# hku-mars/loam_livox

Measured on AMD Instinct MI355X. Metric: scans_per_s, higher is better.
Workload: dtype f32 points / f64 solve; 1 GPU; C2: 24k-pt Mid-40 scan vs 5M-pt corner+surface map, 10 ICP iters (fixed), k=5, Q-full; scan_points=24000, map_points=4975193, map_corner=995155, map_surf=3980038, icp_iters=10, distinct_scans_in_batch=256

## Files before the change

### __graft_entry__.py

```python
import os
import sys

ROOT = os.path.dirname(os.path.abspath(__file__))
if ROOT not in sys.path:
    sys.path.insert(0, ROOT)


def build() -> None:
    from loam_livox_amd import build as b
    lib = b.build()
    assert os.path.exists(lib)
    from oracle import orc
    orc.build()
    from tests.hostcheck import hc
    hc.build()
    from oracle import ref
    ref.build()
    from tests.test_ll_node import build_node
    build_node()
    from tests import verbatim_build
    verbatim_build.build()
    verbatim_build.build_sequence()
    verbatim_build.build_feature()
    verbatim_build.build_keyframes()
    verbatim_build.build_scene_alignment()
    verbatim_build.build_loop_detector()
    verbatim_build.build_cell_refresh()
    verbatim_build.build_mapping_io()
    import loam_livox_amd
    from loam_livox_amd import capi
    capi.load()


def smoke() -> None:
    import numpy as np

    from loam_livox_amd import synth
    from loam_livox_amd.api import Livox_laser, Map_buffer, Point_cloud_registration
    from oracle import orc

    world, corner, surf = synth.make_maps(60_000)
    sc = synth.make_scan(world, 0, n=6000)
    fe = Livox_laser(max_points=6000)
    fe.extract_laser_features(sc.xyzi, 9.0)
    g = fe.get_features(0.0, 1.0)
    o = orc.fe_extract(sc.xyzi, 10.0)
    ci, si, fi = orc.fe_get_features(o, 0.0, 1.0)
    assert np.array_equal(fe.pts_info()["pt_label"], o.pt_label), "label mismatch vs oracle"
    assert np.array_equal(g["corner_idx"], ci) and np.array_equal(g["surf_idx"], si), "index set mismatch vs oracle"
    m = Map_buffer()
    m.setInputCloud(Map_buffer.CORNER, corner)
    m.setInputCloud(Map_buffer.SURF, surf)
    reg = Point_cloud_registration(max_features=6000)
    p = reg.params
    p.icp_max_iterations, p.ceres_max_iterations, p.force_all_iterations = 4, 20, 1
    p.para_max_angular_rate, p.para_max_speed = 20.0, 0.3
    reg.m_pose_w_last = sc.pose_init.copy()
    reg.m_pose_w_curr = sc.pose_init.copy()
    ret = reg.find_out_incremental_transfrom(m, g["pc_corners"], g["pc_surface"])
    prm = orc.RegParams.defaults(icp_iters=4, ceres_iters=20, force_all=1)
    oret, opc, _, _ = orc.reg_solve(orc.KdTree(corner), orc.KdTree(surf), orc.feature_cloud(o, ci), orc.feature_cloud(o, si),
                                    prm, sc.pose_init, sc.pose_init)
    dt, dr = synth.pose_error(reg.m_pose_w_curr, opc)
    assert ret == oret and dt < 1e-4 and dr < 1e-4, f"pose mismatch vs oracle: {dt} m {dr} rad"
    print(f"smoke ok: labels/index sets identical, pose diff vs oracle {dt:.2e} m {dr:.2e} rad")


if __name__ == "__main__":
    build()
    if "--smoke" in sys.argv:
        smoke()
```

### include/loam_livox_hip.h

```cpp
#ifndef LOAM_LIVOX_HIP_H
#define LOAM_LIVOX_HIP_H

#include <stdint.h>

#ifdef __cplusplus
extern "C" {
#endif

typedef struct ll_fe ll_fe;
typedef struct ll_map ll_map;
typedef struct ll_reg ll_reg;

enum { LL_PT_NORMAL = 0, LL_PT_000 = 1, LL_PT_TOO_NEAR = 2, LL_PT_REFL_LOW = 4, LL_PT_REFL_HIGH = 8,
       LL_PT_CIRCLE_EDGE = 16, LL_PT_NAN = 32, LL_PT_SMALL_VIEW_ANGLE = 64 };
enum { LL_LABEL_INVALID = -1, LL_LABEL_UNLABELED = 0, LL_LABEL_CORNER = 1, LL_LABEL_SURFACE = 2,
       LL_LABEL_NEAR_NAN = 4, LL_LABEL_NEAR_ZERO = 8, LL_LABEL_HIGH_INTENSITY = 16 };


typedef struct {
    float thr_corner_curvature;
    float thr_surface_curvature;
    float minimum_view_angle;
    float livox_min_allow_dis;
    float livox_min_sigma;
    float max_fov;
    float time_internal_pts;
    int32_t device;
    int32_t max_points;
    int32_t max_scans;
    int32_t piecewise_number;
} ll_fe_params;

void ll_fe_default_params(ll_fe_params *p);
int ll_fe_create(const ll_fe_params *p, ll_fe **out);
void ll_fe_destroy(ll_fe *h);

int ll_fe_extract(ll_fe *h, const float *xyzi, int32_t n, double time_stamp, int32_t *n_petal_clouds);

int ll_fe_labels(ll_fe *h, int32_t scan, int32_t *pt_type, int32_t *pt_label, float *depth_sq2,
                 float *polar_dis_sq2, float *curvature, float *view_angle, float *time_stamp, float *polar_angle);

int ll_fe_splits(ll_fe *h, int32_t scan, int32_t *split_idx, int32_t *n_split, int32_t *clutter_size,
                 int32_t *n_petal_clouds, int32_t *first_idx, int32_t *last_idx, float *piece_start, float *piece_end);

int ll_fe_select(ll_fe *h, float minimum_blur, float maximum_blur, int32_t *corner_idx, int32_t *n_corner,
                 int32_t *surf_idx, int32_t *n_surf, int32_t *full_idx, int32_t *n_full, float *corner_xyzi,
                 float *surf_xyzi);

int ll_fe_upload(ll_fe *h, int32_t first_scan, int32_t n_scans, const float *xyzi, int32_t n_points,
                 const double *current_time);
int ll_fe_upload_async(ll_fe *h, int32_t first_scan, int32_t n_scans, const float *xyzi, int32_t n_points,
                       const double *current_time);
int ll_fe_extract_batch(ll_fe *h, int32_t n_scans);
int ll_fe_select_batch(ll_fe *h, int32_t n_scans, int32_t piece, float minimum_blur, float maximum_blur);
int ll_fe_selection(ll_fe *h, int32_t scan, int32_t *corner_idx, int32_t *n_corner, int32_t *surf_idx, int32_t *n_surf,
                    int32_t *full_idx, int32_t *n_full, float *corner_xyzi, float *surf_xyzi);
int ll_fe_counts(ll_fe *h, int32_t n_scans, int32_t *n_corner, int32_t *n_surf, int32_t *n_full,
                 int32_t *n_ambiguous);
int ll_fe_sync(ll_fe *h);
int ll_fe_resolve(ll_fe *h);


enum { LL_MAP_CORNER = 0, LL_MAP_SURF = 1 };

int ll_map_create(int32_t device, ll_map **out);
void ll_map_destroy(ll_map *m);
int ll_map_upload(ll_map *m, int32_t kind, const float *xyz, int32_t stride_floats, int64_t n, float cell_size);
int64_t ll_map_size(const ll_map *m, int32_t kind);

int64_t ll_map_generation(const ll_map *m, int32_t kind);
int64_t ll_map_cells(const ll_map *m, int32_t kind);
int ll_map_upload_gen(ll_map *m, int32_t kind, const float *xyz, int32_t stride_floats, int64_t n, float cell_size, int64_t *generation);
int ll_map_to_f16(ll_map *m, int32_t kind);
int ll_map_dequantized(ll_map *m, int32_t kind, float *xyz, int64_t capacity_points);

int ll_map_knn5(ll_map *m, int32_t kind, const float *queries_xyz, int32_t n_queries, float max_sq_dis,
                int32_t *idx5, float *sq_dis5);
int ll_map_knn5_device(ll_map *m, int32_t kind, const float *dev_queries_xyz, int64_t n_queries, float max_sq_dis, int32_t *dev_idx5,
                       float *dev_sq_dis5, float *kernel_ms);


typedef struct {
    int32_t if_motion_deblur;
    int32_t icp_max_iterations;
    int32_t ceres_max_iterations;
    int32_t ceres_prerun_times;
    int32_t icp_line;
    int32_t icp_plane;
    int32_t current_frame_index;
    int32_t mapping_init_accumulate_frames;
    int32_t maximum_allow_residual_block;
    int32_t force_all_iterations;
    double maximum_dis_line_for_match;
    double maximum_dis_plane_for_match;
    double huber_a;
    double inliner_dis;
    double inlier_ratio;
    double minimum_icp_R_diff;
    double minimum_icp_T_diff;
    float para_max_angular_rate;
    float para_max_speed;
    float max_final_cost;
    float minimum_pt_time_stamp;
    float maximum_pt_time_stamp;
    int32_t if_line_feature_check;
    int32_t if_plane_feature_check;
    int32_t subsample_seed;
} ll_reg_params;

void ll_reg_default_params(ll_reg_params *p);

typedef struct {
    double final_cost, initial_cost;
    double inlier_threshold;
    double angular_diff_deg, t_diff;
    int32_t icp_iterations;
    int32_t n_blocks_last;
    int32_t corner_avail, surf_avail;
    int32_t lm_iterations_total;
    int32_t accepted;
    int32_t gated;
    int32_t aborted;
} ll_reg_report;

int ll_reg_create(int32_t device, int32_t max_scans, int32_t max_features_per_scan, ll_reg **out);
void ll_reg_destroy(ll_reg *r);

int ll_reg_solve(ll_reg *r, const ll_map *map, const float *scan_corner_xyzi, int32_t n_corner,
                 const float *scan_surf_xyzi, int32_t n_surf, const ll_reg_params *prm, const double pose_last[7],
                 double pose_curr[7], double pose_incre[7], ll_reg_report *rep);

int ll_reg_solve_batch_fe(ll_reg *r, const ll_map *map, ll_fe *fe, int32_t n_scans, const ll_reg_params *prm,
                          const double *poses_last, double *poses_curr, double *poses_incre, ll_reg_report *reports,
                          int32_t *results);
int ll_reg_upload_features(ll_reg *r, int32_t n_scans, const float *corner_xyzi, const int32_t *n_corner, int32_t stride_corner,
                           const float *surf_xyzi, const int32_t *n_surf, int32_t stride_surf);
int ll_reg_enqueue_uploaded(ll_reg *r, const ll_map *map, int32_t n_scans, const ll_reg_params *prm, const double *poses_last,
                            const double *poses_curr, const double *poses_incre);

int ll_reg_solve_batch(ll_reg *r, const ll_map *map, int32_t n_scans, const float *corner_xyzi,
                       const int32_t *n_corner, int32_t stride_corner, const float *surf_xyzi, const int32_t *n_surf,
                       int32_t stride_surf, const ll_reg_params *prm, const double *poses_last, double *poses_curr,
                       double *poses_incre, ll_reg_report *reports, int32_t *results);

int ll_reg_enqueue_fe_merged(ll_reg *r, const ll_map *map, ll_fe *fe, int32_t n_scans, int32_t heads, const ll_reg_params *prm,
                             const double *poses_last, const double *poses_curr, const double *poses_incre);
int ll_reg_enqueue_fe(ll_reg *r, const ll_map *map, ll_fe *fe, int32_t n_scans, const ll_reg_params *prm,
                      const double *poses_last, const double *poses_curr, const double *poses_incre);
int ll_reg_collect(ll_reg *r, int32_t n_scans, double *poses_curr, double *poses_incre, ll_reg_report *reports,
                   int32_t *results);

int ll_debug_quintic(int32_t device, const double *args10, int32_t n, double *out_sequential, double *out_wavefront);

int ll_reg_debug_knn(ll_reg *r, int32_t scan, int32_t *corner_idx5, float *corner_d25, int32_t *surf_idx5,
                     float *surf_d25);
int ll_reg_set_debug(ll_reg *r, int32_t enable);
int ll_reg_set_debug_knn_iteration(ll_reg *r, int32_t icp_iteration);

typedef struct ll_voxel ll_voxel;
int ll_voxel_create(int32_t device, int32_t max_clouds, int32_t max_points_per_cloud, ll_voxel **out);
void ll_voxel_destroy(ll_voxel *v);
int ll_voxel_filter(ll_voxel *v, int32_t n_clouds, const float *xyzi, const int32_t *n_points, int32_t stride_points,
                    const float leaf[3], float *out_xyzi, int32_t *n_out, int32_t *status);

int ll_reg_enqueue_fe_downsampled(ll_reg *r, const ll_map *map, ll_fe *fe, ll_voxel *vox_corner, ll_voxel *vox_surf,
                                  float line_res, float plane_res, int32_t n_scans, const ll_reg_params *prm,
                                  const double *poses_last, const double *poses_curr, const double *poses_incre);
int ll_reg_enqueue_fe_maps(ll_reg *r, const ll_map *const *maps, ll_fe *fe, int32_t n_scans, const ll_reg_params *prm,
                           const int32_t *frame_index, const double *poses_last, const double *poses_curr, const double *poses_incre);
int ll_reg_enqueue_fe_downsampled_maps(ll_reg *r, const ll_map *const *maps, ll_fe *fe, ll_voxel *vox_corner, ll_voxel *vox_surf,
                                       float line_res, float plane_res, int32_t n_scans, const ll_reg_params *prm,
                                       const int32_t *frame_index, const double *poses_last, const double *poses_curr,
                                       const double *poses_incre);
int ll_voxel_counts(ll_voxel *v, int32_t n_clouds, int32_t *n_out, int32_t *status);

typedef struct ll_history ll_history;
int ll_history_create(int32_t device, int32_t maximum_history_size, int32_t max_points_per_frame, float line_res, float plane_res,
                      ll_history **out);
void ll_history_destroy(ll_history *h);
int ll_history_add(ll_history *h, const float *corner_xyzi, int32_t n_corner, const float *surf_xyzi, int32_t n_surf,
                   const double pose[7], double history_add_t_step, double history_add_angle_step, int32_t *added);
int ll_history_add_fe(ll_history *h, ll_fe *fe, int32_t scan, const double pose[7], double history_add_t_step,
                      double history_add_angle_step, int32_t *added);
int ll_history_add_voxel(ll_history *h, ll_voxel *vox_corner, ll_voxel *vox_surf, int32_t cloud, const double pose[7],
                         double history_add_t_step, double history_add_angle_step, int32_t *added);
int ll_history_set_gate_pose(ll_history *h, const double pose[7]);
int ll_history_refresh(ll_history *h, ll_map *map, int64_t *n_map_corner, int64_t *n_map_surf);
int32_t ll_history_size(const ll_history *h);
int64_t ll_history_map_cloud(ll_history *h, int32_t kind, float *xyzi, int64_t capacity_points);
int ll_history_map_cloud_device(ll_history *h, int32_t kind, const float **dev_xyzi, int64_t *n_points);

typedef struct ll_history_batch ll_history_batch;
int ll_history_batch_create(int32_t device, int32_t n_sequences, int32_t maximum_history_size, int32_t max_points_per_frame,
                            float line_res, float plane_res, ll_history_batch **out);
void ll_history_batch_destroy(ll_history_batch *h);
int ll_history_batch_add_voxel(ll_history_batch *h, ll_voxel *vox_corner, ll_voxel *vox_surf, const int32_t *active,
                               const double *poses7, const double *gate_poses7, double history_add_t_step,
                               double history_add_angle_step, int32_t *added);
int ll_history_batch_add_fe(ll_history_batch *h, ll_fe *fe, const int32_t *active, const double *poses7, const double *gate_poses7,
                            double history_add_t_step, double history_add_angle_step, int32_t *added);
int ll_history_batch_refresh(ll_history_batch *h, ll_map *const *maps, const int32_t *active, int64_t *n_map_corner,
                             int64_t *n_map_surf);
int32_t ll_history_batch_size(const ll_history_batch *h, int32_t sequence);
int64_t ll_history_batch_map_cloud(ll_history_batch *h, int32_t sequence, int32_t kind, float *xyzi, int64_t capacity_points);
int ll_history_batch_enable_cell_maps(ll_history_batch *h, int64_t initial_points_per_map, float cell_resolution,
                                      int32_t threshold_cell_revisit);
int ll_history_batch_sync_cell_maps(ll_history_batch *h);
int ll_history_batch_cell_map_stats(ll_history_batch *h, int32_t sequence, int32_t kind, int64_t *n_cells, int64_t *n_points,
                                    int32_t *frame_idx);
int ll_history_batch_cell_map_dump(ll_history_batch *h, int32_t sequence, int32_t kind, float *xyzi, int64_t capacity_points,
                                   int32_t *cell_ijk, int32_t *cell_start, int32_t *cell_last_update, int64_t capacity_cells);
int ll_history_batch_cell_map_device_view(ll_history_batch *h, int32_t sequence, int32_t kind, const float **dev_xyz0,
                                          const uint64_t **dev_point_keys, int64_t *n_points, int64_t *n_cells);
int ll_history_batch_cell_map_work(ll_history_batch *h, int64_t out[4]);
int ll_history_batch_refresh_cells(ll_history_batch *h, ll_map *const *maps, const int32_t *active, const double *poses7,
                                   float maximum_search_range_corner, float maximum_search_range_surface,
                                   float maximum_in_fov_angle, int32_t down_sample_replace,
                                   int64_t *n_map_corner, int64_t *n_map_surf);
int ll_history_batch_cell_match_work(ll_history_batch *h, int64_t out[8]);
int ll_history_batch_enable_full_maps(ll_history_batch *h, int64_t initial_points_per_map, float cell_resolution,
                                      int32_t threshold_cell_revisit);
int ll_history_batch_append_full_fe(ll_history_batch *h, ll_fe *fe, const int32_t *active, const double *poses7, int32_t min_points,
                                    int64_t *n_touched);
int ll_history_batch_full_touched(ll_history_batch *h, int32_t sequence, int32_t *cell_ijk, int64_t capacity_cells, int64_t *n);
int ll_history_batch_full_map_work(ll_history_batch *h, int64_t out[4]);
int ll_map_grid_geometry(const float bbox_min_max[6], float cell_size, int32_t dims[3], float *cell, float *slack);

typedef struct ll_cellmap ll_cellmap;
int ll_cellmap_create(int32_t device, int64_t max_points, float resolution, int32_t minimum_revisit_threshold, ll_cellmap **out);
void ll_cellmap_destroy(ll_cellmap *c);
int ll_cellmap_reserve(ll_cellmap *c, int64_t max_points);
int ll_cellmap_append(ll_cellmap *c, const float *xyzi, int32_t n);
int ll_cellmap_append_touched(ll_cellmap *c, const float *xyzi, int32_t n, int32_t min_points, int32_t *cell_ijk, int64_t capacity_cells,
                              int64_t *n_touched);
int ll_cellmap_query_filter(ll_cellmap *c, const double pose[7], float radius, float maximum_in_fov_angle, float leaf,
                            int32_t down_sample_replace, int64_t *n_cells_selected, int64_t *n_out);
int64_t ll_cellmap_result(ll_cellmap *c, float *xyzi, int64_t capacity_points);
int ll_cellmap_stats(const ll_cellmap *c, int64_t *n_cells, int64_t *n_points, int32_t *frame_idx);
int ll_cellmap_dump(ll_cellmap *c, float *xyzi, int64_t capacity_points, int32_t *cell_ijk, int32_t *cell_start,
                    int32_t *cell_last_update, int64_t capacity_cells);
int ll_cellmap_device_view(ll_cellmap *c, const float **dev_xyz0, const uint64_t **dev_point_keys, int64_t *n_points, int64_t *n_cells);
int ll_cellmap_extract_cells(ll_cellmap *src, const int32_t *cell_ijk, int64_t n_list, ll_cellmap *dst, int64_t *n_cells_found,
                             int64_t *n_points);
int ll_history_batch_extract_cells(ll_history_batch *h, int32_t kind, int32_t n_requests, const int32_t *sequences,
                                   const int64_t *list_offsets, const int32_t *cell_ijk, ll_cellmap *const *dst, int64_t *n_cells_found,
                                   int64_t *n_points);
int ll_history_batch_extract_work(ll_history_batch *h, int64_t out[4]);

int ll_cellmap_features(ll_cellmap *c, int32_t *feature_type, float *feature_vector, float *mean, float *cov, float *eigen_val,
                        int64_t capacity_cells);

int ll_cellmap_keyframe_images(ll_cellmap *c, float roi_ratio, float *images, float *ratio_nonzero, float *eigen_R, int32_t *n_vectors,
                               float *centre_and_range);
int ll_keyframe_similarity(int32_t device, const float *img_a, const float *img_b, float *similarity);

int ll_cellmap_feature_clouds(ll_cellmap *c, float *line_xyzi, int64_t capacity_line, int64_t *n_line, float *plane_xyzi, int64_t capacity_plane,
                              int64_t *n_plane, float centre[3]);
typedef struct ll_scene_align ll_scene_align;
typedef struct {
    float line_res, plane_res;
    int32_t maximum_icp_iteration;
    float accepted_threshold;
    int32_t maximum_residual_block;
    int32_t registrar_init;
    int32_t subsample_seed;
} ll_scene_align_params;
void ll_scene_align_default_params(ll_scene_align_params *p);
int ll_scene_align_create(int32_t device, int64_t initial_points, ll_scene_align **out);
void ll_scene_align_destroy(ll_scene_align *h);
int ll_scene_align_run(ll_scene_align *h, ll_cellmap *keyframe_a, ll_cellmap *keyframe_b, const ll_scene_align_params *p, double pose[7],
                       double *inlier_threshold, ll_reg_report reports[3], int32_t *n_reports);
int ll_scene_align_work(ll_scene_align *h, int64_t out[4]);

typedef struct ll_keyframe_bank ll_keyframe_bank;
int ll_keyframe_bank_create(int32_t device, int64_t initial_entries, ll_keyframe_bank **out);
void ll_keyframe_bank_destroy(ll_keyframe_bank *b);
int ll_keyframe_bank_add_cellmap(ll_keyframe_bank *b, ll_cellmap *c, float roi_ratio, float *images, float *ratio_nonzero, float *eigen_R,
                                 int32_t *n_vectors, float *centre_and_range, int64_t *id);
int ll_keyframe_bank_add_images(ll_keyframe_bank *b, const float *img_line, const float *img_plane, int64_t *id);
int ll_keyframe_bank_images(ll_keyframe_bank *b, int64_t id, float *img_line, float *img_plane);
int64_t ll_keyframe_bank_size(const ll_keyframe_bank *b);
int ll_keyframe_bank_match(ll_keyframe_bank *b, int64_t n_pairs, const int64_t *ids_a, const int64_t *ids_b, float *sim_line,
                           float *sim_plane);
int ll_keyframe_bank_debug_surface(ll_keyframe_bank *b, int64_t id_a, int64_t id_b, int32_t kind, double *out);
int ll_keyframe_bank_work(ll_keyframe_bank *b, int64_t out[4]);

typedef struct ll_pose_graph ll_pose_graph;
typedef struct {
    int32_t max_num_iterations;
    int32_t max_num_consecutive_invalid_steps;
    double initial_trust_region_radius;
    double max_trust_region_radius;
    double min_trust_region_radius;
    double min_relative_decrease;
    double min_lm_diagonal, max_lm_diagonal;
    double function_tolerance;
    double gradient_tolerance;
    double parameter_tolerance;
} ll_pose_graph_params;
#define LL_POSE_GRAPH_MAX_ITERATIONS 0
#define LL_POSE_GRAPH_GRADIENT 1
#define LL_POSE_GRAPH_PARAMETER 2
#define LL_POSE_GRAPH_FUNCTION 3
#define LL_POSE_GRAPH_RADIUS 4
#define LL_POSE_GRAPH_INVALID_STEPS 5
// ... 86 lines not shown
```

### loam_livox_amd/build.py

```python
from __future__ import annotations

import os
import shutil
import subprocess
import sys

HERE = os.path.dirname(os.path.abspath(__file__))
CSRC = os.path.join(HERE, "csrc")
LIB = os.environ.get("LL_LIB_OUT") or os.path.join(HERE, "libloamlivox_hip.so")
SOURCES = ["ll_api_common.hip", "ll_api_fe.hip", "ll_api_map.hip", "ll_api_reg.hip", "ll_api_voxel.hip", "ll_api_cellmap.hip", "ll_api_scene_align.hip", "ll_api_keyframe_bank.hip", "ll_api_pose_graph.hip", "ll_api_history.hip", "ll_api_history_batch_buffer.hip", "ll_api_history_batch_stores.hip", "ll_api_history_batch_extract.hip", "ll_api_history_batch_cells.hip", "ll_fe_kernels.hip", "ll_map_kernels.hip", "ll_reg_query_kernels.hip", "ll_reg_solve_kernels.hip", "ll_reg_maps_kernels.hip", "ll_reg_aux_kernels.hip", "ll_reg_small_kernels.hip", "ll_knn_kernels.hip", "ll_voxel_kernels.hip", "ll_cellmap_kernels.hip", "ll_cellmap_extract_kernels.hip", "ll_cellmap_select_kernels.hip", "ll_spin_kernels.hip", "ll_spin_api.hip", "ll_history_batch_kernels.hip", "ll_cellmap_batch_kernels.hip", "ll_cellmap_batch_extract_kernels.hip", "ll_cellmatch_batch_kernels.hip", "ll_fullmap_batch_kernels.hip", "ll_keyframe_bank_kernels.hip", "ll_pose_graph_kernels.hip"]
HEADERS = ["ll_api_internal.h", "ll_api_history_batch_internal.h", "ll_device.h", "ll_fe_core.h", "ll_knn_core.h", "ll_knn_coop.h", "ll_knn_tile.h", "ll_reg_query.h", "ll_reg_solve_fast.h", "ll_reg_big_path.h", "ll_reg_solve_general.h", "ll_reg_solve_common.h", "ll_reg_small_solve.h", "ll_reg_core.h", "ll_voxel.h", "ll_voxel_core.h", "ll_cellmap.h", "ll_cellmap_core.h", "ll_cellmap_select_core.h", "ll_spin.h", "ll_spin_core.h", "ll_history_batch.h", "ll_cellmap_batch.h", "ll_cellmap_batch_core.h", "ll_cellmap_batch_extract_core.h", "ll_cellmatch_batch.h", "ll_cellmatch_batch_core.h", "ll_fullmap_batch.h", "ll_fullmap_batch_core.h", "ll_keyframe_bank.h", "ll_keyframe_bank_core.h", "ll_pose_graph.h", "ll_pose_graph_core.h", "../../include/loam_livox_hip.h"]
FLAGS = ["--offload-arch=gfx950", "-O3", "-std=c++17", "-fPIC", "-ffp-contract=off", "-Wno-unused-result"]
FLAGS += os.environ.get("LL_EXTRA_HIPCC_FLAGS", "").split()


def hipcc() -> str:
    for cand in (shutil.which("hipcc"), "/opt/rocm/bin/hipcc"):
        if cand and os.path.exists(cand):
            return cand
    raise RuntimeError("hipcc not found (ROCm toolchain required to build libloamlivox_hip.so)")



def needs_build(lib: str = LIB) -> bool:
    if not os.path.exists(lib):
        return True
    t = os.path.getmtime(lib)
    deps = [os.path.join(CSRC, f) for f in SOURCES + HEADERS] + [os.path.abspath(__file__)]
    return any(os.path.getmtime(d) > t for d in deps)


def build(force: bool = False, verbose: bool = False, lib: str = LIB, extra_flags=()) -> str:
    if not force and not needs_build(lib):
        return lib
    cc = hipcc()
    default = os.path.join(HERE, "libloamlivox_hip.so")
    objdir = os.path.join(HERE, "build" if lib == default else "build_" + os.path.basename(lib).replace(".so", ""))
    os.makedirs(objdir, exist_ok=True)
    objs = []
    procs = []
    for src in SOURCES:
        obj = os.path.join(objdir, src.replace(".hip", ".o"))
        cmd = [cc] + FLAGS + list(extra_flags) + ["-c", os.path.join(CSRC, src), "-o", obj]
        if verbose:
            print(" ".join(cmd), file=sys.stderr)
        procs.append((src, subprocess.Popen(cmd, stdout=subprocess.PIPE, stderr=subprocess.STDOUT)))
        objs.append(obj)
    for src, p in procs:
        out, _ = p.communicate()
        if p.returncode != 0:
            raise RuntimeError(f"hipcc failed on {src}:\n{out.decode()}")
        if verbose and out:
            print(out.decode(), file=sys.stderr)
    cmd = [cc, "--offload-arch=gfx950", "-shared", "-fPIC", "-o", lib] + objs
    subprocess.check_call(cmd)
    return lib


if __name__ == "__main__":
    print(build(force="--force" in sys.argv, verbose=True))
```

### loam_livox_amd/capi.py

```python
from __future__ import annotations

import ctypes as C
import os

import numpy as np

_HERE = os.path.dirname(os.path.abspath(__file__))
LIB_PATH = os.environ.get("LOAM_LIVOX_LIB", os.path.join(_HERE, "libloamlivox_hip.so"))


class LoamLivoxError(RuntimeError):
    pass


class FeParams(C.Structure):
    _fields_ = [("thr_corner_curvature", C.c_float), ("thr_surface_curvature", C.c_float),
                ("minimum_view_angle", C.c_float), ("livox_min_allow_dis", C.c_float), ("livox_min_sigma", C.c_float),
                ("max_fov", C.c_float), ("time_internal_pts", C.c_float), ("device", C.c_int32),
                ("max_points", C.c_int32), ("max_scans", C.c_int32), ("piecewise_number", C.c_int32)]


class SpinParams(C.Structure):
    _fields_ = [("scan_line", C.c_int32), ("minimum_range", C.c_float), ("plane_resolution", C.c_float), ("device", C.c_int32),
                ("max_points", C.c_int32), ("max_scans", C.c_int32), ("max_line_points", C.c_int32)]
# ... 18 lines not shown
                ("n_blocks_last", C.c_int32), ("corner_avail", C.c_int32), ("surf_avail", C.c_int32),
                ("lm_iterations_total", C.c_int32), ("accepted", C.c_int32), ("gated", C.c_int32), ("aborted", C.c_int32)]


class SceneAlignParams(C.Structure):
    _fields_ = [("line_res", C.c_float), ("plane_res", C.c_float), ("maximum_icp_iteration", C.c_int32), ("accepted_threshold", C.c_float),
                ("maximum_residual_block", C.c_int32), ("registrar_init", C.c_int32), ("subsample_seed", C.c_int32)]


class PoseGraphParams(C.Structure):
    _fields_ = [("max_num_iterations", C.c_int32), ("max_num_consecutive_invalid_steps", C.c_int32),
                ("initial_trust_region_radius", C.c_double), ("max_trust_region_radius", C.c_double),
                ("min_trust_region_radius", C.c_double), ("min_relative_decrease", C.c_double), ("min_lm_diagonal", C.c_double),
                ("max_lm_diagonal", C.c_double), ("function_tolerance", C.c_double), ("gradient_tolerance", C.c_double),
                ("parameter_tolerance", C.c_double)]


class PoseGraphSummary(C.Structure):
    _fields_ = [("iterations", C.c_int32), ("successful_steps", C.c_int32), ("unsuccessful_steps", C.c_int32), ("termination", C.c_int32),
                ("initial_cost", C.c_double), ("final_cost", C.c_double)]


POSE_GRAPH_TERMINATION = ("max_iterations", "gradient", "parameter", "function", "radius", "invalid_steps", "nothing")


_vp, _i32, _i64, _f, _d = C.c_void_p, C.c_int32, C.c_int64, C.c_float, C.c_double
SYMBOLS = {
    "ll_fe_default_params": (None, [C.POINTER(FeParams)]),
    "ll_fe_create": (_i32, [C.POINTER(FeParams), C.POINTER(_vp)]),
    "ll_fe_destroy": (None, [_vp]),
    "ll_fe_extract": (_i32, [_vp, _vp, _i32, _d, C.POINTER(_i32)]),
    "ll_fe_labels": (_i32, [_vp, _i32] + [_vp] * 8),
    "ll_fe_splits": (_i32, [_vp, _i32, _vp, C.POINTER(_i32), C.POINTER(_i32), C.POINTER(_i32), _vp, _vp, _vp, _vp]),
    "ll_fe_select": (_i32, [_vp, _f, _f, _vp, C.POINTER(_i32), _vp, C.POINTER(_i32), _vp, C.POINTER(_i32), _vp, _vp]),
    "ll_fe_selection": (_i32, [_vp, _i32, _vp, C.POINTER(_i32), _vp, C.POINTER(_i32), _vp, C.POINTER(_i32), _vp, _vp]),
    "ll_fe_upload": (_i32, [_vp, _i32, _i32, _vp, _i32, _vp]),
    "ll_fe_upload_async": (_i32, [_vp, _i32, _i32, _vp, _i32, _vp]),
    "ll_fe_extract_batch": (_i32, [_vp, _i32]),
    "ll_fe_select_batch": (_i32, [_vp, _i32, _i32, _f, _f]),
    "ll_fe_counts": (_i32, [_vp, _i32, _vp, _vp, _vp, _vp]),
    "ll_fe_sync": (_i32, [_vp]),
    "ll_fe_resolve": (_i32, [_vp]),
    "ll_map_create": (_i32, [_i32, C.POINTER(_vp)]),
    "ll_map_destroy": (None, [_vp]),
    "ll_map_upload": (_i32, [_vp, _i32, _vp, _i32, _i64, _f]),
    "ll_map_upload_gen": (_i32, [_vp, _i32, _vp, _i32, _i64, _f, _vp]),
    "ll_map_size": (_i64, [_vp, _i32]),
    "ll_map_generation": (_i64, [_vp, _i32]),
    "ll_map_to_f16": (_i32, [_vp, _i32]),
    "ll_map_dequantized": (_i32, [_vp, _i32, _vp, _i64]),
    "ll_map_cells": (_i64, [_vp, _i32]),
    "ll_map_knn5": (_i32, [_vp, _i32, _vp, _i32, _f, _vp, _vp]),
    "ll_map_knn5_device": (_i32, [_vp, _i32, _vp, _i64, _f, _vp, _vp, _vp]),
    "ll_reg_default_params": (None, [C.POINTER(RegParams)]),
    "ll_reg_create": (_i32, [_i32, _i32, _i32, C.POINTER(_vp)]),
    "ll_reg_destroy": (None, [_vp]),
    "ll_reg_solve": (_i32, [_vp, _vp, _vp, _i32, _vp, _i32, C.POINTER(RegParams), _vp, _vp, _vp, C.POINTER(RegReport)]),
    "ll_reg_solve_batch_fe": (_i32, [_vp, _vp, _vp, _i32, C.POINTER(RegParams), _vp, _vp, _vp, _vp, _vp]),
    "ll_reg_solve_batch": (_i32, [_vp, _vp, _i32, _vp, _vp, _i32, _vp, _vp, _i32, C.POINTER(RegParams), _vp, _vp, _vp,
                                  _vp, _vp]),
    "ll_reg_upload_features": (_i32, [_vp, _i32, _vp, _vp, _i32, _vp, _vp, _i32]),
    "ll_reg_enqueue_uploaded": (_i32, [_vp, _vp, _i32, C.POINTER(RegParams), _vp, _vp, _vp]),
    "ll_reg_enqueue_fe": (_i32, [_vp, _vp, _vp, _i32, C.POINTER(RegParams), _vp, _vp, _vp]),
    "ll_reg_enqueue_fe_merged": (_i32, [_vp, _vp, _vp, _i32, _i32, C.POINTER(RegParams), _vp, _vp, _vp]),
    "ll_reg_collect": (_i32, [_vp, _i32, _vp, _vp, _vp, _vp]),
    "ll_reg_debug_knn": (_i32, [_vp, _i32, _vp, _vp, _vp, _vp]),
    "ll_reg_set_debug": (_i32, [_vp, _i32]),
    "ll_reg_set_debug_knn_iteration": (_i32, [_vp, _i32]),
    "ll_cloud_transform": (_i32, [_vp, _vp, _vp, _i32, _vp]),
    "ll_cloud_transform_fe_device": (_i32, [_vp, _vp, _i32, _i32, _vp, _vp, _vp, _i64, _vp]),
    "ll_reg_set_profiling": (_i32, [_vp, _i32]),
    "ll_reg_kernel_times": (_i32, [_vp, _vp, _vp]),
    "ll_reg_debug_cycles": (_i32, [_vp, _i32, _vp]),
    "ll_reg_debug_worklists": (_i32, [_vp, _i32, _vp]),
    "ll_voxel_create": (_i32, [_i32, _i32, _i32, C.POINTER(_vp)]),
    "ll_voxel_destroy": (None, [_vp]),
    "ll_voxel_filter": (_i32, [_vp, _i32, _vp, _vp, _i32, _vp, _vp, _vp, _vp]),
    "ll_voxel_counts": (_i32, [_vp, _i32, _vp, _vp]),
    "ll_reg_enqueue_fe_downsampled": (_i32, [_vp, _vp, _vp, _vp, _vp, _f, _f, _i32, C.POINTER(RegParams), _vp, _vp, _vp]),
    "ll_reg_enqueue_fe_maps": (_i32, [_vp, _vp, _vp, _i32, C.POINTER(RegParams), _vp, _vp, _vp, _vp]),
    "ll_reg_enqueue_fe_downsampled_maps": (_i32, [_vp, _vp, _vp, _vp, _vp, _f, _f, _i32, C.POINTER(RegParams), _vp, _vp, _vp, _vp]),
    "ll_history_create": (_i32, [_i32, _i32, _i32, _f, _f, C.POINTER(_vp)]),
    "ll_history_destroy": (None, [_vp]),
    "ll_history_add": (_i32, [_vp, _vp, _i32, _vp, _i32, _vp, C.c_double, C.c_double, _vp]),
    "ll_history_add_fe": (_i32, [_vp, _vp, _i32, _vp, C.c_double, C.c_double, _vp]),
    "ll_history_add_voxel": (_i32, [_vp, _vp, _vp, _i32, _vp, C.c_double, C.c_double, _vp]),
    "ll_history_refresh": (_i32, [_vp, _vp, _vp, _vp]),
    "ll_history_size": (_i32, [_vp]),
    "ll_history_map_cloud": (_i64, [_vp, _i32, _vp, _i64]),
    "ll_history_set_gate_pose": (_i32, [_vp, _vp]),
    "ll_history_map_cloud_device": (_i32, [_vp, _i32, _vp, _vp]),
    "ll_history_batch_create": (_i32, [_i32, _i32, _i32, _i32, _f, _f, C.POINTER(_vp)]),
    "ll_history_batch_destroy": (None, [_vp]),
    "ll_history_batch_add_voxel": (_i32, [_vp, _vp, _vp, _vp, _vp, _vp, C.c_double, C.c_double, _vp]),
    "ll_history_batch_add_fe": (_i32, [_vp, _vp, _vp, _vp, _vp, C.c_double, C.c_double, _vp]),
    "ll_history_batch_refresh": (_i32, [_vp, _vp, _vp, _vp, _vp]),
    "ll_history_batch_size": (_i32, [_vp, _i32]),
    "ll_history_batch_map_cloud": (_i64, [_vp, _i32, _i32, _vp, _i64]),
    "ll_history_batch_enable_cell_maps": (_i32, [_vp, _i64, C.c_float, _i32]),
    "ll_history_batch_sync_cell_maps": (_i32, [_vp]),
    "ll_history_batch_cell_map_stats": (_i32, [_vp, _i32, _i32, _vp, _vp, _vp]),
    "ll_history_batch_cell_map_dump": (_i32, [_vp, _i32, _i32, _vp, _i64, _vp, _vp, _vp, _i64]),
    "ll_history_batch_cell_map_device_view": (_i32, [_vp, _i32, _i32, _vp, _vp, _vp, _vp]),
    "ll_history_batch_cell_map_work": (_i32, [_vp, _vp]),
    "ll_history_batch_refresh_cells": (_i32, [_vp, _vp, _vp, _vp, C.c_float, C.c_float, C.c_float, _i32, _vp, _vp]),
    "ll_history_batch_cell_match_work": (_i32, [_vp, _vp]),
    "ll_history_batch_enable_full_maps": (_i32, [_vp, _i64, C.c_float, _i32]),
    "ll_history_batch_append_full_fe": (_i32, [_vp, _vp, _vp, _vp, _i32, _vp]),
    "ll_history_batch_full_touched": (_i32, [_vp, _i32, _vp, _i64, _vp]),
    "ll_history_batch_full_map_work": (_i32, [_vp, _vp]),
    "ll_history_batch_extract_cells": (_i32, [_vp, _i32, _i32, _vp, _vp, _vp, _vp, _vp, _vp]),
    "ll_history_batch_extract_work": (_i32, [_vp, _vp]),
    "ll_map_grid_geometry": (_i32, [_vp, _f, _vp, _vp, _vp]),
    "ll_cellmap_create": (_i32, [_i32, _i64, C.c_float, _i32, _vp]),
    "ll_cellmap_destroy": (None, [_vp]),
    "ll_cellmap_reserve": (_i32, [_vp, _i64]),
    "ll_cellmap_device_view": (_i32, [_vp, _vp, _vp, _vp, _vp]),
    "ll_cellmap_extract_cells": (_i32, [_vp, _vp, _i64, _vp, _vp, _vp]),
    "ll_cellmap_append": (_i32, [_vp, _vp, _i32]),
    "ll_cellmap_append_touched": (_i32, [_vp, _vp, _i32, _i32, _vp, _i64, C.POINTER(_i64)]),
    "ll_cellmap_query_filter": (_i32, [_vp, _vp, C.c_float, C.c_float, C.c_float, _i32, _vp, _vp]),
    "ll_cellmap_result": (_i64, [_vp, _vp, _i64]),
    "ll_cellmap_stats": (_i32, [_vp, _vp, _vp, _vp]),
    "ll_cellmap_dump": (_i32, [_vp, _vp, _i64, _vp, _vp, _vp, _i64]),
    "ll_cellmap_features": (_i32, [_vp, _vp, _vp, _vp, _vp, _vp, _i64]),
    "ll_cellmap_keyframe_images": (_i32, [_vp, C.c_float, _vp, _vp, _vp, _vp, _vp]),
    "ll_keyframe_similarity": (_i32, [_i32, _vp, _vp, _vp]),
    "ll_cellmap_feature_clouds": (_i32, [_vp, _vp, _i64, C.POINTER(_i64), _vp, _i64, C.POINTER(_i64), _vp]),
    "ll_scene_align_default_params": (None, [C.POINTER(SceneAlignParams)]),
    "ll_scene_align_create": (_i32, [_i32, _i64, C.POINTER(_vp)]),
    "ll_scene_align_destroy": (None, [_vp]),
    "ll_scene_align_run": (_i32, [_vp, _vp, _vp, C.POINTER(SceneAlignParams), _vp, C.POINTER(_d), _vp, C.POINTER(_i32)]),
    "ll_scene_align_work": (_i32, [_vp, _vp]),
    "ll_keyframe_bank_create": (_i32, [_i32, _i64, C.POINTER(_vp)]),
    "ll_keyframe_bank_destroy": (None, [_vp]),
    "ll_keyframe_bank_add_cellmap": (_i32, [_vp, _vp, C.c_float, _vp, _vp, _vp, _vp, _vp, C.POINTER(_i64)]),
    "ll_keyframe_bank_add_images": (_i32, [_vp, _vp, _vp, C.POINTER(_i64)]),
    "ll_keyframe_bank_images": (_i32, [_vp, _i64, _vp, _vp]),
    "ll_keyframe_bank_size": (_i64, [_vp]),
    "ll_keyframe_bank_match": (_i32, [_vp, _i64, _vp, _vp, _vp, _vp]),
    "ll_keyframe_bank_debug_surface": (_i32, [_vp, _i64, _i64, _i32, _vp]),
    "ll_keyframe_bank_work": (_i32, [_vp, _vp]),
    "ll_pose_graph_default_params": (None, [C.POINTER(PoseGraphParams)]),
    "ll_pose_graph_create": (_i32, [_i32, _i64, _i64, _i64, _i64, C.POINTER(_vp)]),
    "ll_pose_graph_destroy": (None, [_vp]),
    "ll_pose_graph_solve": (_i32, [_vp, C.POINTER(PoseGraphParams), _i64, _vp, _vp, _vp, _vp, _vp, _vp, _vp]),
    "ll_pose_graph_work": (_i32, [_vp, _vp]),
    "ll_history_enable_cell_map": (_i32, [_vp, _i64, C.c_float, _i32]),
    "ll_history_set_cell_map_async": (_i32, [_vp, _i32]),
    "ll_history_sync_cell_maps": (_i32, [_vp]),
    "ll_history_cell_map": (_vp, [_vp, _i32]),
    "ll_history_refresh_cells": (_i32, [_vp, _vp, _vp, C.c_float, C.c_float, C.c_float, _i32, _vp, _vp]),
    "ll_debug_quintic": (_i32, [_i32, _vp, _i32, _vp, _vp]),
    "ll_spin_default_params": (None, [C.POINTER(SpinParams)]),
    "ll_spin_create": (_i32, [C.POINTER(SpinParams), C.POINTER(_vp)]),
    "ll_spin_destroy": (None, [_vp]),
    "ll_spin_upload": (_i32, [_vp, _i32, _i32, _vp, _vp, _i32]),
    "ll_spin_extract_batch": (_i32, [_vp, _i32]),
    "ll_spin_resolve": (_i32, [_vp]),
    "ll_spin_sync": (_i32, [_vp]),
    "ll_spin_counts": (_i32, [_vp, _i32, _vp, _vp]),
    "ll_spin_cloud": (_i32, [_vp, _i32, _i32, _vp, _vp, C.POINTER(_i32)]),
    "ll_spin_lines": (_i32, [_vp, _i32, _vp, _vp]),
    "ll_spin_extract": (_i32, [_vp, _vp, _i32]),
    "ll_spin_kernel_times": (_i32, [_vp, _vp]),
    "ll_reg_enqueue_spin": (_i32, [_vp, _vp, _vp, _i32, C.POINTER(RegParams), _vp, _vp, _vp]),
    "ll_reg_enqueue_spin_downsampled": (_i32, [_vp, _vp, _vp, _vp, _vp, _f, _f, _i32, C.POINTER(RegParams), _vp, _vp, _vp]),
    "ll_history_add_spin": (_i32, [_vp, _vp, _i32, _vp, C.c_double, C.c_double, _vp]),
    "ll_cloud_transform_spin_device": (_i32, [_vp, _vp, _i32, _i32, _vp, _vp, _vp, _i64, _vp]),
    "ll_spin_handoff_time": (_i32, [_vp, _vp]),
    "ll_reg_stream": (_vp, [_vp]),
    "ll_fe_stream": (_vp, [_vp]),
    "ll_runtime_hint_hw_queues": (_i32, [_i32]),
    "ll_last_error": (C.c_char_p, []),
    "ll_version": (C.c_char_p, []),
}

_lib = None




def hint_hw_queues(n: int = 16) -> bool:
    return check(load().ll_runtime_hint_hw_queues(int(n)), "ll_runtime_hint_hw_queues") == 1


def load():
    global _lib
    if _lib is not None:
        return _lib
    if not os.path.exists(LIB_PATH):
        raise LoamLivoxError(
            f"{LIB_PATH} not found: build it with `python -m loam_livox_amd.build` (hipcc, gfx950). "
            "There is no CPU fallback.")
    try:
        L = C.CDLL(LIB_PATH)
    except OSError as e:
        raise LoamLivoxError(f"cannot load {LIB_PATH}: {e} (ROCm runtime required; there is no CPU fallback)") from e
    for name, (res, args) in SYMBOLS.items():
        fn = getattr(L, name)
        fn.restype = res
        fn.argtypes = args
    _lib = L
    return L


class use_library:

    def __init__(self, path: str):
        self.path = path

    def __enter__(self):
        global _lib, LIB_PATH
        self.saved = (_lib, LIB_PATH)
        _lib, LIB_PATH = None, self.path
        try:
            return load()
        except Exception:
            _lib, LIB_PATH = self.saved
            raise

    def __exit__(self, *exc):
        global _lib, LIB_PATH
        _lib, LIB_PATH = self.saved
        return False


def check(rc: int, what: str = "") -> int:
    if rc < 0:
        msg = load().ll_last_error()
        raise LoamLivoxError(f"{what}: {msg.decode() if msg else 'error'}")
    return rc


def ptr(a):
    return None if a is None else a.ctypes.data_as(C.c_void_p)


def fe_default_params() -> FeParams:
    p = FeParams()
    load().ll_fe_default_params(C.byref(p))
    return p


def spin_default_params() -> SpinParams:
    p = SpinParams()
    load().ll_spin_default_params(C.byref(p))
    return p


def reg_default_params() -> RegParams:
    p = RegParams()
    load().ll_reg_default_params(C.byref(p))
    return p


def scene_align_default_params() -> SceneAlignParams:
    p = SceneAlignParams()
    load().ll_scene_align_default_params(C.byref(p))
    return p


def pose_graph_default_params() -> PoseGraphParams:
    p = PoseGraphParams()
    load().ll_pose_graph_default_params(C.byref(p))
    return p


def as_f32(a, cols=None):
    a = np.ascontiguousarray(a, dtype=np.float32)
    if cols is not None:
        a = a.reshape(-1, cols)
    return a
```

### loam_livox_amd/csrc/ll_api_reg.hip

```cpp
#include "ll_api_internal.h"

extern "C" void ll_reg_default_params(ll_reg_params *p)
{
    memset(p, 0, sizeof(*p));
    p->if_motion_deblur = 0;
    p->icp_max_iterations = 20;
    p->ceres_max_iterations = 100;
    p->ceres_prerun_times = 2;
    p->icp_line = 1;
    p->icp_plane = 1;
    p->if_line_feature_check = 0;
    p->if_plane_feature_check = 0;
    p->subsample_seed = 0;
    p->current_frame_index = 101;
    p->mapping_init_accumulate_frames = 100;
    p->maximum_allow_residual_block = 100000;
    p->force_all_iterations = 0;
    p->maximum_dis_line_for_match = 2.0;
    p->maximum_dis_plane_for_match = 50.0;
    p->huber_a = 0.1;
    p->inliner_dis = 0.02;
    p->inlier_ratio = 0.80;
    p->minimum_icp_R_diff = 0.01;
    p->minimum_icp_T_diff = 0.01;
// ... 286 lines not shown
    return 0;
}

static int reg_size_check(const char *where, const ll_reg *r, const ll_reg_params *prm, int max_nc, int max_ns, const char *cite)
{
    if (max_nc > r->dev.cap_c || max_ns > r->dev.cap_s) return set_err(where, "feature count exceeds the registrar capacity");
    if (!prm->subsample_seed && (max_nc > prm->maximum_allow_residual_block || max_ns > prm->maximum_allow_residual_block))
        return set_err(where, (std::string("feature count exceeds maximum_allow_residual_block and subsample_seed is 0 (strict mode): raise the "
                                           "limit, or set a seed to get the reference's sub-sampling ") + cite + "with a reproducible random stream").c_str());
    return 0;
}

static int reg_finish(ll_reg *r, int n_scans, PinGuard &pin_guard)
{
    prof_begin(r, 2);
    launch_reg_finalize(r->dev, r->rc, n_scans, r->stream);
    prof_end(r);
    HC(hipGetLastError());
    pin_guard.keep = true;
    return 0;
}

static int reg_enqueue(const char *where, ll_reg *r, const ll_map *map, int n_scans, const ll_reg_params *prm, const double *poses_last,
                       const double *poses_curr, const double *poses_incre, const int *known_counts = nullptr)
{
    if (!map) return set_err(where, "null argument");
    if (reg_params_check(where, r, n_scans, prm, poses_last, poses_curr)) return -1;
    if (map->device != r->device) return set_err(where, "map lives on another device");
    int debug = 0;
    if (reg_begin(r, prm, &debug)) return -1;
    PinGuard pin_guard{r};
    r->pinned[0] = map_pin(map, 0);
    r->pinned[1] = map_pin(map, 1);
    const MapKind empty_kind{};
    const MapKind &mk0 = r->pinned[0] ? r->pinned[0]->mk : empty_kind, &mk1 = r->pinned[1] ? r->pinned[1]->mk : empty_kind;
    const bool run = mk0.n > 0 && mk1.n > 50 && prm->current_frame_index > prm->mapping_init_accumulate_frames;
    r->last_gated = run ? 0 : 1;
    r->last_n_scans = n_scans;
    for (int b = 0; b < n_scans; b++) reg_init_state(r->h_state[b], b, poses_last, poses_curr, poses_incre, run);
    if (reg_exchange_counts(r, n_scans, false, n_scans == 1 ? known_counts : nullptr)) return -1;
    int max_nc = 0, max_ns = 0;
    for (int b = 0; b < n_scans; b++) {
        max_nc = r->h_nc[b] > max_nc ? r->h_nc[b] : max_nc;
        max_ns = r->h_ns[b] > max_ns ? r->h_ns[b] : max_ns;
    }
    if (reg_size_check(where, r, prm, max_nc, max_ns, "(point_cloud_registration.hpp:232-238,339-345,438-458) ")) return -1;
    if (prm->subsample_seed && (max_nc > 2 * prm->maximum_allow_residual_block || max_ns > 2 * prm->maximum_allow_residual_block))
        r->rc.knn_reuse = 0;
    if (max_ns < LL_KNN_TILE_MIN_SURF || max_ns > LL_KNN_TILE_MAX_SURF || (n_scans <= LL_KNN_COOP_MAX_SCANS && !(debug & 2048))) r->rc.knn_tile = 0;
    if (r->rc.knn_tile == 2 && max_ns > LL_KNN_TILE_SEG) r->rc.knn_tile = 1;
    if (r->rc.knn_tile == 2) r->rc.knn_reuse = 0;
    r->rc.solve_group = (r->rc.solve_group == 1 || n_scans > LL_GRP_MAX_SCANS || r->rc.if_motion_deblur || r->rc.force_general ||
                         max_nc + max_ns < LL_GRP_MIN_BLOCKS) ? 1 : LL_GRP;
    if (run) {
        if (!mk0.pts || !mk1.pts) return set_err(where, "map not uploaded (or converted to fp16 points: the registrar needs the fp32 records)");
        Grid g0 = mk0.grid, g1 = mk1.grid;
        g0.guard = g1.guard = r->rc.knn_reuse ? 0.05f : 0.0f;
        if (r->rc.solve_group > 1)
            HC(hipMemsetAsync(r->dev.grp_xch, 0, (size_t)n_scans * 2 * LL_GRP * 56 * sizeof(unsigned long long), r->stream));
        for (int it = 0; it < prm->icp_max_iterations; it++) {
            r->rc.xch_epoch = it + 1;
            prof_begin(r, 0);
            launch_reg_knn_build(r->dev, r->rc, g0, g1, n_scans, it, max_nc, max_ns, r->stream);
            prof_end(r);
            prof_begin(r, 1);
            if (r->rc.solve_group > 1) HC(hipMemsetAsync(r->dev.grp_ctl, 0, (size_t)(2 * n_scans + 1) * sizeof(int), r->stream));
            launch_reg_solve(r->dev, r->rc, mk1.grid, n_scans, max_nc, max_ns, it, r->stream);
            prof_end(r);
        }
    }
    return reg_finish(r, n_scans, pin_guard);
}

extern "C" int ll_reg_collect(ll_reg *r, int32_t n_scans, double *poses_curr, double *poses_incre, ll_reg_report *reports,
                              int32_t *results)
{
    if (!r) return set_err("ll_reg_collect", "null handle");
    if (n_scans < 1 || n_scans > r->max_scans) return set_err("ll_reg_collect", "n_scans out of range");
    HC(hipSetDevice(r->device));
    HC(hipMemcpyAsync(r->h_state.data(), r->dev.state, (size_t)n_scans * sizeof(RegState), hipMemcpyDeviceToHost, r->stream));
    HC(hipStreamSynchronize(r->stream));
    r->pinned[0].reset();
    r->pinned[1].reset();
    r->pinned_maps.clear();
    int n_aborted = 0;
    for (int b = 0; b < n_scans; b++) {
        const RegState &s = r->h_state[b];
        n_aborted += s.aborted ? 1 : 0;
        for (int i = 0; i < 7; i++) {
            if (poses_curr) poses_curr[7 * b + i] = s.pose_curr[i];
            if (poses_incre) poses_incre[7 * b + i] = s.inc[i];
        }
        if (results) results[b] = s.result;
        if (reports) {
            ll_reg_report &rp = reports[b];
            rp.final_cost = s.final_cost;
            rp.initial_cost = s.initial_cost;
            rp.inlier_threshold = s.inlier_thr;
            rp.angular_diff_deg = s.angular_diff;
            rp.t_diff = s.t_diff;
            rp.icp_iterations = s.icp_iters;
            rp.n_blocks_last = s.n_blocks_last;
            rp.corner_avail = s.corner_avail;
            rp.surf_avail = s.surf_avail;
            rp.lm_iterations_total = s.lm_total;
            rp.accepted = s.accepted;
            rp.gated = s.gated;
            rp.aborted = s.aborted ? 1 : 0;
        }
    }
    if (r->profiling) {
        for (int k = 0; k < 3; k++) {
            r->prof_ms[k] = 0.f;
            r->prof_launches[k] = 0;
        }
        for (size_t i = 0; i < r->ev_class.size(); i++) {
            float ms = 0.f;
            if (hipEventElapsedTime(&ms, r->ev[2 * i], r->ev[2 * i + 1]) == hipSuccess) {
                r->prof_ms[r->ev_class[i]] += ms;
                r->prof_launches[r->ev_class[i]]++;
            }
        }
    }
    if (n_aborted) {
        (void)set_err("ll_reg_collect", "a group barrier of the small-batch solver timed out (device oversubscribed?): the affected scans were rejected");
        return n_aborted;
    }
    return 0;
}

extern "C" int ll_debug_quintic(int32_t device, const double *args10, int32_t n, double *out_sequential, double *out_wavefront)
{
    if (!args10 || !out_sequential || !out_wavefront || n < 0) return set_err("ll_debug_quintic", "bad argument");
    if (check_device(device)) return -1;
    double *d_a = nullptr, *d_s = nullptr, *d_w = nullptr;
    const size_t m = (size_t)(n > 0 ? n : 1);
    HC(hipMalloc((void **)&d_a, m * 10 * sizeof(double)));
    HC(hipMalloc((void **)&d_s, m * sizeof(double)));
    HC(hipMalloc((void **)&d_w, m * sizeof(double)));
    int rc = 0;
    if (hipMemcpy(d_a, args10, (size_t)n * 10 * sizeof(double), hipMemcpyHostToDevice) != hipSuccess) rc = -1;
    if (!rc) {
        launch_debug_quintic(d_a, n, d_s, d_w, nullptr);
        if (hipDeviceSynchronize() != hipSuccess || hipMemcpy(out_sequential, d_s, (size_t)n * sizeof(double), hipMemcpyDeviceToHost) != hipSuccess ||
            hipMemcpy(out_wavefront, d_w, (size_t)n * sizeof(double), hipMemcpyDeviceToHost) != hipSuccess)
            rc = -1;
    }
    (void)hipFree(d_a);
    (void)hipFree(d_s);
    (void)hipFree(d_w);
    return rc ? set_err("ll_debug_quintic", "device error") : 0;
}

extern "C" int ll_reg_debug_cycles(ll_reg *r, int32_t scan, long long out[16])
{
    if (!r || scan < 0 || scan >= r->max_scans) return set_err("ll_reg_debug_cycles", "bad argument");
    for (int i = 0; i < 16; i++) out[i] = r->h_state[scan].dbg_cycles[i];
    return 0;
}

extern "C" int ll_reg_debug_worklists(ll_reg *r, int32_t n_scans, int64_t out[4])
{
    if (!r || !out || n_scans < 1 || n_scans > r->max_scans) return set_err("ll_reg_debug_worklists", "bad argument");
    HC(hipSetDevice(r->device));
    const size_t n = (size_t)n_scans * 4;
    std::vector<int> h(n);
    HC(hipStreamSynchronize(r->stream));
    HC(hipMemcpy(h.data(), r->dev.work_cnt, n * sizeof(int), hipMemcpyDeviceToHost));
    out[0] = out[1] = out[2] = out[3] = 0;
    for (size_t i = 0; i < n; i++) out[i & 3] += h[i];
    return 0;
}

extern "C" int ll_reg_kernel_times(ll_reg *r, float ms[3], int32_t launches[3])
{
    if (!r) return set_err("ll_reg_kernel_times", "null handle");
    for (int k = 0; k < 3; k++) {
        if (ms) ms[k] = r->prof_ms[k];
        if (launches) launches[k] = r->prof_launches[k];
    }
    return 0;
}

static int reg_fe_fits(const char *where, const ll_reg *r, const ll_fe *fe, int n_scans)
{
    if (n_scans > fe->prm.max_scans) return set_err(where, "n_scans exceeds the extractor capacity");
    if (fe->prm.max_points > r->max_feat) return set_err(where, "registrar feature capacity < extractor max_points");
    return 0;
}

extern "C" int ll_reg_enqueue_fe(ll_reg *r, const ll_map *map, ll_fe *fe, int32_t n_scans, const ll_reg_params *prm,
                                 const double *poses_last, const double *poses_curr, const double *poses_incre)
{
    static const char *where = "ll_reg_enqueue_fe";
    if (!r || !fe) return set_err(where, "null handle");
    if (fe->prm.device != r->device) return set_err(where, "extractor lives on another device");
    if (reg_fe_fits(where, r, fe, n_scans)) return -1;
    HC(hipSetDevice(r->device));
    if (reg_bind(r, feat_view(fe))) return -1;
    return reg_enqueue(where, r, map, n_scans, prm, poses_last, poses_curr, poses_incre);
}

static int reg_maps_check(const char *where, ll_reg *r, const ll_map *const *maps, int n_scans, const ll_reg_params *prm, const double *poses_last,
                          const double *poses_curr)
{
    if (!r || !maps) return set_err(where, "null argument");
    if (reg_params_check(where, r, n_scans, prm, poses_last, poses_curr)) return -1;
    if (prm->if_motion_deblur)
        return set_err(where, "motion deblur is not supported with a map per slot (if_motion_deblur must be 0): register such scans through the single-map entry points");
    for (int b = 0; b < n_scans; b++)
        if (maps[b] && maps[b]->device != r->device) return set_err(where, "map lives on another device");
    return 0;
}

static int reg_enqueue_maps(const char *where, ll_reg *r, const ll_map *const *maps, int n_scans, const ll_reg_params *prm, const int32_t *frame_index,
                            const double *poses_last, const double *poses_curr, const double *poses_incre)
{
    if (reg_begin(r, prm)) return -1;
    PinGuard pin_guard{r};
    r->rc.knn_tile = 0;
    r->rc.knn_reuse = 0;
    std::vector<const ll_map *> seen;
    std::vector<int> pin_of(n_scans, -1);
    for (int b = 0; b < n_scans; b++) {
        if (!maps[b]) continue;
        size_t k = 0;
        while (k < seen.size() && seen[k] != maps[b]) k++;
        if (k == seen.size()) {
            seen.push_back(maps[b]);
            r->pinned_maps.push_back(map_pin(maps[b], 0));
            r->pinned_maps.push_back(map_pin(maps[b], 1));
        }
        pin_of[b] = (int)k;
    }
    const MapKind empty_kind{};
    int n_run = 0;
    for (int b = 0; b < n_scans; b++) {
        const MapSnap *s0 = pin_of[b] >= 0 ? r->pinned_maps[2 * pin_of[b]].get() : nullptr, *s1 = pin_of[b] >= 0 ? r->pinned_maps[2 * pin_of[b] + 1].get() : nullptr;
        const MapKind &mk0 = s0 ? s0->mk : empty_kind, &mk1 = s1 ? s1->mk : empty_kind;
        const int fi = frame_index ? frame_index[b] : prm->current_frame_index;
        const bool run = mk0.n > 0 && mk1.n > 50 && fi > prm->mapping_init_accumulate_frames;
        if (run && (!mk0.pts || !mk1.pts)) return set_err(where, "map not uploaded (or converted to fp16 points: the registrar needs the fp32 records)");
        Grid g0{}, g1{};
        if (run) g0 = mk0.grid, g1 = mk1.grid;
        g0.guard = g1.guard = 0.0f;
        r->h_map_tab[2 * b] = g0;
        r->h_map_tab[2 * b + 1] = g1;
        n_run += run ? 1 : 0;
        reg_init_state(r->h_state[b], b, poses_last, poses_curr, poses_incre, run);
    }
    r->last_gated = n_run ? 0 : 1;
    r->last_n_scans = n_scans;
    if (reg_exchange_counts(r, n_scans, true)) return -1;
    int max_nc = 0, max_ns = 0;
    RegMapsClasses cls{};
    int max_tot[4] = {0, 0, 0, 0};
    cls.grp_min = r->rc.solve_group == 1 ? 0x7fffffff : LL_GRP_MIN_BLOCKS;
    for (int b = 0; b < n_scans; b++) {
        if (r->h_state[b].done) continue;
        const int nc = r->h_nc[b], ns = r->h_ns[b], c = reg_maps_class(r->rc, nc, ns, cls.grp_min);
        max_nc = nc > max_nc ? nc : max_nc;
        max_ns = ns > max_ns ? ns : max_ns;
        cls.n[c]++;
        cls.max_nc[c] = nc > cls.max_nc[c] ? nc : cls.max_nc[c];
        cls.max_ns[c] = ns > cls.max_ns[c] ? ns : cls.max_ns[c];
        max_tot[c] = nc + ns > max_tot[c] ? nc + ns : max_tot[c];
    }
    for (int c = 0; c < 2; c++) cls.max_ns[c] = max_tot[c] - cls.max_nc[c];
    if (reg_size_check(where, r, prm, max_nc, max_ns, "")) return -1;
    r->rc.solve_group = cls.n[3] ? LL_GRP : 1;
    if (n_run) {
        if ((cls.n[2] && !reg_solve_fast_eligible(r->rc, cls.max_nc[2], cls.max_ns[2])) || (cls.n[3] && !reg_solve_fast_eligible(r->rc, cls.max_nc[3], cls.max_ns[3])))
            return set_err(where, "a scan of this batch is beyond the compact solver's size (or the general solver was forced): not supported with a map "
                                  "per slot, register such scans through the single-map entry points");
        if (r->rc.solve_group > 1)
            HC(hipMemsetAsync(r->dev.grp_xch, 0, (size_t)n_scans * 2 * LL_GRP * 56 * sizeof(unsigned long long), r->stream));
        for (int it = 0; it < prm->icp_max_iterations; it++) {
            r->rc.xch_epoch = it + 1;
            prof_begin(r, 0);
            launch_reg_knn_build_maps(r->dev, r->rc, r->d_map_tab, n_scans, it, max_nc, max_ns, r->stream);
            prof_end(r);
            prof_begin(r, 1);
            if (r->rc.solve_group > 1) HC(hipMemsetAsync(r->dev.grp_ctl, 0, (size_t)(2 * n_scans + 1) * sizeof(int), r->stream));
            launch_reg_solve_maps(r->dev, r->rc, r->d_map_tab, n_scans, cls, it, r->stream);
            prof_end(r);
        }
    }
    return reg_finish(r, n_scans, pin_guard);
}

extern "C" int ll_reg_enqueue_fe_maps(ll_reg *r, const ll_map *const *maps, ll_fe *fe, int32_t n_scans, const ll_reg_params *prm,
                                      const int32_t *frame_index, const double *poses_last, const double *poses_curr, const double *poses_incre)
{
    static const char *where = "ll_reg_enqueue_fe_maps";
    if (!r || !fe) return set_err(where, "null handle");
    if (reg_maps_check(where, r, maps, n_scans, prm, poses_last, poses_curr)) return -1;
    if (fe->prm.device != r->device) return set_err(where, "extractor lives on another device");
    if (reg_fe_fits(where, r, fe, n_scans)) return -1;
    HC(hipSetDevice(r->device));
    if (reg_bind(r, feat_view(fe))) return -1;
    return reg_enqueue_maps(where, r, maps, n_scans, prm, frame_index, poses_last, poses_curr, poses_incre);
}

static int reg_voxel_check(const char *where, const ll_reg *r, const ll_voxel *vc, const ll_voxel *vs)
{
    if (vc->device != r->device || vs->device != r->device) return set_err(where, "handles live on different devices");
// ... 300 lines not shown
```

### loam_livox_amd/csrc/ll_device.h

```cpp
#pragma once
#include <hip/hip_runtime.h>
#include <stdint.h>

#include "ll_fe_core.h"
#include "ll_knn_core.h"

namespace ll {

#define LL_MAX_PIECES 8
#define LL_GRP 8
#define LL_GRP_MIN_BLOCKS 6000
#define LL_GRP_MAX_SCANS 16
#define LL_KNN_COOP_MAX_QUERIES 8192
#define LL_KNN_COOP_MAX_SCANS 16
#define LL_KNN_COOP_MAX_SURF 2048
#define LL_KNN_TILE_MIN_SURF 1024
#define LL_KNN_TILE_SEG 24576
#define LL_KNN_TILE_MAX_SURF (4 * LL_KNN_TILE_SEG)

#define LL_SMALL_MAX_BLOCKS 2048
#define LL_SMALL_W1_MIN_SCANS 512
#define LL_SMALL_ORDER_MIN_SCANS 512
#define LL_SMALL_ORDER_MAX_SCANS 8192

struct FeScanInfo {
    int n_split;
    int clutter_size;
    int n_petal_clouds;
    int pad;
    float piece_start[LL_MAX_PIECES], piece_end[LL_MAX_PIECES];
};

struct FeDev {
    const float4 *xyzi;
    const int *npts;
    const double *time0;
    int stride;
    int *type, *label;
    float *depth2, *polar2, *curv, *view, *tstamp, *polar_angle;
    float2 *img;
    signed char *flags;
    int *cand;
    int split_cap;
    int *split_idx, *petal_first, *petal_last;
    float *run_angle;
    FeScanInfo *info;
    int *corner_idx, *surf_idx, *full_idx;
    float4 *corner_feat, *surf_feat;
    int *n_corner, *n_surf, *n_full;
    int *n_ambig;
    int2 *ambig_list;
    int ambig_cap;
};

void launch_fe_point(const FeDev &fb, const FeConst &fc, int n_scans, int max_n, hipStream_t s);
void launch_fe_split(const FeDev &fb, int pieces, int n_scans, hipStream_t s);
void launch_fe_select(const FeDev &fb, int n_scans, int piece, float min_blur, float max_blur, hipStream_t s);


struct MapKind {
    f4 *pts = nullptr;
    int *cell_start = nullptr;
    unsigned long long *pts16 = nullptr;
    int *perm = nullptr;
    int64_t n = 0;
    int64_t n_valid = 0;
    Grid grid{};
    size_t ncell = 0;
    size_t cap_pts = 0, cap_cells = 0;
    size_t cap_n = 0, cap_tmp = 0;
    unsigned int *b_keys = nullptr, *b_keys2 = nullptr;
    int *b_vals = nullptr, *b_vals2 = nullptr, *b_counts = nullptr;
    void *b_tmp = nullptr;
    float *b_mm = nullptr;
};

int map_build(MapKind &mk, const float *d_raw, int stride, int64_t n, float cell, hipStream_t s, const char **err);
int map_bbox_enqueue(const float *d_raw, int stride, const int *d_n, int64_t n_max, float *d_mm, hipStream_t s, const char **err);
int map_build_boxed(MapKind &mk, const float *d_raw, int stride, int64_t n, float cell, const float mm[6], bool wait, hipStream_t s, const char **err);
void map_free(MapKind &mk);
void map_grid_geometry(const float mm[6], float cell, Grid &g);
int map_to_f16(MapKind &mk, hipStream_t s, const char **err);
int map_f16_dequant(const MapKind &mk, float *d_out_xyz, hipStream_t s, const char **err);
void launch_knn5(const Grid &g, const float *d_q, int nq, float max_d2, int *d_idx, float *d_d2, hipStream_t s);


struct RegState {
    double pose_last[7], pose_curr[7], inc[7];
    double prev_q[4], prev_t[3];
    double interp_theta, hat[9], hat_sq[9];
    double inlier_thr, final_cost, initial_cost, angular_diff, t_diff;
    int icp_iters, n_blocks_last, corner_avail, surf_avail, lm_total;
    int done, accepted, gated, result;
    int last_work;
    int aborted;
    long long dbg_cycles[16];
};

struct RegConst {
    int if_motion_deblur, icp_max_iterations, ceres_max_iterations, ceres_prerun_times;
    int icp_line, icp_plane, force_all_iterations, debug_knn;
    int debug_knn_iter;
    int force_general;
    int knn_reuse;
    int knn_reuse_from;
    int check_line_pca, check_plane_pca;
    int solve_group;
    int xch_epoch;
    int test_group_abort;
    int knn_coop;
    int knn_tile_last_sort;
    int no_solve_order;
    int no_small_solver;
    int small_waves;
    int no_line_cache;
    int knn_tile;
    unsigned int subsample_seed;
    int max_blocks;
    float max_d2_line, max_d2_plane;
    double max_d2_line_d, max_d2_plane_d;
    double huber_a, inliner_dis, inlier_ratio, minimum_icp_R_diff, minimum_icp_T_diff;
    double bound;
    float para_max_angular_rate, max_final_cost, min_ts, max_ts;
};

struct RegDev {
    RegState *state;
    const float4 *corner_feat;
    const float4 *surf_feat;
    const int *n_corner, *n_surf;
    int feat_stride_c, feat_stride_s;
    int cap_c, cap_s, cap;
    float4 *blk_f;
    double *blk_av;
    unsigned short *blk_id;
    int4 *pl_tab;
    int tab_cap;
    float4 *qw;
    float4 *ref_q;
    int4 *ref_p;
    float2 *ref_s;
    int *solve_order;
    int *grp_ctl;
    double *grp_part;
    unsigned long long *grp_xch;
    unsigned char *blk_flag0;
    int *work_search;
    int *work_build;
    int *work_off;
    int *work_cnt;
    int n_chunks;
    int4 *nn;
    unsigned short *qperm;
    unsigned short *qperm_c;
    float4 *qsorted;
    unsigned char *blk_flag;
    double *blk_l1;
    unsigned long long *hash;
    int hash_cap;
    int *dbg_idx;
    float *dbg_d2;
};

void launch_reg_knn_build(const RegDev &rd, const RegConst &rc, const Grid &gc, const Grid &gs, int n_scans, int iter,
                          int max_nc, int max_ns, hipStream_t s);
#define LL_QSORT_CORNER_MAX 2048
void launch_reg_qsort(const RegDev &rd, const RegConst &rc, const Grid &gc, const Grid &gs, int n_scans, int max_nc, int max_ns, bool fused, hipStream_t s);
void launch_debug_quintic(const double *args, int n, double *out_seq, double *out_wave, hipStream_t s);
void launch_reg_knn_tile(const RegDev &rd, const RegConst &rc, const Grid &gc, const Grid &gs, int n_scans, int iter, int max_nc, int max_ns,
                         bool fused, hipStream_t s);
void launch_reg_solve(const RegDev &rd, const RegConst &rc, const Grid &gs, int n_scans, int max_nc, int max_ns, int iter, hipStream_t s);
bool reg_solve_small_eligible(const RegConst &rc, int max_nc, int max_ns);
bool reg_solve_fast_eligible(const RegConst &rc, int max_nc, int max_ns);
void launch_reg_solve_small(const RegDev &rd, const RegConst &rc, const Grid &gs, int n_scans, int max_nc, int max_ns, int iter, hipStream_t s);
int reg_solve_small_waves(const RegConst &rc, int n_scans, int max_nc, int max_ns);
void launch_reg_knn_build_maps(const RegDev &rd, const RegConst &rc, const Grid *map_tab, int n_scans, int iter, int max_nc, int max_ns, hipStream_t s);
__host__ __device__ inline int reg_maps_class(const RegConst &rc, int nc, int ns, int grp_min)
{
    const bool small = !rc.force_general && !rc.no_small_solver && nc + ns > 0 && nc + ns <= LL_SMALL_MAX_BLOCKS && nc <= 1024;
    return small ? (nc + ns <= 1024 ? 0 : 1) : (nc + ns < grp_min ? 2 : 3);
}
struct RegMapsClasses {
    int n[4], max_nc[4], max_ns[4];
    int grp_min;
};
void launch_reg_solve_maps(const RegDev &rd, const RegConst &rc, const Grid *map_tab, int n_scans, const RegMapsClasses &cls, int iter, hipStream_t s);
void launch_reg_solve_small_maps(const RegDev &rd, const RegConst &rc, const Grid *map_tab, int n_scans, int cls, int max_nc, int max_ns, int iter, hipStream_t s);
void launch_reg_finalize(const RegDev &rd, const RegConst &rc, int n_scans, hipStream_t s);
void launch_cloud_transform(const float4 *in, float4 *out, int n, const double *d_pose, hipStream_t s);
#define LL_HIST_CONCAT_MAX 1023
void launch_history_concat(const float4 *frames, const int2 *d_table, int n_seg, int total, float4 *out, hipStream_t s);
void launch_reg_merge_heads(const float4 *fe_corner, const float4 *fe_surf, const int *fe_nc, const int *fe_ns, int fe_stride, int heads,
                            float4 *dst_corner, float4 *dst_surf, int *dst_nc, int *dst_ns, int dst_stride, int n_scans, hipStream_t s);

}
```

### loam_livox_amd/csrc/ll_reg_aux_kernels.hip

```cpp
#include <hip/hip_runtime.h>

#include "ll_device.h"
#include "ll_reg_solve_common.h"

namespace ll {

__global__ void reg_finalize_kernel(RegDev rd, RegConst rc, int n_scans)
{
    const int b = blockIdx.x * blockDim.x + threadIdx.x;
    if (b >= n_scans) return;
    RegState *st = rd.state + b;
    st->result = 1;
    st->accepted = 1;
    if (st->gated || st->icp_iters == 0) return;
    st->inlier_thr = st->inlier_thr * st->final_cost / st->initial_cost;
    const float minimize_cost = (float)st->final_cost;
    const bool broken = st->aborted || !((st->angular_diff - st->angular_diff) == 0.0) || !((st->final_cost - st->final_cost) == 0.0);
    if (broken || st->angular_diff > (double)rc.para_max_angular_rate || minimize_cost > rc.max_final_cost) {
        for (int i = 0; i < 7; i++) st->pose_curr[i] = st->pose_last[i];
        st->result = 0;
        st->accepted = 0;
    }
}
void launch_reg_finalize(const RegDev &rd, const RegConst &rc, int n_scans, hipStream_t s)
{
    hipLaunchKernelGGL(reg_finalize_kernel, dim3((n_scans + 63) / 64), dim3(64), 0, s, rd, rc, n_scans);
}

__global__ void cloud_transform_kernel(const float4 *in, float4 *out, int n, const double *pose)
{
    const int i = blockIdx.x * blockDim.x + threadIdx.x;
    if (i >= n) return;
    double p[7];
#pragma unroll
    for (int k = 0; k < 7; k++) p[k] = pose[k];
    const float4 v = in[i];
    float o[3];
    point_to_map(p, v.x, v.y, v.z, o);
    out[i] = make_float4(o[0], o[1], o[2], v.w);
}
void launch_cloud_transform(const float4 *in, float4 *out, int n, const double *d_pose, hipStream_t s)
{
    if (n <= 0) return;
    hipLaunchKernelGGL(cloud_transform_kernel, dim3((n + 255) / 256), dim3(256), 0, s, in, out, n, d_pose);
}

__global__ void reg_merge_heads_kernel(const float4 *fe_corner, const float4 *fe_surf, const int *fe_nc, const int *fe_ns, int fe_stride,
                                       int heads, float4 *dst_corner, float4 *dst_surf, int *dst_nc, int *dst_ns, int dst_stride)
{
    const int slot = blockIdx.y, kind = blockIdx.z;
    const int b = slot / heads, h = slot - b * heads;
    const int *cnt = kind ? fe_ns : fe_nc;
    int off = 0;
    for (int k = 0; k < h; k++) off += cnt[b * heads + k];
    const int n = cnt[slot];
    const int i = blockIdx.x * blockDim.x + threadIdx.x;
    if (i < n && off + i < dst_stride) {
        const float4 *src = (kind ? fe_surf : fe_corner) + (size_t)slot * fe_stride;
        float4 *dst = (kind ? dst_surf : dst_corner) + (size_t)b * dst_stride;
        dst[off + i] = src[i];
    }
    if (i == 0 && h == heads - 1) (kind ? dst_ns : dst_nc)[b] = off + n;
}
void launch_reg_merge_heads(const float4 *fe_corner, const float4 *fe_surf, const int *fe_nc, const int *fe_ns, int fe_stride, int heads,
                            float4 *dst_corner, float4 *dst_surf, int *dst_nc, int *dst_ns, int dst_stride, int n_scans, hipStream_t s)
{
    hipLaunchKernelGGL(reg_merge_heads_kernel, dim3((fe_stride + 255) / 256, n_scans * heads, 2), dim3(256), 0, s, fe_corner, fe_surf, fe_nc,
                       fe_ns, fe_stride, heads, dst_corner, dst_surf, dst_nc, dst_ns, dst_stride);
}

__global__ __launch_bounds__(256) void history_concat_kernel(const float4 *frames, const int2 *table, int n_seg, float4 *out)
{
    __shared__ int2 s_tab[LL_HIST_CONCAT_MAX + 1];
    for (int e = threadIdx.x; e <= n_seg; e += 256) s_tab[e] = table[e];
    __syncthreads();
    const int total = s_tab[n_seg].y;
    for (int i = blockIdx.x * 256 + threadIdx.x; i < total; i += gridDim.x * 256) {
        int lo = 0, hi = n_seg - 1;
        while (lo < hi) {
            const int mid = (lo + hi + 1) >> 1;
            if (s_tab[mid].y <= i)
                lo = mid;
            else
                hi = mid - 1;
        }
        out[i] = frames[(size_t)s_tab[lo].x + (size_t)(i - s_tab[lo].y)];
    }
}
void launch_history_concat(const float4 *frames, const int2 *d_table, int n_seg, int total, float4 *out, hipStream_t s)
{
    if (n_seg <= 0 || total <= 0) return;
    const int blocks = (total + 255) / 256 < 1024 ? (total + 255) / 256 : 1024;
    hipLaunchKernelGGL(history_concat_kernel, dim3(blocks), dim3(256), 0, s, frames, d_table, n_seg, out);
}

__global__ __launch_bounds__(64) void debug_quintic_kernel(const double *args, int n, double *out_seq, double *out_wave)
{
    const int i = blockIdx.x, lane = threadIdx.x;
    if (i >= n) return;
    const double *a = args + 10 * (size_t)i;
    const double w = lm_quintic_min_step_wave(a[0], a[1], a[2], a[3], a[4], a[5], a[6], a[7], a[8], a[9], lane);
    if (lane == 0) {
        out_wave[i] = w;
        out_seq[i] = lm_quintic_min_step(a[0], a[1], a[2], a[3], a[4], a[5], a[6], a[7], a[8], a[9]);
    }
}
void launch_debug_quintic(const double *args, int n, double *out_seq, double *out_wave, hipStream_t s)
{
    if (n > 0) hipLaunchKernelGGL(debug_quintic_kernel, dim3(n), dim3(64), 0, s, args, n, out_seq, out_wave);
}

}
```

### loam_livox_amd/csrc/ll_reg_big_path.h

```cpp
#pragma once
#include "ll_reg_solve_fast.h"
#include "ll_reg_solve_general.h"

namespace ll {

#define PT_BIG_MAX_PROBE 32

struct Act2 {
    unsigned long long lo, hi;
};
__device__ __forceinline__ bool act_test(const Act2 &a, int k) { return (((k & 64) ? a.hi : a.lo) >> (k & 63)) & 1ull; }
__device__ __forceinline__ void act_set(Act2 &a, int k)
{
    const unsigned long long bit = 1ull << (k & 63);
    a.lo |= (k & 64) ? 0ull : bit;
    a.hi |= (k & 64) ? bit : 0ull;
}
__device__ __forceinline__ void act_clear(Act2 &a, int k)
{
    const unsigned long long bit = 1ull << (k & 63);
    a.lo &= (k & 64) ? ~0ull : ~bit;
    a.hi &= (k & 64) ? ~bit : ~0ull;
}
__device__ __forceinline__ int act_count(const Act2 &a) { return __popcll(a.lo) + __popcll(a.hi); }
// ... 286 lines not shown
        Q.b = lds_load_i4(tabL + 2 * idl_);                                                        \
        Q.c = lds_load_i4(tabL + 2 * idl_ + 1);                                                    \
        if (!TAB_LDS) {                                                                            \
            G_.b = gload_i4(tabG + 2 * idg_);                                                      \
            G_.c = gload_i4(tabG + 2 * idg_ + 1);                                                  \
        }                                                                                          \
    }
#define LB_USE(R, Q, G_, K)                                                                                \
    if ((K) < kp) {                                                                                        \
        const int pp_ = tid + (K) * RS_THREADS;                                                            \
        if (pp_ < nS && act_test(act, (K))) {                                                              \
            const bool near_ = TAB_LDS || R.id < (unsigned int)Tl;                                         \
            const int4 pb_ = near_ ? Q.b : G_.b, pc_ = near_ ? Q.c : G_.c;                                 \
            const double f[3] = {(double)__int_as_float(R.fx), (double)__int_as_float(R.fy), (double)__int_as_float(R.fz)}; \
            const double v[3] = {__hiloint2double(pb_.y, pb_.x), __hiloint2double(pb_.w, pb_.z), __hiloint2double(pc_.y, pc_.x)}; \
            const double a[3] = {__hiloint2double(pc_.w, pc_.z), 0.0, 0.0};                                \
            if (DEBLUR) {                                                                                  \
                const double s_ = (double)refine_blur(1, __int_as_float(R.fw), min_ts, max_ts);  \
                block_accumulate_mb(BLK_PLANE, mb_, t_, s_, f, a, v, huber_a, acc);                        \
                if (L1OUT) gstore_f64(l1_planes + pp_, block_l1_mb(BLK_PLANE, mb_, t_, s_, f, a, v, huber_a, q_last)); \
            } else {                                                                                       \
                block_accumulate(BLK_PLANE, R_, t_, f, a, v, huber_a, acc);                                \
                if (L1OUT) gstore_f64(l1_planes + pp_, block_l1(BLK_PLANE, R_, t_, f, a, v, huber_a, q_last)); \
            }                                                                                              \
        }                                                                                                  \
    }
#define LB_PIPE()                                                      \
    {                                                                  \
        if (kp > 0) {                                                  \
            RecB r0, r1, r2, r3, r4;                                   \
            Pl3 q0, q1, g0, g1;                                        \
            LB_LOAD(r0, 0)                                             \
            LB_LOAD(r1, 1)                                             \
            LB_LOAD(r2, 2)                                             \
            LB_LOAD(r3, 3)                                             \
            LB_PLANE(q0, g0, r0)                                       \
            for (int k = 0; k < kp; k += 10) {                         \
                LB_LOAD(r4, k + 4)                                     \
                LB_PLANE(q1, g1, r1)                                   \
                LB_USE(r0, q0, g0, k)                                  \
                LB_LOAD(r0, k + 5)                                     \
                LB_PLANE(q0, g0, r2)                                   \
                LB_USE(r1, q1, g1, k + 1)                              \
                LB_LOAD(r1, k + 6)                                     \
                LB_PLANE(q1, g1, r3)                                   \
                LB_USE(r2, q0, g0, k + 2)                              \
                LB_LOAD(r2, k + 7)                                     \
                LB_PLANE(q0, g0, r4)                                   \
                LB_USE(r3, q1, g1, k + 3)                              \
                LB_LOAD(r3, k + 8)                                     \
                LB_PLANE(q1, g1, r0)                                   \
                LB_USE(r4, q0, g0, k + 4)                              \
                LB_LOAD(r4, k + 9)                                     \
                LB_PLANE(q0, g0, r1)                                   \
                LB_USE(r0, q1, g1, k + 5)                              \
                LB_LOAD(r0, k + 10)                                    \
                LB_PLANE(q1, g1, r2)                                   \
                LB_USE(r1, q0, g0, k + 6)                              \
                LB_LOAD(r1, k + 11)                                    \
                LB_PLANE(q0, g0, r3)                                   \
                LB_USE(r2, q1, g1, k + 7)                              \
                LB_LOAD(r2, k + 12)                                    \
                LB_PLANE(q1, g1, r4)                                   \
                LB_USE(r3, q0, g0, k + 8)                              \
                LB_LOAD(r3, k + 13)                                    \
                LB_PLANE(q0, g0, r0)                                   \
                LB_USE(r4, q1, g1, k + 9)                              \
            }                                                          \
        }                                                              \
    }

template <bool L1OUT, int DEBLUR>
__device__ __noinline__ void big_eval(const RegDev &rd, const RegConst &rc, int b, int nC, int nS, const double *x, Act2 act, uint4 *s_raw,
                                      const double *q_last_g, SolveShared &sh)
{
    const int tid = threadIdx.x, lane = tid & 63, wave = tid >> 6;
    const double huber_a = rc.huber_a;
    const float min_ts = rc.min_ts, max_ts = rc.max_ts;
    double q_last[4] = {0.0, 0.0, 0.0, 1.0};
    if (L1OUT) {
        q_last[0] = q_last_g[0];
        q_last[1] = q_last_g[1];
        q_last[2] = q_last_g[2];
        q_last[3] = q_last_g[3];
    }
    double *l1_planes = rd.blk_l1 + (size_t)b * rd.cap + rd.cap_c;
    double *l1_lines = rd.blk_l1 + (size_t)b * rd.cap;
    LL_CTX_DECL(x)
    double acc[LL_NACC];
#pragma unroll
    for (int i = 0; i < LL_NACC; i++) acc[i] = 0.0;
    const int Tl = sh.pt_Tl;
    const int kp = (nS + RS_THREADS - 1) / RS_THREADS;
    const int4 *tabL = (const int4 *)s_raw;
    const int4 *tabG = pt_table_global(rd, b, 0, false);
    const unsigned short *ids = rd.blk_id + (size_t)b * rd.cap_s;
    const float4 *feat = rd.surf_feat + (size_t)b * rd.feat_stride_s;
    if (sh.pt_T <= PT_TCAP) {
        constexpr bool TAB_LDS = true;
        LB_PIPE()
    } else {
        constexpr bool TAB_LDS = false;
        LB_PIPE()
    }
    {
        const size_t sb = (size_t)b * rd.cap;
        const double *av = rd.blk_av + (size_t)b * 6 * rd.cap;
        int k = kp;
        for (int l = tid; l < nC; l += RS_THREADS, k++) {
            if (!act_test(act, k)) continue;
            BlkRegs br;
            load_blk(rd, sb, av, l, br);
            const double a[3] = {br.a0, br.a1, br.a2};
            const double v[3] = {br.v0, br.v1, br.v2};
            LL_CTX_ACCUM(BLK_LINE, br.f, a, v, huber_a, acc);
            if (L1OUT) {
                double l1;
                LL_CTX_L1(l1, BLK_LINE, br.f, a, v, huber_a, q_last);
                l1_lines[l] = l1;
            }
        }
    }
    wave_sum_acc(acc, sh.red[wave], lane);
    __syncthreads();
    if (tid < LL_NACC) {
        double s = 0.0;
        for (int w = 0; w < RS_WAVES; w++) s += sh.red[w][tid];
        sh.sum[tid] = s;
    }
    __syncthreads();
}
#undef LB_LOAD
#undef LB_PLANE
#undef LB_USE
#undef LB_PIPE

template <bool WANT_L1, int DEBLUR>
__device__ __forceinline__ void big_lm(const RegDev &rd, const RegConst &rc, int b, int nC, int nS, const double *x0, int max_iter, int n_active, Act2 act,
                                       uint4 *s_raw, const double *q_last, SolveShared &sh)
{
    const int tid = threadIdx.x;
    if (tid == 0) {
        lm_begin(sh.ctl, x0, max_iter, rc.bound);
        sh.l1_valid = 0;
    }
    __syncthreads();
    {
        LL_T0(t0);
        big_eval<false, DEBLUR>(rd, rc, b, nC, nS, sh.ctl.x, act, s_raw, q_last, sh);
        LL_TACC(0, t0);
    }
    {
        LL_T0(t1);
        if (tid == 0) sh.need = lm_init(sh.ctl, sh.sum, n_active);
        __syncthreads();
        LL_TACC(1, t1);
    }
    while (sh.need) {
        const bool spec = WANT_L1 && sh.ctl.iteration >= max_iter;
        LL_T0(t0);
        if (spec)
            big_eval<true, DEBLUR>(rd, rc, b, nC, nS, sh.ctl.cand, act, s_raw, q_last, sh);
        else
            big_eval<false, DEBLUR>(rd, rc, b, nC, nS, sh.ctl.cand, act, s_raw, q_last, sh);
        LL_TACC(0, t0);
        LL_T0(t1);
        if (tid < 64) {
            const int need = lm_update_wave(sh.ctl, sh.sum, sh.fit, tid);
            if (tid == 0) {
                sh.need = need;
                sh.l1_valid = (spec && !need && sh.ctl.last_accept == 1) ? 1 : 0;
            }
        }
        __syncthreads();
        LL_TACC(1, t1);
    }
}

template <int DEBLUR>
__device__ __noinline__ Act2 big_inlier(const RegDev &rd, const RegConst &rc, int b, RegState *st, SolveShared &sh, uint4 *s_raw, Act2 act, int nC, int nS)
{
    const int tid = threadIdx.x, lane = tid & 63, wave = tid >> 6;
    const int kp = (nS + RS_THREADS - 1) / RS_THREADS;
    const int nSp = kp * RS_THREADS;
    const int totp = nSp + nC;
    const int kt = (totp + RS_THREADS - 1) / RS_THREADS;
    const size_t sb = (size_t)b * rd.cap;
    double *l1g = rd.blk_l1 + sb;
    LL_T0(t_l1);
    if (!sh.l1_valid) {
        LL_CTX_DECL(sh.ctl.x)
        const int4 *tabG = pt_table_global(rd, b, 0, false);
        const unsigned short *ids = rd.blk_id + (size_t)b * rd.cap_s;
        const float4 *feat = rd.surf_feat + (size_t)b * rd.feat_stride_s;
        const double *av = rd.blk_av + (size_t)b * 6 * rd.cap;
        int k = 0;
        for (int p = tid; p < nS; p += RS_THREADS, k++) {
            if (!act_test(act, k)) continue;
            const float4 ff = gload_f4(feat + p);
            const unsigned int id = gload_u16(ids + p);
            const int4 qb = gload_i4(tabG + 2 * id), qc = gload_i4(tabG + 2 * id + 1);
            const double f[3] = {(double)ff.x, (double)ff.y, (double)ff.z};
            const double v[3] = {__hiloint2double(qb.y, qb.x), __hiloint2double(qb.w, qb.z), __hiloint2double(qc.y, qc.x)};
            const double a[3] = {__hiloint2double(qc.w, qc.z), 0.0, 0.0};
            if (DEBLUR)
                l1g[rd.cap_c + p] = block_l1_mb(BLK_PLANE, mb_, t_, (double)refine_blur(1, ff.w, rc.min_ts, rc.max_ts), f, a, v, rc.huber_a, st->pose_last);
            else
                l1g[rd.cap_c + p] = block_l1(BLK_PLANE, R_, t_, f, a, v, rc.huber_a, st->pose_last);
        }
        k = kp;
        for (int l = tid; l < nC; l += RS_THREADS, k++) {
            if (!act_test(act, k)) continue;
            BlkRegs br;
            load_blk(rd, sb, av, l, br);
            const double a[3] = {br.a0, br.a1, br.a2};
            const double v[3] = {br.v0, br.v1, br.v2};
            double l1;
            LL_CTX_L1(l1, BLK_LINE, br.f, a, v, rc.huber_a, st->pose_last);
            l1g[l] = l1;
        }
    } else if (tid == 0) {
        sh.tcyc[9] += 1;
    }
    __syncthreads();
    LL_TACC(2, t_l1);
    LL_T0(t_dd);

#define LB_KEYS8(V8, K0)                                                                                   \
    {                                                                                                      \
        _Pragma("unroll") for (int u = 0; u < 8; u++)                                                      \
        {                                                                                                  \
            const int j = tid + ((K0) + u) * RS_THREADS;                                                   \
            const int jc = j < totp ? j : 0;                                                               \
            const size_t src = jc < nS ? (size_t)rd.cap_c + jc : (jc >= nSp ? (size_t)(jc - nSp) : (size_t)rd.cap_c); \
            V8[u] = gload_f64(l1g + src);                                                                  \
        }                                                                                                  \
        _Pragma("unroll") for (int u = 0; u < 8; u++) V8[u] = ((K0) + u < kt && act_test(act, (K0) + u)) ? V8[u] : -1.0; \
    }
    auto slot_a = [](unsigned long long key) -> unsigned int {
        unsigned int h = (unsigned int)key * 0x9E3779B1u;
        h ^= h >> 15;
        h += (unsigned int)(key >> 32) * 0x85EBCA77u;
        h ^= h >> 13;
        return h & (DD2_SLOTS - 1);
    };
    auto slot_b = [](unsigned long long key) -> unsigned int {
        unsigned int h2 = ((unsigned int)(key >> 32) * 0xC2B2AE3Du) ^ ((unsigned int)key * 0x27D4EB2Fu);
        return (h2 ^ (h2 >> 16)) & (DD2B_SLOTS - 1);
    };
    unsigned int *bmA = (unsigned int *)s_raw;
    unsigned int *bmB = bmA + DD2_WORDS;
    unsigned long long *dlk = (unsigned long long *)(bmB + DD2B_WORDS);
    int *dlj = (int *)(dlk + DD2_LIST);
    int *bins = dlj + DD2_LIST;
    static_assert((DD2_WORDS + DD2B_WORDS) * 4 + DD2_LIST * 12 + SEL_BINS * 4 <= PT_LDS_BYTES, "tables of the inlier phase fit s_raw");
    {
        uint4 *z = (uint4 *)s_raw;
        for (int e = tid; e < (DD2_WORDS + DD2B_WORDS) / 4; e += RS_THREADS) z[e] = make_uint4(0u, 0u, 0u, 0u);
        for (int e = tid; e < SEL_BINS; e += RS_THREADS) bins[e] = 0;
        if (tid == 0) sh.n_cand = 0;
    }
    __syncthreads();
    LL_T0(t_a);
    Act2 valid = {0ull, 0ull};
    double kmin = INFINITY, kmax = -INFINITY;
    for (int k0 = 0; k0 < kt; k0 += 8) {
        double v8[8];
        LB_KEYS8(v8, k0)
#pragma unroll
        for (int u = 0; u < 8; u++) {
            const double l1 = v8[u];
            const bool ok = l1 >= 0.0;
            const unsigned int slot = slot_a((unsigned long long)__double_as_longlong(l1));
            const unsigned int bit0 = ok ? (1u << ((slot & 15u) * 2u)) : 0u;
            const unsigned int old = atomicOr(&bmA[slot >> 4], bit0);
            atomicOr(&bmA[slot >> 4], (old & bit0) << 1);
            if (ok) {
                act_set(valid, k0 + u);
                kmin = fmin(kmin, l1);
                kmax = fmax(kmax, l1);
            }
        }
    }
    for (int off = 32; off > 0; off >>= 1) {
        kmin = fmin(kmin, __shfl_down(kmin, off));
        kmax = fmax(kmax, __shfl_down(kmax, off));
    }
    if (lane == 0) {
        sh.red[wave][0] = kmin;
        sh.red[wave][1] = kmax;
    }
    __syncthreads();
    double lo = sh.red[0][0], hi = sh.red[0][1];
    for (int w = 1; w < RS_WAVES; w++) {
        lo = fmin(lo, sh.red[w][0]);
        hi = fmax(hi, sh.red[w][1]);
    }
    const double scale = (hi > lo) ? (double)(SEL_BINS - 1) / (hi - lo) : 0.0;
    LL_TACC(10, t_a);
    LL_T0(t_b);
    Act2 cont = {0ull, 0ull};
    for (int k0 = 0; k0 < kt; k0 += 8) {
        double v8[8];
        LB_KEYS8(v8, k0)
#pragma unroll
        for (int u = 0; u < 8; u++) {
            const unsigned long long key = (unsigned long long)__double_as_longlong(v8[u]);
            const unsigned int slot = slot_a(key);
            const bool contested = act_test(valid, k0 + u) && ((bmA[slot >> 4] >> ((slot & 15u) * 2u)) & 2u);
            const unsigned int h2 = slot_b(key);
            const unsigned int bit0 = contested ? (1u << ((h2 & 15u) * 2u)) : 0u;
            const unsigned int old = atomicOr(&bmB[h2 >> 4], bit0);
            atomicOr(&bmB[h2 >> 4], (old & bit0) << 1);
            if (contested) act_set(cont, k0 + u);
        }
    }
    __syncthreads();
    LL_TACC(11, t_b);
    LL_T0(t_c);
    Act2 first = {0ull, 0ull};
    for (int k0 = 0; k0 < kt; k0 += 8) {
// ... 101 lines not shown
            int part = 0;
            for (int e = 0; e < per; e++) part += bins[tid * per + e];
            int incl = part;
#pragma unroll
            for (int off = 1; off < 64; off <<= 1) {
                const int y = __shfl_up(incl, off);
                if (lane >= off) incl += y;
            }
            if (lane == 63) sh.isum[wave] = incl;
            if (tid == 0) sh.n_cand = 0;
            __syncthreads();
            int below = incl - part;
            for (int w = 0; w < wave; w++) below += sh.isum[w];
            const int rank = sh.sel_rank;
            __syncthreads();
            const bool last_thread = tid == RS_THREADS - 1;
            if ((rank >= below && rank < below + part) || (last_thread && rank >= below + part)) {
                int cum = below, bi = tid * per;
                for (; bi < tid * per + per - 1; bi++) {
                    if (cum + bins[bi] > rank) break;
                    cum += bins[bi];
                }
                sh.sel_bin = bi;
                sh.sel_rank = rank - cum;
                sh.sel_cnt = bins[bi];
            }
            __syncthreads();
        }
        const int sel_bin = sh.sel_bin;
        if (sh.sel_cnt <= SEL_CAND) {
            for (int k0 = 0; k0 < kt; k0 += 8) {
                double v8[8];
                LB_KEYS8(v8, k0)
#pragma unroll
                for (int u = 0; u < 8; u++) {
                    if (!act_test(first, k0 + u)) continue;
                    int bi = (int)((v8[u] - lo) * scale);
                    bi = bi < 0 ? 0 : (bi > SEL_BINS - 1 ? SEL_BINS - 1 : bi);
                    if (bi == sel_bin) cand[atomicAdd(&sh.n_cand, 1)] = (unsigned long long)__double_as_longlong(v8[u]);
                }
            }
#pragma unroll
            for (int q = 0; q < 4; q++) {
                if (!((list_first >> q) & 1u)) continue;
                const unsigned long long key = dlk[tid + q * RS_THREADS];
                int bi = (int)((__longlong_as_double((long long)key) - lo) * scale);
                bi = bi < 0 ? 0 : (bi > SEL_BINS - 1 ? SEL_BINS - 1 : bi);
                if (bi == sel_bin) cand[atomicAdd(&sh.n_cand, 1)] = key;
            }
            __syncthreads();
            const int m = sh.n_cand;
            for (int i = tid; i < m; i += RS_THREADS) {
                const unsigned long long ki = cand[i];
                int rk = 0;
                for (int j = 0; j < m; j++) rk += (cand[j] < ki) ? 1 : 0;
                if (rk == sh.sel_rank) sh.sel_prefix = ki;
            }
            __syncthreads();
        } else {
            if (tid == 0) sh.sel_prefix = 0ull;
            __syncthreads();
            for (int pass = 0; pass < 8; pass++) {
                const int shift = 56 - 8 * pass;
                for (int e = tid; e < 256; e += RS_THREADS) sh.hist[e] = 0;
                __syncthreads();
                const unsigned long long prefix = sh.sel_prefix;
                for (int k0 = 0; k0 < kt; k0 += 8) {
                    double v8[8];
                    LB_KEYS8(v8, k0)
#pragma unroll
                    for (int u = 0; u < 8; u++) {
                        if (!act_test(first, k0 + u)) continue;
                        int bi = (int)((v8[u] - lo) * scale);
                        bi = bi < 0 ? 0 : (bi > SEL_BINS - 1 ? SEL_BINS - 1 : bi);
                        if (bi != sel_bin) continue;
                        const unsigned long long key = (unsigned long long)__double_as_longlong(v8[u]);
                        if (pass == 0 || (key >> (shift + 8)) == prefix) atomicAdd(&sh.hist[(int)((key >> shift) & 255ull)], 1);
                    }
                }
#pragma unroll
                for (int q = 0; q < 4; q++) {
                    if (!((list_first >> q) & 1u)) continue;
                    const unsigned long long key = dlk[tid + q * RS_THREADS];
                    int bi = (int)((__longlong_as_double((long long)key) - lo) * scale);
                    bi = bi < 0 ? 0 : (bi > SEL_BINS - 1 ? SEL_BINS - 1 : bi);
                    if (bi == sel_bin && (pass == 0 || (key >> (shift + 8)) == prefix)) atomicAdd(&sh.hist[(int)((key >> shift) & 255ull)], 1);
                }
                __syncthreads();
                if (tid == 0) {
                    int rank = sh.sel_rank, d = 0, cum = 0;
                    for (d = 0; d < 256; d++) {
                        if (cum + sh.hist[d] > rank) break;
                        cum += sh.hist[d];
                    }
                    if (d > 255) d = 255;
                    sh.sel_rank = rank - cum;
                    sh.sel_prefix = (prefix << 8) | (unsigned long long)d;
                }
                __syncthreads();
            }
        }
        if (tid == 0) sh.thr = fmax(rc.inliner_dis, __longlong_as_double((long long)sh.sel_prefix));
    } else {
        if (tid == 0) sh.thr = rc.inliner_dis;
    }
    __syncthreads();
    LL_TACC(4, t_sel);
    LL_T0(t_prune);
    {
        const double thr = sh.thr;
        int na = 0;
        for (int k0 = 0; k0 < kt; k0 += 8) {
            double v8[8];
            LB_KEYS8(v8, k0)
#pragma unroll
            for (int u = 0; u < 8; u++) {
                const int k = k0 + u;
                if (k >= kt || !act_test(act, k)) continue;
                if (v8[u] > thr)
                    act_clear(act, k);
                else
                    na++;
            }
        }
        na = block_sum_int(na, sh);
        if (tid == 0) sh.n_active = na;
        __syncthreads();
    }
    LL_TACC(7, t_prune);
#undef LB_KEYS8
    return act;
}

template <int DEBLUR>
__device__ void solve_big(const RegDev &rd, const RegConst &rc, const f4 *map_pts, int b, RegState *st, SolveShared &sh, uint4 *s_raw)
{
    const int tid = threadIdx.x;
    const int nC = rd.n_corner[b], nS = rd.n_surf[b];
    if (tid < 16) sh.tcyc[tid] = 0;
    __syncthreads();
    LL_T0(t_total);
    Act2 act = big_census_and_plane_table(rd, rc, map_pts, b, st, nC, nS, s_raw, sh);
    big_lm<true, DEBLUR>(rd, rc, b, nC, nS, st->inc, rc.ceres_prerun_times, sh.n_active, act, s_raw, st->pose_last, sh);
    int lm_iters = sh.ctl.iteration;
    act = big_inlier<DEBLUR>(rd, rc, b, st, sh, s_raw, act, nC, nS);
    {
        __shared__ double x_start_b[7];
        if (tid < 7) x_start_b[tid] = sh.ctl.x[tid];
        plane_table_reload(rd, b, false, s_raw, sh);
        big_lm<false, DEBLUR>(rd, rc, b, nC, nS, x_start_b, rc.ceres_max_iterations, sh.n_active, act, s_raw, st->pose_last, sh);
    }
    lm_iters += sh.ctl.iteration;
    solve_epilogue(rc, st, sh, lm_iters);
#ifdef LL_SOLVE_TIMING
    LL_TACC(5, t_total);
    if (tid == 0)
        for (int i = 0; i < 16; i++) st->dbg_cycles[i] += sh.tcyc[i];
#endif
}

template <int DEBLUR>
__global__ __launch_bounds__(RS_THREADS) void reg_solve_big_kernel(RegDev rd, RegConst rc, const f4 *map_surf)
{
    __shared__ SolveShared sh;
    __shared__ uint4 s_raw[PT_LDS_BYTES / 16];
    static_assert(PT_LDS_BYTES >= HT_SIZE * 8, "s_raw holds the general path's tables");
    const int b = blockIdx.x;
    RegState *st = rd.state + b;
    if (st->done) return;
    if (threadIdx.x == 0) {
        sh.grp_g = 0;
        sh.grp_G = 1;
        sh.grp_seq = 0;
        sh.xch_seq = 0;
        sh.xch_epoch = rc.xch_epoch;
        sh.grp_abort = 0;
    }
    __syncthreads();
    if (scan_is_compact(rd, rc, b))
        solve_big<DEBLUR>(rd, rc, map_surf, b, st, sh, s_raw);
    else
        solve_general<DEBLUR>(rd, rc, b, st, sh, (unsigned long long *)s_raw);
}

}
```

### loam_livox_amd/csrc/ll_reg_small_kernels.hip

```cpp
#include <hip/hip_runtime.h>

#include "ll_reg_query.h"
#include "ll_reg_solve_common.h"

namespace ll {

#define LL_CTX_DECL_SMALL(x)                                   \
    double R_[9], t_[3];                                        \
    {                                                           \
        const double q_[4] = {(x)[0], (x)[1], (x)[2], (x)[3]};  \
        quat_to_mat(q_, R_);                                    \
        t_[0] = (x)[4];                                         \
        t_[1] = (x)[5];                                         \
        t_[2] = (x)[6];                                         \
    }

#ifdef LL_SOLVE_TIMING
#define SM_T0(var) long long var = clock64()
#define SM_TACC(slot, var)                                      \
    do {                                                        \
        if (threadIdx.x == 0) sh.tcyc[slot] += clock64() - var; \
    } while (0)
#else
#define SM_T0(var)
// ... 10 lines not shown
    double x_start[7];
    int need, n_active, n_corner_avail, n_surf_avail;
    int nL, nA;
    int n_eval;
    int cnt[16][8];
    int isum[8];
    unsigned long long lsum[8];
    int hist[256];
    int sel_digit, sel_rank;
};

struct SmallArgs {
    RegState *state;
    const int *n_corner, *n_surf;
    const int *order;
    const unsigned char *blk_flag0;
    const float4 *blk_f;
    const double *blk_av;
    const int4 *nn;
    const float4 *surf_feat;
    const f4 *map_surf;
    int cap_all, cap_c, feat_stride_s;
    int cap, capl;
};

struct SmallBlocks {
    LL_AS_LDS double *v0, *v1, *v2, *a0, *a1, *a2;
    LL_AS_LDS float *fx, *fy, *fz;
};

template <int W>
__device__ __forceinline__ unsigned long long small_sum_u64(unsigned long long v, SmallShared &sh)
{
    const int tid = threadIdx.x, lane = tid & 63, wave = tid >> 6;
#pragma unroll
    for (int off = 32; off > 0; off >>= 1) v += (unsigned long long)__shfl_xor((long long)v, off);
    if (W == 1) return v;
    if (lane == 0) sh.lsum[wave] = v;
    __syncthreads();
    unsigned long long s = 0;
#pragma unroll
    for (int w = 0; w < W; w++) s += sh.lsum[w];
    __syncthreads();
    return s;
}

__device__ __forceinline__ void cx_local(unsigned long long &a, unsigned long long &b, bool up)
{
    const bool sw = (b < a) == up;
    const unsigned long long lo = sw ? b : a, hi = sw ? a : b;
    a = lo;
    b = hi;
}

template <int K>
__device__ __forceinline__ void wave_bitonic_sort(unsigned long long (&key)[K], int lane)
{
    static_assert(K == 1 || K == 2 || K == 4 || K == 8 || K == 16, "keys per lane: a power of two");
    constexpr int N = 64 * K;
#pragma unroll
    for (int k = 2; k <= N; k <<= 1) {
#pragma unroll
        for (int j = k >> 1; j >= 1; j >>= 1) {
            if (j >= K) {
                const int lj = j / K;
                const bool lower = (lane & lj) == 0;
#pragma unroll
                for (int r = 0; r < K; r++) {
                    const int g = lane * K + r;
                    const bool up = (g & k) == 0;
                    const unsigned long long mine = key[r];
                    const unsigned long long other = (unsigned long long)__shfl_xor((long long)mine, lj);
                    const bool keep_min = lower == up;
                    const bool take = (other < mine) == keep_min;
                    key[r] = take ? other : mine;
                }
            } else {
#pragma unroll
                for (int r = 0; r < K; r++) {
                    if ((r & j) == 0) {
                        const int g = lane * K + r;
                        const bool up = (g & k) == 0;
                        cx_local(key[r], key[r | j], up);
                    }
                }
            }
        }
    }
}

template <int W>
__device__ __forceinline__ void small_eval(const SmallBlocks &B, const double *x, double huber_a, unsigned int act, int nL, int nA, SmallShared &sh)
{
    constexpr int DEBLUR = 0;
    constexpr int NT = 64 * W;
    const int tid = threadIdx.x, lane = tid & 63, wave = tid >> 6;
    LL_CTX_DECL_SMALL(x)
    double acc[LL_NACC];
#pragma unroll
    for (int i = 0; i < LL_NACC; i++) acc[i] = 0.0;
    if (nA > 0) {
        int idx = tid < nA ? tid : nA - 1;
        float nfx = B.fx[idx], nfy = B.fy[idx], nfz = B.fz[idx];
        double nv0 = B.v0[idx], nv1 = B.v1[idx], nv2 = B.v2[idx], na0 = B.a0[idx];
        int il = idx < nL ? idx : 0;
        double na1 = B.a1[il], na2 = B.a2[il];
        for (int r = 0; r * NT < nA; r++) {
            const int cur = r * NT + tid;
            const double f[3] = {(double)nfx, (double)nfy, (double)nfz};
            const double v[3] = {nv0, nv1, nv2};
            const double a[3] = {na0, na1, na2};
            {
                const int nx = cur + NT;
                idx = nx < nA ? nx : nA - 1;
                nfx = B.fx[idx], nfy = B.fy[idx], nfz = B.fz[idx];
                nv0 = B.v0[idx], nv1 = B.v1[idx], nv2 = B.v2[idx], na0 = B.a0[idx];
                il = idx < nL ? idx : 0;
                na1 = B.a1[il], na2 = B.a2[il];
            }
            if (cur < nA && ((act >> r) & 1u)) {
                if (cur < nL) {
                    block_accumulate(BLK_LINE, R_, t_, f, a, v, huber_a, acc);
                } else {
                    const double ap[3] = {a[0], 0.0, 0.0};
                    block_accumulate(BLK_PLANE, R_, t_, f, ap, v, huber_a, acc);
                }
            }
        }
    }
    wave_sum_acc(acc, sh.red[wave], lane);
    __syncthreads();
    if (tid < LL_NACC) {
        double s = sh.red[0][tid];
#pragma unroll
        for (int w = 1; w < W; w++) s += sh.red[w][tid];
        sh.sum[tid] = s;
    }
    __syncthreads();
}

template <int W>
__device__ __forceinline__ void small_lm(const SmallBlocks &B, const RegConst &rc, const double *x0, int max_iter, unsigned int act, SmallShared &sh)
{
    const int tid = threadIdx.x;
    if (tid == 0) lm_begin(sh.ctl, x0, max_iter, rc.bound);
    __syncthreads();
    {
        SM_T0(t0);
        small_eval<W>(B, sh.ctl.x, rc.huber_a, act, sh.nL, sh.nA, sh);
        SM_TACC(0, t0);
    }
    {
        SM_T0(t1);
        if (tid == 0) sh.need = lm_init(sh.ctl, sh.sum, sh.n_active);
        __syncthreads();
        SM_TACC(1, t1);
    }
    while (sh.need) {
        SM_T0(t0);
        small_eval<W>(B, sh.ctl.cand, rc.huber_a, act, sh.nL, sh.nA, sh);
        SM_TACC(0, t0);
        SM_T0(t1);
        if (tid < 64) {
            const int need = lm_update_wave(sh.ctl, sh.sum, sh.fit, tid);
            if (tid == 0) {
                sh.need = need;
                sh.n_eval++;
            }
        }
        __syncthreads();
        SM_TACC(1, t1);
#ifdef LL_SOLVE_TIMING
        if (tid == 0) sh.tcyc[9] += 1;
#endif
    }
}

#define LL_SMALL_KERNEL reg_solve_small_kernel
#define LL_SMALL_MORE_ARGS
#define LL_SMALL_BIND_MAP
#include "ll_reg_small_solve.h"
#undef LL_SMALL_KERNEL
#undef LL_SMALL_MORE_ARGS
#undef LL_SMALL_BIND_MAP

#define LL_SMALL_KERNEL reg_solve_small_maps_kernel
#define LL_SMALL_MORE_ARGS , const Grid *map_tab, int cls
#define LL_SMALL_BIND_MAP                                                         \
    if (reg_maps_class(rc, rd.n_corner[b], rd.n_surf[b], 0x7fffffff) != cls) return;  \
    map_surf = map_tab[2 * b + 1].pts;
#include "ll_reg_small_solve.h"
#undef LL_SMALL_KERNEL
#undef LL_SMALL_MORE_ARGS
#undef LL_SMALL_BIND_MAP

#define SO_THREADS 1024
#define SO_BINS 256
__global__ __launch_bounds__(SO_THREADS) void reg_solve_order_kernel(const RegState *state, int n_scans, int *order)
{
    __shared__ int hist[SO_BINS], start[SO_BINS];
    const int tid = threadIdx.x;
    for (int e = tid; e < SO_BINS; e += SO_THREADS) hist[e] = 0;
    __syncthreads();
    for (int b = tid; b < n_scans; b += SO_THREADS) {
        int w = state[b].last_work;
        w = w < 0 ? 0 : (w > SO_BINS - 1 ? SO_BINS - 1 : w);
        atomicAdd(&hist[SO_BINS - 1 - w], 1);
    }
    __syncthreads();
    if (tid == 0) {
        int run = 0;
        for (int e = 0; e < SO_BINS; e++) {
            start[e] = run;
            run += hist[e];
        }
    }
    __syncthreads();
    for (int b = tid; b < n_scans; b += SO_THREADS) {
        int w = state[b].last_work;
        w = w < 0 ? 0 : (w > SO_BINS - 1 ? SO_BINS - 1 : w);
        order[atomicAdd(&start[SO_BINS - 1 - w], 1)] = b;
    }
}

static size_t small_lds_bytes(int W, int M, int cap, int capl)
{
    const int keys = M * 64 * W;
    const int ns = W <= 2 ? 0 : (keys <= 256 ? 256 : (keys <= 512 ? 512 : (keys <= 1024 ? 1024 : 2048)));
    return (size_t)cap * (4 * 8 + 3 * 4) + (size_t)capl * 16 + (size_t)ns * 16;
}

template <int W, int M, bool MAPS>
static void launch_small(const SmallArgs &a, const RegConst &rc, const Grid *map_tab, int maps_cls, int n_scans, hipStream_t s)
{
    const size_t lds = small_lds_bytes(W, M, a.cap, a.capl);
    const void *fn = MAPS ? (const void *)reg_solve_small_maps_kernel<W, M> : (const void *)reg_solve_small_kernel<W, M>;
    static bool attr_set = false;
    if (!attr_set) {
        hipFuncAttributes fa;
        int room = 160 * 1024 - 8 * 1024;
        if (hipFuncGetAttributes(&fa, fn) == hipSuccess) room = 160 * 1024 - (int)fa.sharedSizeBytes;
        if (hipFuncSetAttribute(fn, hipFuncAttributeMaxDynamicSharedMemorySize, room) != hipSuccess)
            (void)hipGetLastError();
        attr_set = true;
    }
    if (MAPS)
        hipLaunchKernelGGL((reg_solve_small_maps_kernel<W, M>), dim3(n_scans), dim3(64 * W), lds, s, a, rc, map_tab, maps_cls);
    else
        hipLaunchKernelGGL((reg_solve_small_kernel<W, M>), dim3(n_scans), dim3(64 * W), lds, s, a, rc);
}

bool reg_solve_small_eligible(const RegConst &rc, int max_nc, int max_ns)
{
    return !rc.if_motion_deblur && !rc.force_general && !rc.no_small_solver && max_nc + max_ns > 0 &&
           max_nc + max_ns <= LL_SMALL_MAX_BLOCKS && max_nc <= 1024;
}

int reg_solve_small_waves(const RegConst &rc, int n_scans, int max_nc, int max_ns)
{
    const int total = max_nc + max_ns;
    if (total > 1024) return 8;
    if (rc.small_waves) return rc.small_waves;
    if (n_scans < LL_SMALL_W1_MIN_SCANS) return 4;
    const int cap = (total + 63) / 64 * 64, capl = (max_nc + 63) / 64 * 64 + 64;
    const size_t per_scan = small_lds_bytes(1, 1, cap, capl) + sizeof(SmallShared) + 512;
    const int per_cu = (int)((size_t)(160 * 1024) / per_scan);
    return per_cu >= 8 ? 1 : (per_cu >= 4 ? 2 : 4);
}

template <bool MAPS>
static void launch_reg_solve_small_any(const RegDev &rd, const RegConst &rc, const f4 *map_surf, const Grid *map_tab, int maps_cls, int n_scans, int max_nc, int max_ns, int iter, hipStream_t s)
{
    const int total = max_nc + max_ns;
    SmallArgs a;
    a.state = rd.state, a.n_corner = rd.n_corner, a.n_surf = rd.n_surf, a.blk_flag0 = rd.blk_flag0, a.blk_f = rd.blk_f, a.blk_av = rd.blk_av;
    a.nn = rd.nn, a.surf_feat = rd.surf_feat, a.map_surf = map_surf, a.cap_all = rd.cap, a.cap_c = rd.cap_c, a.feat_stride_s = rd.feat_stride_s;
    a.cap = (total + 63) / 64 * 64, a.capl = (max_nc + 63) / 64 * 64 + 64;
    const int W = reg_solve_small_waves(rc, MAPS ? 1 : n_scans, max_nc, max_ns);
    a.order = nullptr;
    if (rd.solve_order && !rc.no_solve_order && n_scans >= LL_SMALL_ORDER_MIN_SCANS && n_scans <= LL_SMALL_ORDER_MAX_SCANS && iter > 0) {
        hipLaunchKernelGGL(reg_solve_order_kernel, dim3(1), dim3(SO_THREADS), 0, s, rd.state, n_scans, rd.solve_order);
        a.order = rd.solve_order;
    }
    const int cls = total <= 256 ? 0 : (total <= 512 ? 1 : 2);
    if (W == 1) {
        if (cls == 0) launch_small<1, 4, MAPS>(a, rc, map_tab, maps_cls, n_scans, s);
        else if (cls == 1) launch_small<1, 8, MAPS>(a, rc, map_tab, maps_cls, n_scans, s);
        else launch_small<1, 16, MAPS>(a, rc, map_tab, maps_cls, n_scans, s);
    } else if (W == 2) {
        if (cls == 0) launch_small<2, 2, MAPS>(a, rc, map_tab, maps_cls, n_scans, s);
        else if (cls == 1) launch_small<2, 4, MAPS>(a, rc, map_tab, maps_cls, n_scans, s);
        else launch_small<2, 8, MAPS>(a, rc, map_tab, maps_cls, n_scans, s);
    } else if (W == 4) {
        if (cls == 0) launch_small<4, 1, MAPS>(a, rc, map_tab, maps_cls, n_scans, s);
        else if (cls == 1) launch_small<4, 2, MAPS>(a, rc, map_tab, maps_cls, n_scans, s);
        else launch_small<4, 4, MAPS>(a, rc, map_tab, maps_cls, n_scans, s);
    } else {
        launch_small<8, 4, MAPS>(a, rc, map_tab, maps_cls, n_scans, s);
    }
}
void launch_reg_solve_small(const RegDev &rd, const RegConst &rc, const Grid &gs, int n_scans, int max_nc, int max_ns, int iter, hipStream_t s)
{
    launch_reg_solve_small_any<false>(rd, rc, gs.pts, nullptr, 0, n_scans, max_nc, max_ns, iter, s);
}
void launch_reg_solve_small_maps(const RegDev &rd, const RegConst &rc, const Grid *map_tab, int n_scans, int cls, int max_nc, int max_ns, int iter, hipStream_t s)
{
    launch_reg_solve_small_any<true>(rd, rc, nullptr, map_tab, cls, n_scans, max_nc, max_ns, iter, s);
}

}
```

### loam_livox_amd/csrc/ll_reg_small_solve.h

```cpp
template <int W, int M>
__global__ __launch_bounds__(64 * W) __attribute__((amdgpu_waves_per_eu(W == 4 ? 1 : 2, 8)))
void LL_SMALL_KERNEL(SmallArgs rd, RegConst rc LL_SMALL_MORE_ARGS)
{
    const int cap = rd.cap, capl = rd.capl;
    const f4 *map_surf = rd.map_surf;
    constexpr int NT = 64 * W;
    constexpr int K = W <= 2 ? M * W : 1;
    constexpr int NS = W <= 2 ? 1 : (M * NT <= 256 ? 256 : (M * NT <= 512 ? 512 : (M * NT <= 1024 ? 1024 : 2048)));
    static_assert(M <= 16 && K <= 16 && M * NT <= 2048, "census rounds / sort keys per lane / LDS sort size");
    __shared__ SmallShared sh;
    extern __shared__ double s_dyn[];
    const int tid = threadIdx.x, lane = tid & 63, wave = tid >> 6;
    const int b = rd.order ? rd.order[blockIdx.x] : (int)blockIdx.x;
    RegState *st = rd.state + b;
    if (st->done) return;
    LL_SMALL_BIND_MAP
    SmallBlocks B;
    {
        LL_AS_LDS double *p = (LL_AS_LDS double *)s_dyn;
        B.v0 = p, B.v1 = p + cap, B.v2 = p + 2 * cap, B.a0 = p + 3 * cap;
        B.a1 = p + 4 * cap, B.a2 = p + 4 * cap + capl;
        LL_AS_LDS float *q = (LL_AS_LDS float *)(p + 4 * cap + 2 * capl + (W >= 4 ? 2 * NS : 0));
        B.fx = q, B.fy = q + cap, B.fz = q + 2 * cap;
    }
    const int nC = rd.n_corner[b], nS = rd.n_surf[b];
    const int ncand = nC + nS;
    if (ncand > NT * M) {
        if (tid == 0) {
            st->aborted = 1;
            st->done = 1;
            st->icp_iters += 1;
        }
        return;
    }
    const size_t sb = (size_t)b * rd.cap_all;
    const unsigned char *flag0 = rd.blk_flag0 + sb;
#ifdef LL_SOLVE_TIMING
    if (tid < 16) sh.tcyc[tid] = 0;
    __syncthreads();
#endif
    SM_T0(t_total);
    SM_T0(t_census);

    unsigned int act = 0;
    int na = 0, nca = 0, nsa = 0;
#pragma unroll
    for (int r = 0; r < M; r++) {
        const int c = r * NT + tid;
        const int cc = c < ncand ? c : 0;
        const size_t slot = cc < nC ? (size_t)cc : (size_t)rd.cap_c + (cc - nC);
        const unsigned char fl = (c < ncand) ? gload_u8(flag0 + slot) : (unsigned char)0;
        if (fl & BLK_ACTIVE) {
            act |= 1u << r;
            na++;
        }
        if (fl & 8) {
            if (c < nC) nca++; else nsa++;
        }
    }
    {
        const unsigned long long tot = small_sum_u64<W>((unsigned long long)na | ((unsigned long long)nca << 20) | ((unsigned long long)nsa << 40), sh);
        na = (int)(tot & 0xfffffull);
        nca = (int)((tot >> 20) & 0xfffffull);
        nsa = (int)((tot >> 40) & 0xfffffull);
    }
    if (rc.subsample_seed && na > rc.max_blocks) {
#pragma unroll
        for (int r = 0; r < M; r++) {
            if (!((act >> r) & 1u)) continue;
            if (subsample_drop_block(rc.subsample_seed, st->icp_iters, r * NT + tid, na, rc.max_blocks)) act &= ~(1u << r);
        }
    }
    int pos[M];
    {
        int mine[M];
#pragma unroll
        for (int r = 0; r < M; r++) {
            const unsigned long long bal = __ballot((act >> r) & 1u);
            mine[r] = __popcll(bal & ((1ull << lane) - 1ull));
            if (lane == 0) sh.cnt[r][wave] = __popcll(bal);
        }
        __syncthreads();
        int base = 0, kept_lines = 0;
#pragma unroll
        for (int r = 0; r < M; r++) {
            int before = 0, round_total = 0;
#pragma unroll
            for (int w = 0; w < W; w++) {
                const int c = sh.cnt[r][w];
                if (w < wave) before += c;
                round_total += c;
            }
            pos[r] = base + before + mine[r];
            base += round_total;
        }
        {
            int kl = 0;
#pragma unroll
            for (int r = 0; r < M; r++)
                if (((act >> r) & 1u) && r * NT + tid < nC) kl++;
            kept_lines = (int)small_sum_u64<W>((unsigned long long)kl, sh);
        }
        if (tid == 0) {
            sh.n_eval = 0;
            sh.n_active = base;
            sh.nA = base;
            sh.nL = kept_lines;
            sh.n_corner_avail = nca;
            sh.n_surf_avail = nsa;
        }
    }
    SM_TACC(6, t_census);
    SM_T0(t_build);
    {
        double pose_last[7];
#pragma unroll
        for (int i = 0; i < 7; i++) pose_last[i] = gload_f64(st->pose_last + i);
        const double *av = rd.blk_av + (size_t)b * 6 * rd.cap_all;
        const float4 *sfeat = rd.surf_feat + (size_t)b * rd.feat_stride_s;
#pragma unroll
        for (int r = 0; r < M; r++) {
            const int c = r * NT + tid;
            if (!((act >> r) & 1u)) continue;
            const int p = pos[r];
            if (c < nC) {
                const float4 f = gload_f4(rd.blk_f + sb + c);
                double a0, a1, a2, v0, v1, v2;
                av_load(av, rd.cap_all, c, true, a0, a1, a2, v0, v1, v2);
                B.fx[p] = f.x, B.fy[p] = f.y, B.fz[p] = f.z;
                B.v0[p] = v0, B.v1[p] = v1, B.v2[p] = v2;
                B.a0[p] = a0, B.a1[p] = a1, B.a2[p] = a2;
            } else {
                const int q = c - nC;
                const int4 t = gload_i4(rd.nn + sb + rd.cap_c + q);
                const f4 m0 = gload_pt(map_surf + (unsigned int)t.x), m1 = gload_pt(map_surf + (unsigned int)t.y), m2 = gload_pt(map_surf + (unsigned int)t.z);
                float fx, fy, fz;
                gload_f3(sfeat + q, fx, fy, fz);
                const double pa[3] = {(double)m0.x, (double)m0.y, (double)m0.z};
                const double pb[3] = {(double)m1.x, (double)m1.y, (double)m1.z};
                const double pc[3] = {(double)m2.x, (double)m2.y, (double)m2.z};
                double a_out[3] = {0.0, 0.0, 0.0}, v_out[3] = {0.0, 0.0, 0.0};
                (void)block_plane(pose_last, pa, pb, pc, a_out, v_out);
                B.fx[p] = fx, B.fy[p] = fy, B.fz[p] = fz;
                B.v0[p] = v_out[0], B.v1[p] = v_out[1], B.v2[p] = v_out[2];
                B.a0[p] = a_out[0];
            }
        }
    }
    __syncthreads();
    SM_TACC(8, t_build);
    const int nA = sh.nA, nL = sh.nL;
    unsigned int live = 0;
#pragma unroll
    for (int r = 0; r < M; r++)
        if (r * NT + tid < nA) live |= 1u << r;

    small_lm<W>(B, rc, st->inc, rc.ceres_prerun_times, live, sh);
    int lm_iters = sh.ctl.iteration;

    double l1[M];
    SM_T0(t_l1);
    {
        constexpr int DEBLUR = 0;
        LL_CTX_DECL_SMALL(sh.ctl.x)
        double q_last[4];
#pragma unroll
        for (int i = 0; i < 4; i++) q_last[i] = gload_f64(st->pose_last + i);
#pragma unroll
        for (int r = 0; r < M; r++) {
            const int idx = r * NT + tid;
            double v1 = -1.0;
            if ((live >> r) & 1u) {
                const double f[3] = {(double)B.fx[idx], (double)B.fy[idx], (double)B.fz[idx]};
                const double v[3] = {B.v0[idx], B.v1[idx], B.v2[idx]};
                if (idx < nL) {
                    const double a[3] = {B.a0[idx], B.a1[idx], B.a2[idx]};
                    v1 = block_l1(BLK_LINE, R_, t_, f, a, v, rc.huber_a, q_last);
                } else {
                    const double a[3] = {B.a0[idx], 0.0, 0.0};
                    v1 = block_l1(BLK_PLANE, R_, t_, f, a, v, rc.huber_a, q_last);
                }
            }
            l1[r] = v1;
        }
    }
    SM_TACC(2, t_l1);
    SM_T0(t_sort);
    if (W <= 2) {
        unsigned long long key[K];
#pragma unroll
// ... 4 lines not shown
        if (W > 1) {
            unsigned long long *xch = (unsigned long long *)&sh.red[0][0];
            static_assert(sizeof(sh.red) >= 64 * sizeof(unsigned long long), "exchange buffer");
#pragma unroll
            for (int w = 1; w < (W <= 2 ? W : 1); w++) {
#pragma unroll
                for (int r = 0; r < M; r++) {
                    if (wave == w) xch[lane] = key[r];
                    __syncthreads();
                    if (wave == 0) key[(w * M + r) < K ? (w * M + r) : 0] = xch[lane];
                    __syncthreads();
                }
            }
        }
        if (wave == 0) {
            wave_bitonic_sort<K>(key, lane);
            const unsigned long long prev_last = (unsigned long long)__shfl_up((long long)key[K - 1], 1);
            unsigned int first = 0;
#pragma unroll
            for (int k = 0; k < K; k++) {
                const unsigned long long pv = k == 0 ? prev_last : key[k - 1];
                const bool valid = key[k] != 0xffffffffffffffffull;
                if (valid && ((k == 0 && lane == 0) || key[k] != pv)) first |= 1u << k;
            }
            const int cnt = __popc(first);
            int incl = cnt;
#pragma unroll
            for (int off = 1; off < 64; off <<= 1) {
                const int y = __shfl_up(incl, off);
                if (lane >= off) incl += y;
            }
            const int nu = __shfl(incl, 63);
            int target = (int)(rc.inlier_ratio * (double)nu);
            if (target > nu - 1) target = nu - 1;
            if (nu == 0) {
                if (lane == 0) sh.thr = rc.inliner_dis;
            } else if (target >= incl - cnt && target < incl) {
                int rk = incl - cnt;
                unsigned long long sel = 0;
#pragma unroll
                for (int k = 0; k < K; k++) {
                    if ((first >> k) & 1u) {
                        if (rk == target) sel = key[k];
                        rk++;
                    }
                }
                sh.thr = fmax(rc.inliner_dis, __longlong_as_double((long long)sel));
            }
        }
    } else {
        LL_AS_LDS unsigned long long *tab = (LL_AS_LDS unsigned long long *)(B.a2 + capl);
        constexpr unsigned int TS = 2u * NS;
        for (int e = tid; e < (int)TS; e += NT) tab[e] = 0xffffffffffffffffull;
        __syncthreads();
        unsigned int uniq = 0;
#pragma unroll
        for (int r = 0; r < M; r++) {
            const double v = l1[r];
            if (!(v >= 0.0)) continue;
            const unsigned long long key = (unsigned long long)__double_as_longlong(v);
            unsigned int hsh = (unsigned int)key * 0x9E3779B1u;
            hsh ^= hsh >> 15;
            hsh += (unsigned int)(key >> 32) * 0x85EBCA77u;
            hsh ^= hsh >> 13;
            unsigned int slot = hsh & (TS - 1u);
            for (;;) {
                const unsigned long long old = atomicCAS((unsigned long long *)&tab[slot], 0xffffffffffffffffull, key);
                if (old == 0xffffffffffffffffull) {
                    uniq |= 1u << r;
                    break;
                }
                if (old == key) break;
                slot = (slot + 1u) & (TS - 1u);
            }
        }
        const int nu = (int)small_sum_u64<W>((unsigned long long)__popc(uniq), sh);
        int target = (int)(rc.inlier_ratio * (double)nu);
        if (target > nu - 1) target = nu - 1;
        if (nu == 0) {
            if (tid == 0) sh.thr = rc.inliner_dis;
        } else {
            unsigned long long prefix = 0ull;
            int rank = target;
            for (int pass = 0; pass < 8; pass++) {
                const int shift = 56 - 8 * pass;
                if (tid < 256) sh.hist[tid] = 0;
                __syncthreads();
#pragma unroll
                for (int r = 0; r < M; r++) {
                    if (!((uniq >> r) & 1u)) continue;
                    const unsigned long long key = (unsigned long long)__double_as_longlong(l1[r]);
                    if (pass == 0 || (key >> (shift + 8)) == prefix) atomicAdd(&sh.hist[(int)((key >> shift) & 255ull)], 1);
                }
                __syncthreads();
                if (wave == 0) {
                    const int b0 = sh.hist[4 * lane], b1 = sh.hist[4 * lane + 1], b2 = sh.hist[4 * lane + 2], b3 = sh.hist[4 * lane + 3];
                    const int part = b0 + b1 + b2 + b3;
                    int incl = part;
#pragma unroll
                    for (int off = 1; off < 64; off <<= 1) {
                        const int y = __shfl_up(incl, off);
                        if (lane >= off) incl += y;
                    }
                    const int below = incl - part;
                    if (rank >= below && rank < incl) {
                        int d = 4 * lane, cum = below;
                        if (cum + b0 <= rank) {
                            cum += b0;
                            d++;
                            if (cum + b1 <= rank) {
                                cum += b1;
                                d++;
                                if (cum + b2 <= rank) {
                                    cum += b2;
                                    d++;
                                }
                            }
                        }
                        sh.sel_digit = d;
                        sh.sel_rank = rank - cum;
                    }
                }
                __syncthreads();
                prefix = (prefix << 8) | (unsigned long long)sh.sel_digit;
                rank = sh.sel_rank;
            }
            if (tid == 0) sh.thr = fmax(rc.inliner_dis, __longlong_as_double((long long)prefix));
        }
    }
    __syncthreads();
    SM_TACC(3, t_sort);
    SM_T0(t_prune);
    {
        const double thr = sh.thr;
        int keep = 0;
#pragma unroll
        for (int r = 0; r < M; r++) {
            if (!((live >> r) & 1u)) continue;
            if (l1[r] > thr)
                live &= ~(1u << r);
            else
                keep++;
        }
        keep = (int)small_sum_u64<W>((unsigned long long)keep, sh);
        if (tid == 0) sh.n_active = keep;
        if (tid < 7) sh.x_start[tid] = sh.ctl.x[tid];
        __syncthreads();
    }
    SM_TACC(7, t_prune);
    small_lm<W>(B, rc, sh.x_start, rc.ceres_max_iterations, live, sh);
    lm_iters += sh.ctl.iteration;
    solve_epilogue(rc, st, sh, lm_iters);
    if (tid == 0) st->last_work = sh.n_eval;
#ifdef LL_SOLVE_TIMING
    SM_TACC(5, t_total);
    if (tid == 0)
        for (int i = 0; i < 16; i++) st->dbg_cycles[i] += sh.tcyc[i];
#endif
}
```

### loam_livox_amd/csrc/ll_reg_solve_common.h

```cpp
#pragma once
#include <hip/hip_runtime.h>

#include "ll_reg_query.h"

namespace ll {

__device__ __forceinline__ void wave_sum_acc(const double (&acc)[LL_NACC], double *red, int lane)
{
    static_assert(LL_NACC <= 32 && LL_NACC > 16, "butterfly over 32 value slots");
    const bool b5 = (lane & 32) != 0, b4 = (lane & 16) != 0, b3 = (lane & 8) != 0, b2 = (lane & 4) != 0, b1 = (lane & 2) != 0;
    double w16[16], w8[8], w4[4], w2[2];
#pragma unroll
    for (int i = 0; i < 16; i++) {
        const double hi = (16 + i < LL_NACC) ? acc[16 + i] : 0.0;
        const double keep = b5 ? hi : acc[i], send = b5 ? acc[i] : hi;
        w16[i] = keep + __shfl_xor(send, 32);
    }
#pragma unroll
    for (int i = 0; i < 8; i++) {
        const double keep = b4 ? w16[8 + i] : w16[i], send = b4 ? w16[i] : w16[8 + i];
        w8[i] = keep + __shfl_xor(send, 16);
    }
#pragma unroll
    for (int i = 0; i < 4; i++) {
        const double keep = b3 ? w8[4 + i] : w8[i], send = b3 ? w8[i] : w8[4 + i];
        w4[i] = keep + __shfl_xor(send, 8);
    }
#pragma unroll
    for (int i = 0; i < 2; i++) {
        const double keep = b2 ? w4[2 + i] : w4[i], send = b2 ? w4[i] : w4[2 + i];
        w2[i] = keep + __shfl_xor(send, 4);
    }
    const double keep1 = b1 ? w2[1] : w2[0], send1 = b1 ? w2[0] : w2[1];
    const double w1 = keep1 + __shfl_xor(send1, 2);
    const double tot = w1 + __shfl_xor(w1, 1);
    const int idx = (lane >> 1) & 31;
    if (!(lane & 1) && idx < LL_NACC) red[idx] = tot;
}

__device__ inline void compute_interp(const double q[4], RegState *st)
{
    double n = sqrt(q[0] * q[0] + q[1] * q[1] + q[2] * q[2]);
    double axis[3];
    if (q[3] < 0) n = -n;
    if (n != 0.0) {
        st->interp_theta = 2.0 * atan2(n, fabs(q[3]));
        axis[0] = q[0] / n;
        axis[1] = q[1] / n;
        axis[2] = q[2] / n;
    } else {
        st->interp_theta = 0.0;
        axis[0] = 1.0;
        axis[1] = 0.0;
        axis[2] = 0.0;
    }
    const double an = sqrt(dot3(axis, axis));
    axis[0] /= an;
    axis[1] /= an;
    axis[2] /= an;
    for (int i = 0; i < 9; i++) st->hat[i] = 0.0;
    st->hat[1] = -axis[2];
    st->hat[3] = axis[2];
    st->hat[2] = axis[1];
    st->hat[6] = -axis[1];
    st->hat[5] = -axis[0];
    st->hat[7] = axis[0];
    for (int i = 0; i < 3; i++)
        for (int j = 0; j < 3; j++) {
            double s = 0;
            for (int k = 0; k < 3; k++) s += st->hat[i * 3 + k] * st->hat[k * 3 + j];
            st->hat_sq[i * 3 + j] = s;
        }
}

template <class SH>
__device__ void solve_epilogue(const RegConst &rc, RegState *st, SH &sh, int lm_iters)
{
    const int tid = threadIdx.x;
    if (tid == 0) {
        for (int i = 0; i < 7; i++) st->inc[i] = sh.ctl.x[i];
        if (rc.if_motion_deblur) compute_interp(st->inc, st);
        double tw[3];
        quat_rot(st->pose_last, &st->inc[4], tw);
        st->pose_curr[4] = tw[0] + st->pose_last[4];
        st->pose_curr[5] = tw[1] + st->pose_last[5];
        st->pose_curr[6] = tw[2] + st->pose_last[6];
        double qc[4];
        quat_mul(st->pose_last, st->inc, qc);
        for (int i = 0; i < 4; i++) st->pose_curr[i] = qc[i];
        st->angular_diff = (double)((float)quat_angular_distance(qc, st->pose_last)) * 57.3;
        const double dt[3] = {st->pose_curr[4] - st->pose_last[4], st->pose_curr[5] - st->pose_last[5],
                              st->pose_curr[6] - st->pose_last[6]};
        st->t_diff = sqrt(dot3(dt, dt));
        st->final_cost = sh.ctl.final_cost;
        st->initial_cost = sh.ctl.initial_cost;
        st->inlier_thr = sh.thr;
        st->n_blocks_last = sh.n_active;
        st->corner_avail = sh.n_corner_avail;
        st->surf_avail = sh.n_surf_avail;
        st->lm_total += lm_iters;
        st->icp_iters += 1;
        const double dto[3] = {st->prev_t[0] - st->inc[4], st->prev_t[1] - st->inc[5], st->prev_t[2] - st->inc[6]};
        const bool conv = quat_angular_distance(st->prev_q, st->inc) < 57.3 * rc.minimum_icp_R_diff &&
                          sqrt(dot3(dto, dto)) < rc.minimum_icp_T_diff;
        if (conv && !rc.force_all_iterations) {
            st->done = 1;
        } else {
            for (int i = 0; i < 4; i++) st->prev_q[i] = st->inc[i];
            for (int i = 0; i < 3; i++) st->prev_t[i] = st->inc[4 + i];
        }
        if (st->icp_iters >= rc.icp_max_iterations) st->done = 1;
    }
}

__device__ __forceinline__ double lm_quintic_min_step_wave(double f0, double g0, double x1, double f1, double g1, double x2, double f2, double g2,
                                                           double lo, double hi, int lane)
{
    Quintic q;
    if (!quintic_fit(f0, g0, x1, f1, g1, x2, f2, g2, q)) return fmin(fmax(0.5 * x1, lo), hi);
    QuinticChain c;
    quintic_chain(q, c);
    double r3[2] = {hi, hi};
    const int n3 = quintic_quadratic_roots(c.A, c.B, c.C, lo, hi, r3);
    const double P1 = n3 >= 1 ? r3[0] : hi, P2 = n3 >= 2 ? r3[1] : hi;
    double R0, R1, R2;
    int n2;
    {
        const double a = lane == 0 ? lo : (lane == 1 ? P1 : P2), b = lane == 0 ? P1 : (lane == 1 ? P2 : hi);
        double root = 0.0;
        const bool has = lane <= n3 && lane < 3 && quintic_interval_root(c.d2, a, b, quintic_poly4(c.d2, a), quintic_poly4(c.d2, b), &root);
        const int h0 = __shfl((int)has, 0), h1 = __shfl((int)has, 1), h2 = __shfl((int)has, 2);
        const double y0 = __shfl(root, 0), y1 = __shfl(root, 1), y2 = __shfl(root, 2);
        n2 = h0 + h1 + h2;
        R0 = h0 ? y0 : (h1 ? y1 : y2);
        R1 = (h0 && h1) ? y1 : y2;
        R2 = y2;
        const double last = n2 == 3 ? R2 : (n2 == 2 ? R1 : R0);
        if (n2 > 0 && !(last < hi)) n2--;
    }
    const double Q1 = n2 >= 1 ? R0 : hi, Q2 = n2 >= 2 ? R1 : hi, Q3 = n2 >= 3 ? R2 : hi;
    const double a = lane == 0 ? lo : (lane == 1 ? Q1 : (lane == 2 ? Q2 : Q3)), b = lane == 0 ? Q1 : (lane == 1 ? Q2 : (lane == 2 ? Q3 : hi));
    double root = 0.0;
    const bool has = lane <= n2 && lane < 4 && quintic_interval_root(c.dq, a, b, quintic_poly4(c.dq, a), quintic_poly4(c.dq, b), &root);
    const double xe = lane == 4 ? lo : (lane == 5 ? hi : root);
    double ve, de;
    quintic_eval(q, xe, ve, de);
    (void)de;
    double best_x = lo, best_v = __shfl(ve, 4);
    const double vh = __shfl(ve, 5);
    if (!(best_v < vh)) {
        best_v = vh;
        best_x = hi;
    }
#pragma unroll
    for (int i = 0; i < 4; i++) {
        const int hi_ = __shfl((int)has, i);
        const double xi = __shfl(root, i), v = __shfl(ve, i);
        if (hi_ && v < best_v) {
            best_v = v;
            best_x = xi;
        }
    }
    return best_x;
}

__device__ __forceinline__ double lm_quintic_min_step_wave_call(const double *a, int lane)
{
    return lm_quintic_min_step_wave(a[0], a[1], a[2], a[3], a[4], a[5], a[6], a[7], a[8], a[9], lane);
}

__device__ __forceinline__ int lm_update_wave(LmCtl &c, const double *sum, double *fit, int lane)
{
    int code = 0;
    double e[LL_NACC];
    if (lane == 0) {
#pragma unroll
        for (int i = 0; i < LL_NACC; i++) e[i] = sum[i];
        double cur_cost = 0.0, cg = 0.0;
        code = lm_update_pre(c, e, &cur_cost, &cg);
        if (code == LM_FIT) {
            fit[0] = c.cost, fit[1] = c.gd, fit[2] = c.ls_step, fit[3] = cur_cost, fit[4] = cg, fit[5] = c.ls_prev_x, fit[6] = c.ls_prev_f, fit[7] = c.ls_prev_g;
            fit[8] = 1e-3 * c.ls_step, fit[9] = 0.6 * c.ls_step;
        }
    }
    if (__shfl(code, 0) == LM_FIT) {
        __builtin_amdgcn_fence(__ATOMIC_RELEASE, "wavefront");
        __builtin_amdgcn_wave_barrier();
        __builtin_amdgcn_fence(__ATOMIC_ACQUIRE, "wavefront");
        const double step = lm_quintic_min_step_wave_call(fit, lane);
        if (lane == 0) code = lm_update_post(c, fit[3], fit[4], step);
    }
    int r = 0;
    if (lane == 0) r = lm_update_close(c, e, code);
    return r;
}

}
```

### loam_livox_amd/csrc/ll_reg_solve_fast.h

```cpp
#pragma once
#include <hip/hip_runtime.h>

#include "ll_reg_query.h"
#include "ll_reg_solve_common.h"

namespace ll {

#define RS_WAVES (RS_THREADS / 64)

#define LL_CTX_DECL(x)                                   \
    double R_[9], t_[3];                                  \
    MbRot mb_;                                            \
    {                                                     \
        const double q_[4] = {(x)[0], (x)[1], (x)[2], (x)[3]}; \
        quat_to_mat(q_, R_);                              \
        t_[0] = (x)[4];                                   \
        t_[1] = (x)[5];                                   \
        t_[2] = (x)[6];                                   \
        if (DEBLUR) mb_prepare(q_, mb_);                  \
    }
#define LL_CTX_ACCUM(kind, ff, a, v, huber_a, acc)                                                        \
    do {                                                                                                  \
        const double f_[3] = {(double)(ff).x, (double)(ff).y, (double)(ff).z};                            \
        if (DEBLUR)                                                                                       \
// ... 908 lines not shown
            if (L1OUT) gstore_f64(l1_planes + pp_, plane_l1_scaled(R_, t_, f, v, beta_, huber_a, q_last)); \
        }                                                                                                  \
    }
#define LL3_PIPE(FROM_CACHE, KB, KE)                                   \
    {                                                                  \
        constexpr bool FROM_CACHE_ = FROM_CACHE;                       \
        const int KB_ = (KB), KE_ = (KE);                              \
        if (KB_ < KE_) {                                               \
            Rec3 r0, r1, r2, r3, r4;                                   \
            Pl3 q0, q1, q2, q3, q4;                                    \
            LL3_LOAD(r0, KB_)                                          \
            LL3_LOAD(r1, KB_ + 1)                                      \
            LL3_LOAD(r2, KB_ + 2)                                      \
            LL3_LOAD(r3, KB_ + 3)                                      \
            LL3_PLANE(q0, r0)                                          \
            for (int k = KB_; k < KE_; k += 5) {                       \
                LL3_LOAD(r4, k + 4)                                    \
                LL3_PLANE(q1, r1)                                      \
                LL3_USE(r0, q0, k)                                     \
                LL3_LOAD(r0, k + 5)                                    \
                LL3_PLANE(q2, r2)                                      \
                LL3_USE(r1, q1, k + 1)                                 \
                LL3_LOAD(r1, k + 6)                                    \
                LL3_PLANE(q3, r3)                                      \
                LL3_USE(r2, q2, k + 2)                                 \
                LL3_LOAD(r2, k + 7)                                    \
                LL3_PLANE(q4, r4)                                      \
                LL3_USE(r3, q3, k + 3)                                 \
                LL3_LOAD(r3, k + 8)                                    \
                LL3_PLANE(q0, r0)                                      \
                LL3_USE(r4, q4, k + 4)                                 \
            }                                                          \
        }                                                              \
    }

template <bool FILL, bool L1OUT, bool GROUPED>
__device__ __noinline__ void solver_eval3(const RegDev &rd, int b, int nC, int nS, const double *x, double huber_a, unsigned long long act,
                                          uint4 *s_raw, const double *q_last_g, SolveShared &sh)
{
    constexpr int DEBLUR = 0;
    const int tid = threadIdx.x, lane = tid & 63, wave = tid >> 6;
    double q_last[4] = {0.0, 0.0, 0.0, 1.0};
    if (L1OUT) {
        q_last[0] = q_last_g[0];
        q_last[1] = q_last_g[1];
        q_last[2] = q_last_g[2];
        q_last[3] = q_last_g[3];
    }
    double *l1_planes = rd.blk_l1 + (size_t)b * rd.cap + rd.cap_c;
    double *l1_lines = rd.blk_l1 + (size_t)b * rd.cap;
    LL_CTX_DECL(x)
    double acc[LL_NACC];
#pragma unroll
    for (int i = 0; i < LL_NACC; i++) acc[i] = 0.0;
    constexpr int G = GROUPED ? LL_GRP : 1, GS = G * RS_THREADS;
    const int g = GROUPED ? sh.grp_g : 0;
    const int p0 = g * RS_THREADS + tid;
    const int Tl = sh.pt_Tl, kc = sh.pt_kc;
    const int kp = (nS + GS - 1) / GS;
    const int4 *tabL = (const int4 *)s_raw;
    int4 *cache = (int4 *)s_raw + 2 * Tl;
    const int4 *tabG = pt_table_global(rd, b, g, GROUPED);
    const unsigned short *ids = rd.blk_id + (size_t)b * rd.cap_s;
    const float4 *feat = rd.surf_feat + (size_t)b * rd.feat_stride_s;
    if (sh.pt_T <= PT_TCAP) {
        constexpr bool TAB_LDS = true;
        if (!FILL) LL3_PIPE(true, 0, kc)
        LL3_PIPE(false, FILL ? 0 : kc, kp)
    } else {
        constexpr bool TAB_LDS = false;
        if (!FILL) LL3_PIPE(true, 0, kc)
        LL3_PIPE(false, FILL ? 0 : kc, kp)
    }
    plane_unfold2(acc);
    {
        const size_t sb = (size_t)b * rd.cap;
        const double *av = rd.blk_av + (size_t)b * 6 * rd.cap;
        const int kpl = (nS + RS_THREADS - 1) / RS_THREADS;
        const int nl = sh.pt_nl;
        int4 *lc = (int4 *)s_raw + (PT_LDS_BYTES / 16 - 4 * nl);
        int k = 0;
        for (int l = p0; l < nC; l += GS, k++) {
            if (!((act >> (kpl + g + G * k)) & 1ull)) continue;
            BlkRegs br;
            const int j = GROUPED ? (k == 0 ? tid : nl) : l;
            if (!FILL && j < nl) {
                const int4 c0 = lds_load_i4(lc + j), c1 = lds_load_i4(lc + nl + j), c2 = lds_load_i4(lc + 2 * nl + j), c3 = lds_load_i4(lc + 3 * nl + j);
                br.f = make_float4(__int_as_float(c0.x), __int_as_float(c0.y), __int_as_float(c0.z), __int_as_float(c0.w));
                br.a0 = __hiloint2double(c1.y, c1.x);
                br.v0 = __hiloint2double(c1.w, c1.z);
                br.v1 = __hiloint2double(c2.y, c2.x);
                br.v2 = __hiloint2double(c2.w, c2.z);
                br.a1 = __hiloint2double(c3.y, c3.x);
                br.a2 = __hiloint2double(c3.w, c3.z);
            } else {
                load_blk(rd, sb, av, l, br);
                if (FILL && j < nl) {
                    lds_store_i4(lc + j, make_int4(__float_as_int(br.f.x), __float_as_int(br.f.y), __float_as_int(br.f.z), __float_as_int(br.f.w)));
                    lds_store_i4(lc + nl + j, make_int4(__double2loint(br.a0), __double2hiint(br.a0), __double2loint(br.v0), __double2hiint(br.v0)));
                    lds_store_i4(lc + 2 * nl + j, make_int4(__double2loint(br.v1), __double2hiint(br.v1), __double2loint(br.v2), __double2hiint(br.v2)));
                    lds_store_i4(lc + 3 * nl + j, make_int4(__double2loint(br.a1), __double2hiint(br.a1), __double2loint(br.a2), __double2hiint(br.a2)));
                }
            }
            const double a[3] = {br.a0, br.a1, br.a2};
            const double v[3] = {br.v0, br.v1, br.v2};
            LL_CTX_ACCUM(BLK_LINE, br.f, a, v, huber_a, acc);
            if (L1OUT) {
                double l1;
                LL_CTX_L1(l1, BLK_LINE, br.f, a, v, huber_a, q_last);
                l1_lines[l] = l1;
            }
        }
    }
    if (__ballot(act != 0ull) != 0ull) {
        wave_sum_acc(acc, sh.red[wave], lane);
    } else if (lane < LL_NACC) {
        sh.red[wave][lane] = 0.0;
    }
    __syncthreads();
    if (tid < LL_NACC) {
        double s = 0.0;
        for (int w = 0; w < RS_WAVES; w++) s += sh.red[w][tid];
        sh.sum[tid] = s;
    }
    __syncthreads();
    if (GROUPED) {
        LL_T0(t_grp);
        group_reduce<L1OUT>(rd, b, sh);
        LL_TACC(9, t_grp);
    }
}
#undef LL3_LOAD
#undef LL3_PLANE
#undef LL3_USE
#undef LL3_PIPE

template <bool WANT_L1, bool GROUPED>
__device__ __forceinline__ void solver_lm3(const RegDev &rd, const RegConst &rc, int b, int nC, int nS, const double *x0, int max_iter,
                                           int n_active, unsigned long long act, uint4 *s_raw, const double *q_last, SolveShared &sh)
{
    const int tid = threadIdx.x;
    if (tid == 0) {
        lm_begin(sh.ctl, x0, max_iter, rc.bound);
        sh.l1_valid = 0;
    }
    __syncthreads();
    {
        LL_T0(t0);
        solver_eval3<true, false, GROUPED>(rd, b, nC, nS, sh.ctl.x, rc.huber_a, act, s_raw, q_last, sh);
        LL_TACC(0, t0);
    }
    {
        LL_T0(t1);
        if (tid == 0) sh.need = lm_init(sh.ctl, sh.sum, n_active);
        __syncthreads();
        LL_TACC(1, t1);
    }
    while (sh.need) {
        const bool spec = WANT_L1 && sh.ctl.iteration >= max_iter;
        LL_T0(t0);
        if (spec)
            solver_eval3<false, true, GROUPED>(rd, b, nC, nS, sh.ctl.cand, rc.huber_a, act, s_raw, q_last, sh);
        else
            solver_eval3<false, false, GROUPED>(rd, b, nC, nS, sh.ctl.cand, rc.huber_a, act, s_raw, q_last, sh);
        LL_TACC(0, t0);
        LL_T0(t1);
        if (tid < 64) {
            const int need = lm_update_wave(sh.ctl, sh.sum, sh.fit, tid);
            if (tid == 0) {
                sh.need = need;
                sh.l1_valid = (spec && !need && sh.ctl.last_accept == 1) ? 1 : 0;
            }
        }
        __syncthreads();
        LL_TACC(1, t1);
    }
}

template <int NK, bool GROUPED>
__device__ __noinline__ unsigned long long inlier_phase3(const RegDev &rd, const RegConst &rc, int b, RegState *st, SolveShared &sh, uint4 *s_raw,
                                                         unsigned long long act, int nC, int nS)
{
    constexpr int DEBLUR = 0;
    const int tid = threadIdx.x;
    const int nSp = (nS + RS_THREADS - 1) / RS_THREADS * RS_THREADS;
    const int totp = nSp + nC;
    const size_t sb = (size_t)b * rd.cap;
    LL_T0(t_l1);
    double *l1g = rd.blk_l1 + sb;
    if (!sh.l1_valid) {
        LL_CTX_DECL(sh.ctl.x)
        constexpr int G = GROUPED ? LL_GRP : 1, GS = G * RS_THREADS;
        const int g = GROUPED ? sh.grp_g : 0;
        const int p0 = g * RS_THREADS + tid;
        const int4 *tabG = pt_table_global(rd, b, g, GROUPED);
        const unsigned short *ids = rd.blk_id + (size_t)b * rd.cap_s;
        const float4 *feat = rd.surf_feat + (size_t)b * rd.feat_stride_s;
        const double *av = rd.blk_av + (size_t)b * 6 * rd.cap;
        int k = 0;
        for (int p = p0; p < nS; p += GS, k++) {
            if (!((act >> (g + G * k)) & 1ull)) continue;
            const float4 ff = gload_f4(feat + p);
            const unsigned int id = gload_u16(ids + p);
            const int4 qb = gload_i4(tabG + 2 * id), qc = gload_i4(tabG + 2 * id + 1);
            const double f[3] = {(double)ff.x, (double)ff.y, (double)ff.z};
            const double v[3] = {__hiloint2double(qb.y, qb.x), __hiloint2double(qb.w, qb.z), __hiloint2double(qc.y, qc.x)};
            l1g[rd.cap_c + p] = plane_l1_scaled(R_, t_, f, v, __hiloint2double(qc.w, qc.z), rc.huber_a, st->pose_last);
        }
        const int kpl = nSp / RS_THREADS;
        k = 0;
        for (int l = p0; l < nC; l += GS, k++) {
            if (!((act >> (kpl + g + G * k)) & 1ull)) continue;
            BlkRegs br;
            load_blk(rd, sb, av, l, br);
            const double a[3] = {br.a0, br.a1, br.a2};
            const double v[3] = {br.v0, br.v1, br.v2};
            double l1;
            LL_CTX_L1(l1, BLK_LINE, br.f, a, v, rc.huber_a, st->pose_last);
            l1g[l] = l1;
        }
        if (GROUPED)
            group_barrier<true>(rd, b, sh);
        else
            __syncthreads();
    } else if (tid == 0) {
        sh.tcyc[9] += 1;
    }
    double l1r[NK];
    {
        const int kt = (totp + RS_THREADS - 1) / RS_THREADS;
#pragma unroll
        for (int k = 0; k < NK; k++) {
            const int j = tid + k * RS_THREADS;
            double v = -1.0;
            if (k < kt) {
                const int jc = j < totp ? j : 0;
                const size_t src = jc < nS ? (size_t)rd.cap_c + jc : (jc >= nSp ? (size_t)(jc - nSp) : (size_t)rd.cap_c);
                v = gload_f64(l1g + src);
            }
            l1r[k] = v;
        }
#pragma unroll
        for (int k = 0; k < NK; k++) l1r[k] = ((act >> k) & 1ull) ? l1r[k] : -1.0;
    }
    __syncthreads();
    LL_TACC(2, t_l1);

    inlier_threshold_regs<NK>(l1r, totp, (unsigned long long *)s_raw, sh, rc);

    LL_T0(t_prune);
    {
        const double thr = sh.thr;
        int na = 0;
#pragma unroll
        for (int k = 0; k < NK; k++) {
            if (!((act >> k) & 1ull)) continue;
            if (l1r[k] > thr)
                act &= ~(1ull << k);
            else
                na++;
        }
        na = block_sum_int(na, sh);
        if (tid == 0) sh.n_active = na;
        __syncthreads();
    }
    LL_TACC(7, t_prune);
    return act;
}

template <bool GROUPED>
__device__ void solve_fast3(const RegDev &rd, const RegConst &rc, const f4 *map_pts, int b, RegState *st, SolveShared &sh, uint4 *s_raw)
{
    constexpr int DEBLUR = 0;
    const int tid = threadIdx.x;
    const int nC = rd.n_corner[b], nS = rd.n_surf[b];
    const int nSp = (nS + RS_THREADS - 1) / RS_THREADS * RS_THREADS;
    const int totp = nSp + nC;
    const size_t sb = (size_t)b * rd.cap;
    if (tid < 16) sh.tcyc[tid] = 0;
    __syncthreads();
    LL_T0(t_total);

    unsigned long long act = census_and_plane_table<GROUPED>(rd, rc, map_pts, b, st, nC, nS, s_raw, sh);

    solver_lm3<true, GROUPED>(rd, rc, b, nC, nS, st->inc, rc.ceres_prerun_times, sh.n_active, act, s_raw, st->pose_last, sh);
    int lm_iters = sh.ctl.iteration;

    if (totp <= 36 * RS_THREADS)
        act = inlier_phase3<36, GROUPED>(rd, rc, b, st, sh, s_raw, act, nC, nS);
    else
        act = inlier_phase3<FAST_MAXK, GROUPED>(rd, rc, b, st, sh, s_raw, act, nC, nS);

    {
        __shared__ double x_start_3[7];
        if (tid < 7) x_start_3[tid] = sh.ctl.x[tid];
        plane_table_reload(rd, b, GROUPED, s_raw, sh);
        solver_lm3<false, GROUPED>(rd, rc, b, nC, nS, x_start_3, rc.ceres_max_iterations, sh.n_active, act, s_raw, st->pose_last, sh);
    }
    lm_iters += sh.ctl.iteration;
    if (GROUPED) {
        group_barrier<false>(rd, b, sh);
        if (sh.grp_g != 0) return;
        if (sh.grp_abort) {
            if (tid == 0) {
                st->aborted = 1;
                st->done = 1;
                st->icp_iters += 1;
            }
            return;
        }
    }
    solve_epilogue(rc, st, sh, lm_iters);
#ifdef LL_SOLVE_TIMING
    LL_TACC(5, t_total);
    if (tid == 0)
        for (int i = 0; i < 16; i++) st->dbg_cycles[i] += sh.tcyc[i];
#endif
}

struct SolveTicket {
    int b, g, G;
};
__device__ __forceinline__ SolveTicket solve_fast_ticket(const RegDev &rd, const RegConst &rc, SolveShared &sh)
{
    SolveTicket t = {(int)blockIdx.x, 0, 1};
    if (rc.solve_group > 1) {
        if (threadIdx.x == 0) sh.grp_seq = atomicAdd(rd.grp_ctl, 1);
        __syncthreads();
        t.G = rc.solve_group;
        t.b = sh.grp_seq / t.G;
        t.g = sh.grp_seq - t.b * t.G;
        __syncthreads();
    }
    return t;
}
__device__ __forceinline__ bool solve_fast_check(const RegDev &rd, const RegConst &rc, int b, int g, int nC, int nS, RegState *st)
{
    if (padded_block_count(nC, nS) > FAST_MAX_BLOCKS || !scan_is_compact(rd, rc, b)) {
        if (g == 0 && threadIdx.x == 0) {
            st->aborted = 1;
            st->done = 1;
            st->icp_iters += 1;
        }
        return false;
    }
    return true;
}
__device__ __forceinline__ void solve_fast_group_fields(const RegConst &rc, int g, int G, SolveShared &sh)
{
    if (threadIdx.x == 0) {
        sh.grp_g = g;
        sh.grp_G = G;
        sh.grp_seq = 0;
        sh.xch_seq = 0;
        sh.xch_epoch = rc.xch_epoch;
        sh.grp_abort = (rc.test_group_abort && G > 1) ? 1 : 0;
    }
    __syncthreads();
}

}
```

Before: 52700 scans/s.

## Run LM init/update trust-region step across a full wavefront instead of lane 0

Adds a wavefront-parallel Levenberg-Marquardt controller (lmw_init/lmw_update), where the 6x6 Cholesky solve, the step and the state-plus candidates are spread across 64 lanes using readlane broadcasts. The solver paths now use it by default in place of the serial lane-0 lm_init/lm_update, which is meant to shorten the serial critical section between evaluation passes. It also adds a lane-0 comparison build, a debug entry point that checks the two controllers match, and forceinlines solve_fast3. The cost is more register pressure and more code size, and the numerics must match the serial path exactly.

```diff
diff --git a/__graft_entry__.py b/__graft_entry__.py
--- a/__graft_entry__.py
+++ b/__graft_entry__.py
@@ -10,6 +10,7 @@
     from loam_livox_amd import build as b
     lib = b.build()
     assert os.path.exists(lib)
+    assert os.path.exists(b.build_lm_lane0())
     from oracle import orc
     orc.build()
     from tests.hostcheck import hc
diff --git a/include/loam_livox_hip.h b/include/loam_livox_hip.h
--- a/include/loam_livox_hip.h
+++ b/include/loam_livox_hip.h
@@ -151,6 +151,9 @@
                    int32_t *results);
 
 int ll_debug_quintic(int32_t device, const double *args10, int32_t n, double *out_sequential, double *out_wavefront);
+
+int ll_debug_lm_sequence(int32_t device, const double *hdr12, const double *evals28, int32_t n, int32_t max_calls, void *out_lane0,
+                         void *out_wavefront, int32_t *ret_lane0, int32_t *ret_wavefront, int32_t *ctl_bytes);
 
 int ll_reg_debug_knn(ll_reg *r, int32_t scan, int32_t *corner_idx5, float *corner_d25, int32_t *surf_idx5,
                      float *surf_d25);
diff --git a/loam_livox_amd/build.py b/loam_livox_amd/build.py
--- a/loam_livox_amd/build.py
+++ b/loam_livox_amd/build.py
@@ -9,7 +9,7 @@
 CSRC = os.path.join(HERE, "csrc")
 LIB = os.environ.get("LL_LIB_OUT") or os.path.join(HERE, "libloamlivox_hip.so")
 SOURCES = ["ll_api_common.hip", "ll_api_fe.hip", "ll_api_map.hip", "ll_api_reg.hip", "ll_api_voxel.hip", "ll_api_cellmap.hip", "ll_api_scene_align.hip", "ll_api_keyframe_bank.hip", "ll_api_pose_graph.hip", "ll_api_history.hip", "ll_api_history_batch_buffer.hip", "ll_api_history_batch_stores.hip", "ll_api_history_batch_extract.hip", "ll_api_history_batch_cells.hip", "ll_fe_kernels.hip", "ll_map_kernels.hip", "ll_reg_query_kernels.hip", "ll_reg_solve_kernels.hip", "ll_reg_maps_kernels.hip", "ll_reg_aux_kernels.hip", "ll_reg_small_kernels.hip", "ll_knn_kernels.hip", "ll_voxel_kernels.hip", "ll_cellmap_kernels.hip", "ll_cellmap_extract_kernels.hip", "ll_cellmap_select_kernels.hip", "ll_spin_kernels.hip", "ll_spin_api.hip", "ll_history_batch_kernels.hip", "ll_cellmap_batch_kernels.hip", "ll_cellmap_batch_extract_kernels.hip", "ll_cellmatch_batch_kernels.hip", "ll_fullmap_batch_kernels.hip", "ll_keyframe_bank_kernels.hip", "ll_pose_graph_kernels.hip"]
-HEADERS = ["ll_api_internal.h", "ll_api_history_batch_internal.h", "ll_device.h", "ll_fe_core.h", "ll_knn_core.h", "ll_knn_coop.h", "ll_knn_tile.h", "ll_reg_query.h", "ll_reg_solve_fast.h", "ll_reg_big_path.h", "ll_reg_solve_general.h", "ll_reg_solve_common.h", "ll_reg_small_solve.h", "ll_reg_core.h", "ll_voxel.h", "ll_voxel_core.h", "ll_cellmap.h", "ll_cellmap_core.h", "ll_cellmap_select_core.h", "ll_spin.h", "ll_spin_core.h", "ll_history_batch.h", "ll_cellmap_batch.h", "ll_cellmap_batch_core.h", "ll_cellmap_batch_extract_core.h", "ll_cellmatch_batch.h", "ll_cellmatch_batch_core.h", "ll_fullmap_batch.h", "ll_fullmap_batch_core.h", "ll_keyframe_bank.h", "ll_keyframe_bank_core.h", "ll_pose_graph.h", "ll_pose_graph_core.h", "../../include/loam_livox_hip.h"]
+HEADERS = ["ll_api_internal.h", "ll_api_history_batch_internal.h", "ll_device.h", "ll_fe_core.h", "ll_knn_core.h", "ll_knn_coop.h", "ll_knn_tile.h", "ll_reg_query.h", "ll_reg_solve_fast.h", "ll_reg_big_path.h", "ll_reg_solve_general.h", "ll_reg_solve_common.h", "ll_lm_wave.h", "ll_reg_small_solve.h", "ll_reg_core.h", "ll_voxel.h", "ll_voxel_core.h", "ll_cellmap.h", "ll_cellmap_core.h", "ll_cellmap_select_core.h", "ll_spin.h", "ll_spin_core.h", "ll_history_batch.h", "ll_cellmap_batch.h", "ll_cellmap_batch_core.h", "ll_cellmap_batch_extract_core.h", "ll_cellmatch_batch.h", "ll_cellmatch_batch_core.h", "ll_fullmap_batch.h", "ll_fullmap_batch_core.h", "ll_keyframe_bank.h", "ll_keyframe_bank_core.h", "ll_pose_graph.h", "ll_pose_graph_core.h", "../../include/loam_livox_hip.h"]
 FLAGS = ["--offload-arch=gfx950", "-O3", "-std=c++17", "-fPIC", "-ffp-contract=off", "-Wno-unused-result"]
 FLAGS += os.environ.get("LL_EXTRA_HIPCC_FLAGS", "").split()
 
@@ -57,5 +57,33 @@
     return lib
 
 
+LM_LANE0_LIB = os.path.join(HERE, "libloamlivox_hip_lm_lane0.so")
+LM_LANE0_SOURCES = ["ll_reg_solve_kernels.hip", "ll_reg_maps_kernels.hip", "ll_reg_small_kernels.hip"]
+
+
+def build_lm_lane0(force: bool = False) -> str:
+    build()
+    if not force and not needs_build(LM_LANE0_LIB) and os.path.getmtime(LM_LANE0_LIB) >= os.path.getmtime(LIB):
+        return LM_LANE0_LIB
+    flags = ["-DLL_LM_LANE0", "-DLL_LM_COUNTS"]
+    shared = [os.path.join(HERE, "build", s.replace(".hip", ".o")) for s in SOURCES if s not in LM_LANE0_SOURCES]
+    if not all(os.path.exists(o) for o in shared):
+        return build(force=True, lib=LM_LANE0_LIB, extra_flags=flags)
+    cc = hipcc()
+    objdir = os.path.join(HERE, "build_lm_lane0")
+    os.makedirs(objdir, exist_ok=True)
+    procs = []
+    for src in LM_LANE0_SOURCES:
+        obj = os.path.join(objdir, src.replace(".hip", ".o"))
+        procs.append((src, obj, subprocess.Popen([cc] + FLAGS + flags + ["-c", os.path.join(CSRC, src), "-o", obj], stdout=subprocess.PIPE,
+                                                 stderr=subprocess.STDOUT)))
+    for src, _, p in procs:
+        out, _ = p.communicate()
+        if p.returncode != 0:
+            raise RuntimeError(f"hipcc failed on {src}:\n{out.decode()}")
+    subprocess.check_call([cc, "--offload-arch=gfx950", "-shared", "-fPIC", "-o", LM_LANE0_LIB] + shared + [o for _, o, _ in procs])
+    return LM_LANE0_LIB
+
+
 if __name__ == "__main__":
     print(build(force="--force" in sys.argv, verbose=True))
diff --git a/loam_livox_amd/capi.py b/loam_livox_amd/capi.py
--- a/loam_livox_amd/capi.py
+++ b/loam_livox_amd/capi.py
@@ -194,6 +194,7 @@
     "ll_history_cell_map": (_vp, [_vp, _i32]),
     "ll_history_refresh_cells": (_i32, [_vp, _vp, _vp, C.c_float, C.c_float, C.c_float, _i32, _vp, _vp]),
     "ll_debug_quintic": (_i32, [_i32, _vp, _i32, _vp, _vp]),
+    "ll_debug_lm_sequence": (_i32, [_i32, _vp, _vp, _i32, _i32, _vp, _vp, _vp, _vp, _vp]),
     "ll_spin_default_params": (None, [C.POINTER(SpinParams)]),
     "ll_spin_create": (_i32, [C.POINTER(SpinParams), C.POINTER(_vp)]),
     "ll_spin_destroy": (None, [_vp]),
diff --git a/loam_livox_amd/csrc/ll_api_reg.hip b/loam_livox_amd/csrc/ll_api_reg.hip
--- a/loam_livox_amd/csrc/ll_api_reg.hip
+++ b/loam_livox_amd/csrc/ll_api_reg.hip
@@ -462,6 +462,47 @@
     return rc ? set_err("ll_debug_quintic", "device error") : 0;
 }
 
+extern "C" int ll_debug_lm_sequence(int32_t device, const double *hdr12, const double *evals28, int32_t n, int32_t max_calls, void *out_lane0,
+                                    void *out_wavefront, int32_t *ret_lane0, int32_t *ret_wavefront, int32_t *ctl_bytes)
+{
+    if (!ctl_bytes || n < 0 || max_calls < 0) return set_err("ll_debug_lm_sequence", "bad argument");
+    *ctl_bytes = debug_lm_ctl_bytes();
+    if (n == 0 || max_calls == 0) return 0;
+    if (!hdr12 || !evals28 || !out_lane0 || !out_wavefront || !ret_lane0 || !ret_wavefront) return set_err("ll_debug_lm_sequence", "bad argument");
+    if (check_device(device)) return -1;
+    const size_t slots = (size_t)n * (size_t)max_calls, img = slots * (size_t)*ctl_bytes;
+    double *d_h = nullptr, *d_e = nullptr;
+    unsigned int *d_s = nullptr, *d_w = nullptr;
+    int *d_rs = nullptr, *d_rw = nullptr;
+    HC(hipMalloc((void **)&d_h, (size_t)n * 12 * sizeof(double)));
+    HC(hipMalloc((void **)&d_e, slots * 28 * sizeof(double)));
+    HC(hipMalloc((void **)&d_s, img));
+    HC(hipMalloc((void **)&d_w, img));
+    HC(hipMalloc((void **)&d_rs, slots * sizeof(int)));
+    HC(hipMalloc((void **)&d_rw, slots * sizeof(int)));
+    int rc = 0;
+    if (hipMemcpy(d_h, hdr12, (size_t)n * 12 * sizeof(double), hipMemcpyHostToDevice) != hipSuccess ||
+        hipMemcpy(d_e, evals28, slots * 28 * sizeof(double), hipMemcpyHostToDevice) != hipSuccess || hipMemset(d_s, 0, img) != hipSuccess ||
+        hipMemset(d_w, 0, img) != hipSuccess || hipMemset(d_rs, 0xff, slots * sizeof(int)) != hipSuccess ||
+        hipMemset(d_rw, 0xff, slots * sizeof(int)) != hipSuccess)
+        rc = -1;
+    if (!rc) {
+        launch_debug_lm_sequence(d_h, d_e, n, max_calls, d_s, d_w, d_rs, d_rw, nullptr);
+        if (hipDeviceSynchronize() != hipSuccess || hipMemcpy(out_lane0, d_s, img, hipMemcpyDeviceToHost) != hipSuccess ||
+            hipMemcpy(out_wavefront, d_w, img, hipMemcpyDeviceToHost) != hipSuccess ||
+            hipMemcpy(ret_lane0, d_rs, slots * sizeof(int), hipMemcpyDeviceToHost) != hipSuccess ||
+            hipMemcpy(ret_wavefront, d_rw, slots * sizeof(int), hipMemcpyDeviceToHost) != hipSuccess)
+            rc = -1;
+    }
+    (void)hipFree(d_h);
+    (void)hipFree(d_e);
+    (void)hipFree(d_s);
+    (void)hipFree(d_w);
+    (void)hipFree(d_rs);
+    (void)hipFree(d_rw);
+    return rc ? set_err("ll_debug_lm_sequence", "device error") : 0;
+}
+
 extern "C" int ll_reg_debug_cycles(ll_reg *r, int32_t scan, long long out[16])
 {
     if (!r || scan < 0 || scan >= r->max_scans) return set_err("ll_reg_debug_cycles", "bad argument");
diff --git a/loam_livox_amd/csrc/ll_device.h b/loam_livox_amd/csrc/ll_device.h
--- a/loam_livox_amd/csrc/ll_device.h
+++ b/loam_livox_amd/csrc/ll_device.h
@@ -167,6 +167,9 @@
 #define LL_QSORT_CORNER_MAX 2048
 void launch_reg_qsort(const RegDev &rd, const RegConst &rc, const Grid &gc, const Grid &gs, int n_scans, int max_nc, int max_ns, bool fused, hipStream_t s);
 void launch_debug_quintic(const double *args, int n, double *out_seq, double *out_wave, hipStream_t s);
+void launch_debug_lm_sequence(const double *hdr, const double *evals, int n, int max_calls, unsigned int *img_seq, unsigned int *img_wave, int *ret_seq,
+                              int *ret_wave, hipStream_t s);
+int debug_lm_ctl_bytes();
 void launch_reg_knn_tile(const RegDev &rd, const RegConst &rc, const Grid &gc, const Grid &gs, int n_scans, int iter, int max_nc, int max_ns,
                          bool fused, hipStream_t s);
 void launch_reg_solve(const RegDev &rd, const RegConst &rc, const Grid &gs, int n_scans, int max_nc, int max_ns, int iter, hipStream_t s);
diff --git a/loam_livox_amd/csrc/ll_lm_wave.h b/loam_livox_amd/csrc/ll_lm_wave.h
--- /dev/null
+++ b/loam_livox_amd/csrc/ll_lm_wave.h
@@ -0,0 +1,401 @@
+#pragma once
+#include "ll_reg_core.h"
+
+#if defined(__HIP_DEVICE_COMPILE__)
+namespace ll {
+__device__ __forceinline__ double lmw_readlane(double v, int src)
+{
+    return __hiloint2double(__builtin_amdgcn_readlane(__double2hiint(v), src), __builtin_amdgcn_readlane(__double2loint(v), src));
+}
+__device__ __forceinline__ void lmw_fence()
+{
+    __builtin_amdgcn_fence(__ATOMIC_RELEASE, "wavefront");
+    __builtin_amdgcn_wave_barrier();
+    __builtin_amdgcn_fence(__ATOMIC_ACQUIRE, "wavefront");
+}
+}
+#define LMW_FOR(l) for (int l = lane_, lmw_once_ = 1; lmw_once_; lmw_once_ = 0)
+#define LMW_VAR(T, name) T name
+#define LMW_ARR(T, name, n) T name[n]
+#define LMW_V(name) name
+#define LMW_A(name, k) name[k]
+#define LMW_BC(name, src) lmw_readlane(name, src)
+#define LMW_BCA(name, k, src) lmw_readlane(name[k], src)
+#define LMW_BCI(name, src) __builtin_amdgcn_readlane(name, src)
+#define LMW_ONE if (lane_ == 0)
+#define LMW_FENCE() lmw_fence()
+#define LMW_QUINTIC(a) lm_quintic_min_step_wave_call(a, lane_)
+#else
+#define LMW_FOR(l) for (int l = 0; l < 64; l++)
+#define LMW_VAR(T, name) T name[64]
+#define LMW_ARR(T, name, n) T name[64][n]
+#define LMW_V(name) name[l]
+#define LMW_A(name, k) name[l][k]
+#define LMW_BC(name, src) name[src]
+#define LMW_BCA(name, k, src) name[src][k]
+#define LMW_BCI(name, src) name
+#define LMW_ONE
+#define LMW_FENCE() ((void)0)
+#define LMW_QUINTIC(a) lm_quintic_min_step(a[0], a[1], a[2], a[3], a[4], a[5], a[6], a[7], a[8], a[9])
+#endif
+
+namespace ll {
+
+LL_HD int lmw_propose(LmCtl &c, bool defer_gmax, bool stop, int lane_)
+{
+    (void)lane_;
+    LMW_FENCE();
+    int iteration = c.iteration, invalid_steps = c.invalid_steps, reuse = c.reuse_diagonal;
+    const int max_iter = c.max_iter;
+    double radius = c.radius;
+    const double bound = c.bound;
+    bool need_gmax = defer_gmax;
+    if (!defer_gmax && c.gmax <= 1e-10) stop = true;
+    double xv[7], gv[6], scv[6];
+    LL_UNROLL
+    for (int i = 0; i < 7; i++) xv[i] = c.x[i];
+    LL_UNROLL
+    for (int i = 0; i < 6; i++) gv[i] = c.g[i], scv[i] = c.scale[i];
+    LMW_ARR(double, Hs, 6);
+    LMW_VAR(double, gs);
+    LMW_VAR(double, Hd);
+    LMW_VAR(double, dg);
+    LMW_FOR(l)
+    {
+        const int a = l < 6 ? l : 5;
+        const double sa = c.scale[a];
+        LMW_V(gs) = c.g[a] * sa;
+        LL_UNROLL
+        for (int b = 0; b < 6; b++) {
+            const double h = (a <= b) ? c.H[hidx(a, b)] : c.H[hidx(b, a)];
+            LMW_A(Hs, b) = h * sa * scv[b];
+        }
+        LMW_V(Hd) = c.H[hidx(a, a)] * sa * sa;
+        LMW_V(dg) = c.diag[a];
+    }
+    int ret;
+    double step[6], delta[6] = {0, 0, 0, 0, 0, 0}, mcc = 0.0, gd = 0.0, dmax = 0.0;
+    LMW_ARR(double, po, 7);
+    LMW_VAR(double, pm);
+    for (;;) {
+        int mode;
+        if (stop || iteration >= max_iter || radius < 1e-32) {
+            if (!need_gmax) {
+                ret = 0;
+                break;
+            }
+            mode = 2;
+        } else {
+            iteration++;
+            if (!reuse) {
+                LMW_FOR(l) LMW_V(dg) = fmin(fmax(LMW_V(Hd), 1e-6), 1e32);
+            }
+            reuse = 1;
+            LMW_ARR(double, Ar, 6);
+            LMW_ARR(double, Lr, 6);
+            LMW_VAR(double, s);
+            LMW_FOR(l)
+            {
+                const double dr = LMW_V(dg) / radius;
+                LL_UNROLL
+                for (int b = 0; b < 6; b++) {
+                    LMW_A(Ar, b) = (b == l) ? LMW_A(Hs, b) + dr : LMW_A(Hs, b);
+                    LMW_A(Lr, b) = 0.0;
+                }
+            }
+            int ok = 1;
+            double inv[6];
+            LL_UNROLL
+            for (int j = 0; j < 6; j++) {
+                LMW_FOR(l)
+                {
+                    double t = LMW_A(Ar, j);
+                    LL_UNROLL
+                    for (int k = 0; k < 6; k++)
+                        if (k < j) t -= LMW_A(Lr, k) * LMW_BCA(Lr, k, j);
+                    LMW_V(s) = t;
+                }
+                const double sp = LMW_BC(s, j);
+                if (!(sp > 0.0)) ok = 0;
+                const double d = sqrt(sp);
+                inv[j] = 1.0 / d;
+                LMW_FOR(l) LMW_A(Lr, j) = (l == j) ? d : LMW_V(s) * inv[j];
+            }
+            double y[6], x[6];
+            LMW_VAR(double, fs);
+            LMW_FOR(l) LMW_V(fs) = LMW_V(gs);
+            LL_UNROLL
+            for (int i = 0; i < 6; i++) {
+                y[i] = LMW_BC(fs, i) * inv[i];
+                LMW_FOR(l) LMW_V(fs) -= LMW_A(Lr, i) * y[i];
+            }
+            LL_UNROLL
+            for (int i = 5; i >= 0; i--) {
+                double t = y[i];
+                LL_UNROLL
+                for (int k = 0; k < 6; k++)
+                    if (k > i) t -= LMW_BCA(Lr, i, k) * x[k];
+                x[i] = t * inv[i];
+            }
+            LL_UNROLL
+            for (int i = 0; i < 6; i++)
+                if (!((x[i] - x[i]) == 0.0)) ok = 0;
+            mcc = 0.0;
+            if (ok) {
+                double sg = 0.0, sHs = 0.0;
+                LL_UNROLL
+                for (int a = 0; a < 6; a++) step[a] = -x[a];
+                LMW_VAR(double, tr);
+                LMW_FOR(l)
+                {
+                    double t = 0.0;
+                    LL_UNROLL
+                    for (int b = 0; b < 6; b++) t += LMW_A(Hs, b) * step[b];
+                    LMW_V(tr) = t;
+                }
+                LL_UNROLL
+                for (int a = 0; a < 6; a++) {
+                    sg += step[a] * LMW_BC(gs, a);
+                    sHs += step[a] * LMW_BC(tr, a);
+                }
+                mcc = -sg - 0.5 * sHs;
+            }
+            mode = (ok && mcc > 0.0) ? 0 : 1;
+        }
+        if (mode == 0) {
+            gd = 0.0;
+            dmax = 0.0;
+            LL_UNROLL
+            for (int j = 0; j < 6; j++) {
+                delta[j] = step[j] * scv[j];
+                gd += gv[j] * delta[j];
+                dmax = fmax(dmax, fabs(delta[j]));
+            }
+        }
+        if (mode == 0 || need_gmax) {
+            LMW_FOR(l)
+            {
+                const bool grad = need_gmax && (l == 1 || mode != 0);
+                double d[6], out[7], m = 0.0;
+                LL_UNROLL
+                for (int j = 0; j < 6; j++) d[j] = grad ? -gv[j] : delta[j];
+                state_plus(xv, d, bound, out);
+                LL_UNROLL
+                for (int i = 0; i < 7; i++) {
+                    m = fmax(m, fabs(xv[i] - out[i]));
+                    LMW_A(po, i) = out[i];
+                }
+                LMW_V(pm) = m;
+            }
+        }
+        if (need_gmax) {
+            const double gm = LMW_BC(pm, 1);
+            need_gmax = false;
+            LMW_ONE c.gmax = gm;
+            if (gm <= 1e-10 || mode == 2) {
+                LMW_ONE c.done = 1;
+                return 0;
+            }
+        }
+        if (mode == 1) {
+            if (++invalid_steps >= 5) {
+                ret = 0;
+                break;
+            }
+            radius *= 0.5;
+            continue;
+        }
+        invalid_steps = 0;
+        ret = 1;
+        break;
+    }
+    LMW_FOR(l)
+    {
+        if (l < 6) c.diag[l] = LMW_V(dg);
+        if (l == 0 && ret)
+            for (int i = 0; i < 7; i++) c.cand[i] = LMW_A(po, i);
+    }
+    LMW_ONE
+    {
+        c.iteration = iteration;
+        c.reuse_diagonal = reuse;
+        c.invalid_steps = invalid_steps;
+        c.radius = radius;
+        if (ret) {
+            c.model_cost_change = mcc;
+            c.gd = gd;
+            c.dmax = dmax;
+            for (int j = 0; j < 6; j++) c.delta[j] = delta[j];
+            c.ls_step = 1.0;
+            c.ls_iter = 0;
+            c.ls_active = 0;
+            c.ls_prev_valid = 0;
+        } else {
+            c.done = 1;
+        }
+    }
+    return ret;
+}
+
+LL_HD int lmw_init(LmCtl &c, const double *e, int n_active, int lane_)
+{
+    (void)lane_;
+    LMW_FOR(l)
+    {
+        const double ev = e[l < LL_NACC ? l : LL_NACC - 1];
+        if (l < 21)
+            c.H[l] = ev;
+        else if (l < 27)
+            c.g[l - 21] = ev;
+        if (l < 6) c.scale[l] = 1.0 / (1.0 + sqrt(e[hidx(l, l)]));
+    }
+    LMW_ONE
+    {
+        c.cost = e[27];
+        c.initial_cost = e[27];
+        c.final_cost = e[27];
+        c.iteration = 0;
+        c.radius = 1e4;
+        c.decrease_factor = 2.0;
+        c.reuse_diagonal = 0;
+        c.invalid_steps = 0;
+    }
+    return lmw_propose(c, true, n_active == 0, lane_);
+}
+
+LL_HD int lmw_line_search(LmCtl &c, double cur_cost, const double eg[6], double *cg_out)
+{
+    const bool finite_cost = (cur_cost - cur_cost) == 0.0;
+    if (!finite_cost || cur_cost > c.cost + 1e-4 * c.gd * c.ls_step) {
+        int failed = 0;
+        double new_step = 0.0, cg = 0.0;
+        if (++c.ls_iter >= 20) {
+            failed = 1;
+        } else {
+            if (!finite_cost) {
+                new_step = fmin(fmax(c.ls_step * 0.5, 1e-3 * c.ls_step), 0.6 * c.ls_step);
+            } else {
+                for (int j = 0; j < 6; j++) cg += eg[j] * c.delta[j];
+                if (c.ls_prev_valid) {
+                    *cg_out = cg;
+                    return LM_FIT;
+                }
+                new_step = lm_cubic_min_step(c.cost, c.gd, c.ls_step, cur_cost, cg, 1e-3 * c.ls_step, 0.6 * c.ls_step);
+            }
+            if (new_step * c.dmax < 1e-9) failed = 1;
+        }
+        return lm_update_contract(c, failed, new_step, finite_cost ? 1 : 0, cur_cost, cg);
+    } else if (c.ls_step != 1.0) {
+        for (int j = 0; j < 6; j++) c.delta[j] *= c.ls_step;
+    }
+    return LM_FINISH_E;
+}
+
+LL_HD int lmw_update(LmCtl &c, const double *sum, double *fit, int lane_)
+{
+    (void)lane_;
+    LMW_VAR(double, ev);
+    LMW_FOR(l) LMW_V(ev) = sum[l < LL_NACC ? l : LL_NACC - 1];
+    const bool bounded = c.bound >= 0;
+    const int ls_active = c.ls_active;
+    int code = LM_FINISH_E;
+    if (bounded && !ls_active) {
+        LMW_FOR(l)
+        {
+            if (l < LL_NACC) c.first_eval[l] = LMW_V(ev);
+            if (l < 7) c.first_cand[l] = c.cand[l];
+        }
+        LMW_FENCE();
+    }
+    {
+        const double cur_cost = LMW_BC(ev, 27);
+        double eg[6];
+        LL_UNROLL
+        for (int j = 0; j < 6; j++) eg[j] = LMW_BC(ev, 21 + j);
+        LMW_ONE
+        {
+            c.last_accept = 0;
+            if (bounded) {
+                c.ls_active = 1;
+                double cg = 0.0;
+                code = lmw_line_search(c, cur_cost, eg, &cg);
+                if (code == LM_FIT) {
+                    fit[0] = c.cost, fit[1] = c.gd, fit[2] = c.ls_step, fit[3] = cur_cost, fit[4] = cg, fit[5] = c.ls_prev_x, fit[6] = c.ls_prev_f, fit[7] = c.ls_prev_g;
+                    fit[8] = 1e-3 * c.ls_step, fit[9] = 0.6 * c.ls_step;
+                }
+            }
+        }
+        code = LMW_BCI(code, 0);
+    }
+    if (code == LM_FIT) {
+        LMW_FENCE();
+        const double step = LMW_QUINTIC(fit);
+        LMW_ONE code = lm_update_post(c, fit[3], fit[4], step);
+        code = LMW_BCI(code, 0);
+    }
+    if (code == LM_EVAL) return 1;
+    LMW_FENCE();
+    const int from_first = (code == LM_FINISH_FIRST && c.ls_iter > 1) ? 1 : 0;
+    if (code == LM_FINISH_FIRST) {
+        LMW_FOR(l) LMW_V(ev) = c.first_eval[l < LL_NACC ? l : LL_NACC - 1];
+    }
+    double cand_cost = LMW_BC(ev, 27);
+    if (!((cand_cost - cand_cost) == 0.0)) cand_cost = DBL_MAX;
+    LMW_VAR(double, nrm);
+    LMW_FOR(l)
+    {
+        double n = 0.0;
+        LL_UNROLL
+        for (int i = 0; i < 7; i++) {
+            const double xi = c.x[i], ci = c.cand[i];
+            const double v = (l == 1) ? ci : xi - ci;
+            n += v * v;
+        }
+        LMW_V(nrm) = sqrt(n);
+    }
+    const double step_norm = LMW_BC(nrm, 0), cand_norm = LMW_BC(nrm, 1);
+    if (step_norm <= 1e-8 * (c.x_norm + 1e-8)) {
+        LMW_ONE c.done = 1;
+        return 0;
+    }
+    const double cost = c.cost;
+    const double cost_change = cost - cand_cost;
+    if (fabs(cost_change) <= 1e-6 * cost) {
+        LMW_ONE c.done = 1;
+        return 0;
+    }
+    const double relative_decrease = cost_change / c.model_cost_change;
+    const bool accepted = relative_decrease > 1e-3;
+    if (accepted) {
+        LMW_FOR(l)
+        {
+            if (l < 7) c.x[l] = c.cand[l];
+            if (l < 21)
+                c.H[l] = LMW_V(ev);
+            else if (l < 27)
+                c.g[l - 21] = LMW_V(ev);
+        }
+        LMW_ONE
+        {
+            c.last_accept = from_first ? 2 : 1;
+            c.x_norm = cand_norm;
+            c.cost = cand_cost;
+            if (cand_cost < c.final_cost) c.final_cost = cand_cost;
+            const double t = 2.0 * relative_decrease - 1.0;
+            c.radius = c.radius / fmax(1.0 / 3.0, 1.0 - t * t * t);
+            c.radius = fmin(1e16, c.radius);
+            c.decrease_factor = 2.0;
+            c.reuse_diagonal = 0;
+        }
+    } else {
+        LMW_ONE
+        {
+            c.radius = c.radius / c.decrease_factor;
+            c.decrease_factor *= 2.0;
+            c.reuse_diagonal = 1;
+        }
+    }
+    return lmw_propose(c, accepted, false, lane_);
+}
+
+}
diff --git a/loam_livox_amd/csrc/ll_reg_aux_kernels.hip b/loam_livox_amd/csrc/ll_reg_aux_kernels.hip
--- a/loam_livox_amd/csrc/ll_reg_aux_kernels.hip
+++ b/loam_livox_amd/csrc/ll_reg_aux_kernels.hip
@@ -110,4 +110,57 @@
     if (n > 0) hipLaunchKernelGGL(debug_quintic_kernel, dim3(n), dim3(64), 0, s, args, n, out_seq, out_wave);
 }
 
+__global__ __launch_bounds__(64) void debug_lm_sequence_kernel(const double *hdr, const double *evals, int n, int max_calls, unsigned int *img_seq,
+                                                               unsigned int *img_wave, int *ret_seq, int *ret_wave)
+{
+    constexpr int WORDS = (int)(sizeof(LmCtl) / sizeof(unsigned int));
+    static_assert(sizeof(LmCtl) % sizeof(unsigned int) == 0, "LmCtl is copied in 32-bit words");
+    __shared__ LmCtl cs, cw;
+    __shared__ double sum[LL_NACC], fit_s[10], fit_w[10];
+    const int i = blockIdx.x, lane = threadIdx.x;
+    if (i >= n) return;
+    const double *h = hdr + 12 * (size_t)i;
+    for (int w = lane; w < WORDS; w += 64) ((unsigned int *)&cs)[w] = 0u, ((unsigned int *)&cw)[w] = 0u;
+    __syncthreads();
+    const int max_iter = (int)h[8], n_active = (int)h[9];
+    int calls = (int)h[10];
+    calls = calls < max_calls ? calls : max_calls;
+    if (lane == 0) {
+        double x0[7];
+        for (int k = 0; k < 7; k++) x0[k] = h[k];
+        lm_begin(cs, x0, max_iter, h[7]);
+        lm_begin(cw, x0, max_iter, h[7]);
+    }
+    for (int k = 0; k < calls; k++) {
+        const size_t slot = (size_t)i * max_calls + k;
+        __syncthreads();
+        if (lane < LL_NACC) sum[lane] = evals[slot * LL_NACC + lane];
+        __syncthreads();
+        int rs, rw;
+        if (k == 0) {
+            rs = lane == 0 ? lm_init(cs, sum, n_active) : 0;
+            rw = lmw_init(cw, sum, n_active, lane);
+        } else {
+            rs = lm_update_lane0(cs, sum, fit_s, lane);
+            rw = lmw_update(cw, sum, fit_w, lane);
+        }
+        rs = __shfl(rs, 0);
+        rw = __shfl(rw, 0);
+        __syncthreads();
+        for (int w = lane; w < WORDS; w += 64) {
+            img_seq[slot * WORDS + w] = ((const unsigned int *)&cs)[w];
+            img_wave[slot * WORDS + w] = ((const unsigned int *)&cw)[w];
+        }
+        if (lane == 0) ret_seq[slot] = rs, ret_wave[slot] = rw;
+        if (!rs || !rw) break;
+    }
 }
+void launch_debug_lm_sequence(const double *hdr, const double *evals, int n, int max_calls, unsigned int *img_seq, unsigned int *img_wave, int *ret_seq,
+                              int *ret_wave, hipStream_t s)
+{
+    if (n > 0 && max_calls > 0)
+        hipLaunchKernelGGL(debug_lm_sequence_kernel, dim3(n), dim3(64), 0, s, hdr, evals, n, max_calls, img_seq, img_wave, ret_seq, ret_wave);
+}
+int debug_lm_ctl_bytes() { return (int)sizeof(LmCtl); }
+
+}
diff --git a/loam_livox_amd/csrc/ll_reg_big_path.h b/loam_livox_amd/csrc/ll_reg_big_path.h
--- a/loam_livox_amd/csrc/ll_reg_big_path.h
+++ b/loam_livox_amd/csrc/ll_reg_big_path.h
@@ -462,7 +462,10 @@
     }
     {
         LL_T0(t1);
-        if (tid == 0) sh.need = lm_init(sh.ctl, sh.sum, n_active);
+        if (tid < 64) {
+            const int need = lm_init_wave(sh.ctl, sh.sum, n_active, tid);
+            if (tid == 0) sh.need = need;
+        }
         __syncthreads();
         LL_TACC(1, t1);
     }
@@ -476,7 +479,7 @@
         LL_TACC(0, t0);
         LL_T0(t1);
         if (tid < 64) {
-            const int need = lm_update_wave(sh.ctl, sh.sum, sh.fit, tid);
+            const int need = lm_update_wave(sh.ctl, sh.sum, sh.fit, tid, sh.tcyc + 14);
             if (tid == 0) {
                 sh.need = need;
                 sh.l1_valid = (spec && !need && sh.ctl.last_accept == 1) ? 1 : 0;
@@ -884,7 +887,7 @@
     }
     lm_iters += sh.ctl.iteration;
     solve_epilogue(rc, st, sh, lm_iters);
-#ifdef LL_SOLVE_TIMING
+#if defined(LL_SOLVE_TIMING) || defined(LL_LM_COUNTS)
     LL_TACC(5, t_total);
     if (tid == 0)
         for (int i = 0; i < 16; i++) st->dbg_cycles[i] += sh.tcyc[i];
diff --git a/loam_livox_amd/csrc/ll_reg_small_kernels.hip b/loam_livox_amd/csrc/ll_reg_small_kernels.hip
--- a/loam_livox_amd/csrc/ll_reg_small_kernels.hip
+++ b/loam_livox_amd/csrc/ll_reg_small_kernels.hip
@@ -186,7 +186,10 @@
     }
     {
         SM_T0(t1);
-        if (tid == 0) sh.need = lm_init(sh.ctl, sh.sum, sh.n_active);
+        if (tid < 64) {
+            const int need = lm_init_wave(sh.ctl, sh.sum, sh.n_active, tid);
+            if (tid == 0) sh.need = need;
+        }
         __syncthreads();
         SM_TACC(1, t1);
     }
@@ -196,7 +199,7 @@
         SM_TACC(0, t0);
         SM_T0(t1);
         if (tid < 64) {
-            const int need = lm_update_wave(sh.ctl, sh.sum, sh.fit, tid);
+            const int need = lm_update_wave(sh.ctl, sh.sum, sh.fit, tid, sh.tcyc + 14);
             if (tid == 0) {
                 sh.need = need;
                 sh.n_eval++;
diff --git a/loam_livox_amd/csrc/ll_reg_small_solve.h b/loam_livox_amd/csrc/ll_reg_small_solve.h
--- a/loam_livox_amd/csrc/ll_reg_small_solve.h
+++ b/loam_livox_amd/csrc/ll_reg_small_solve.h
@@ -35,7 +35,7 @@
     }
     const size_t sb = (size_t)b * rd.cap_all;
     const unsigned char *flag0 = rd.blk_flag0 + sb;
-#ifdef LL_SOLVE_TIMING
+#if defined(LL_SOLVE_TIMING) || defined(LL_LM_COUNTS)
     if (tid < 16) sh.tcyc[tid] = 0;
     __syncthreads();
 #endif
@@ -346,7 +346,7 @@
     lm_iters += sh.ctl.iteration;
     solve_epilogue(rc, st, sh, lm_iters);
     if (tid == 0) st->last_work = sh.n_eval;
-#ifdef LL_SOLVE_TIMING
+#if defined(LL_SOLVE_TIMING) || defined(LL_LM_COUNTS)
     SM_TACC(5, t_total);
     if (tid == 0)
         for (int i = 0; i < 16; i++) st->dbg_cycles[i] += sh.tcyc[i];
diff --git a/loam_livox_amd/csrc/ll_reg_solve_common.h b/loam_livox_amd/csrc/ll_reg_solve_common.h
--- a/loam_livox_amd/csrc/ll_reg_solve_common.h
+++ b/loam_livox_amd/csrc/ll_reg_solve_common.h
@@ -169,7 +169,7 @@
     return lm_quintic_min_step_wave(a[0], a[1], a[2], a[3], a[4], a[5], a[6], a[7], a[8], a[9], lane);
 }
 
-__device__ __forceinline__ int lm_update_wave(LmCtl &c, const double *sum, double *fit, int lane)
+__device__ __forceinline__ int lm_update_lane0(LmCtl &c, const double *sum, double *fit, int lane, int *fits = nullptr)
 {
     int code = 0;
     double e[LL_NACC];
@@ -189,6 +189,7 @@
         __builtin_amdgcn_fence(__ATOMIC_ACQUIRE, "wavefront");
         const double step = lm_quintic_min_step_wave_call(fit, lane);
         if (lane == 0) code = lm_update_post(c, fit[3], fit[4], step);
+        if (fits) *fits += 1;
     }
     int r = 0;
     if (lane == 0) r = lm_update_close(c, e, code);
@@ -196,3 +197,40 @@
 }
 
 }
+
+#include "ll_lm_wave.h"
+
+namespace ll {
+
+__device__ __forceinline__ int lm_init_wave(LmCtl &c, const double *sum, int n_active, int lane)
+{
+#if defined(LL_LM_LANE0)
+    return lane == 0 ? lm_init(c, sum, n_active) : 0;
+#else
+    return lmw_init(c, sum, n_active, lane);
+#endif
+}
+__device__ __forceinline__ int lm_update_wave(LmCtl &c, const double *sum, double *fit, int lane, long long *counts)
+{
+#if defined(LL_LM_COUNTS)
+#if !defined(LL_LM_LANE0) || defined(LL_SOLVE_TIMING)
+#error "LL_LM_COUNTS goes with LL_LM_LANE0 and without LL_SOLVE_TIMING"
+#endif
+    int fits = 0;
+    const double radius = c.radius;
+    const int need = lm_update_lane0(c, sum, fit, lane, &fits);
+    if (lane == 0) {
+        counts[0] += fits;
+        if (!need && c.last_accept == 0 && c.radius != radius) counts[1] += 1;
+    }
+    return need;
+#elif defined(LL_LM_LANE0)
+    (void)counts;
+    return lm_update_lane0(c, sum, fit, lane);
+#else
+    (void)counts;
+    return lmw_update(c, sum, fit, lane);
+#endif
+}
+
+}
diff --git a/loam_livox_amd/csrc/ll_reg_solve_fast.h b/loam_livox_amd/csrc/ll_reg_solve_fast.h
--- a/loam_livox_amd/csrc/ll_reg_solve_fast.h
+++ b/loam_livox_amd/csrc/ll_reg_solve_fast.h
@@ -1084,7 +1084,10 @@
     }
     {
         LL_T0(t1);
-        if (tid == 0) sh.need = lm_init(sh.ctl, sh.sum, n_active);
+        if (tid < 64) {
+            const int need = lm_init_wave(sh.ctl, sh.sum, n_active, tid);
+            if (tid == 0) sh.need = need;
+        }
         __syncthreads();
         LL_TACC(1, t1);
     }
@@ -1098,7 +1101,7 @@
         LL_TACC(0, t0);
         LL_T0(t1);
         if (tid < 64) {
-            const int need = lm_update_wave(sh.ctl, sh.sum, sh.fit, tid);
+            const int need = lm_update_wave(sh.ctl, sh.sum, sh.fit, tid, sh.tcyc + 14);
             if (tid == 0) {
                 sh.need = need;
                 sh.l1_valid = (spec && !need && sh.ctl.last_accept == 1) ? 1 : 0;
@@ -1201,7 +1204,7 @@
 }
 
 template <bool GROUPED>
-__device__ void solve_fast3(const RegDev &rd, const RegConst &rc, const f4 *map_pts, int b, RegState *st, SolveShared &sh, uint4 *s_raw)
+__device__ __forceinline__ void solve_fast3(const RegDev &rd, const RegConst &rc, const f4 *map_pts, int b, RegState *st, SolveShared &sh, uint4 *s_raw)
 {
     constexpr int DEBLUR = 0;
     const int tid = threadIdx.x;
@@ -1243,7 +1246,7 @@
         }
     }
     solve_epilogue(rc, st, sh, lm_iters);
-#ifdef LL_SOLVE_TIMING
+#if defined(LL_SOLVE_TIMING) || defined(LL_LM_COUNTS)
     LL_TACC(5, t_total);
     if (tid == 0)
         for (int i = 0; i < 16; i++) st->dbg_cycles[i] += sh.tcyc[i];
```

Measured after the change: 53290 scans/s, median of 6. 1.1% higher.
